# HiLab-git/FPL-plus

Hardware: NVIDIA B200
Metric: train_voxels_per_s (higher is better)
Workload: dtype bf16

## Files before the change

fpl-plus_b200/build.py:

```python
import os
import shutil
import subprocess
import sys

HERE = os.path.dirname(os.path.abspath(__file__))
CSRC = os.path.join(HERE, "csrc")
LIB = os.path.join(HERE, "libfplplus_b200.so")
SOURCES = ["api.cu", "dsbn.cu", "loss.cu", "filter.cu", "conv_direct.cu", "conv_tc.cu", "conv_wgrad_tc.cu", "conv_wgrad_hs.cu", "convt_tc.cu", "conv_tc_dfold.cu", "grad.cu", "adam.cu", "datapath.cu", "head.cu", "head_tc.cu", "stem_tc.cu", "upsample.cu"]
NVCC_FLAGS = ["-gencode", "arch=compute_100a,code=sm_100a", "-lineinfo", "-O3", "-std=c++17",
              "-Xcompiler", "-fPIC", "--use_fast_math=false"]


def _nvcc():
    for cand in (os.environ.get("NVCC"), shutil.which("nvcc"), "/usr/local/cuda/bin/nvcc"):
        if cand and os.path.exists(cand):
            return cand
    raise RuntimeError("nvcc not found; the fplplus_b200 CUDA library cannot be built")


def needs_build():
    if not os.path.exists(LIB):
        return True
    t = os.path.getmtime(LIB)
    deps = [os.path.join(CSRC, f) for f in os.listdir(CSRC)] + [os.path.join(HERE, "..", "include", "fplplus_b200.h")]
    return any(os.path.getmtime(d) > t for d in deps)


def build(force=False, verbose=False):
    ab = os.environ.get("FPL_LIB_AB")
    if ab and os.path.exists(ab):
        return ab
    if not force and not needs_build():
        return LIB
    nvcc = _nvcc()
    flags = [f for f in NVCC_FLAGS if not f.startswith("--use_fast_math")]
    objs = []
    bdir = os.path.join(HERE, "build")
    os.makedirs(bdir, exist_ok=True)
    procs = []
    for src in SOURCES:
        path = os.path.join(CSRC, src)
        if not os.path.exists(path):
            continue
        obj = os.path.join(bdir, src.replace(".cu", ".o"))
        objs.append(obj)
        cmd = [nvcc] + flags + ["-c", path, "-o", obj]
        if verbose:
            print(" ".join(cmd))
        procs.append((src, subprocess.Popen(cmd, stdout=subprocess.PIPE, stderr=subprocess.STDOUT)))
    for src, p in procs:
        out, _ = p.communicate()
        if p.returncode != 0:
            raise RuntimeError("nvcc failed on %s:\n%s" % (src, out.decode()))
    cmd = [nvcc, "-shared", "-gencode", "arch=compute_100a,code=sm_100a", "-o", LIB] + objs
    subprocess.check_call(cmd)
    return LIB


if __name__ == "__main__":
    print(build(force="--force" in sys.argv, verbose=True))
```

fpl-plus_b200/csrc/conv_wgrad_tc.cu:

```cuda
#include "common.cuh"
#include "tc_ptx.cuh"
#include "../../include/fplplus_b200.h"

namespace {

int g_wg_hs_dbg = 0;
int g_wg_hs = 1;
int g_wg_swap = 0, g_wg_allow_m64 = 1, g_wg_m64_quadrant = 1, g_wg_allow_pair = 1, g_wg_force_tw = 0, g_wg_tiles_per_cta = 2, g_wg_skip_epilogue = 0;

constexpr int kThreadsW = 192;
constexpr int kMaxStagesW = 8;
constexpr int kSmemBudgetW = 220 * 1024;

struct WgCfg {
    int th, tw;
    int nkd;
    int c8chunk;
    int mtiles_c, mtiles_kd;
    int m;
    int nb, nchunks;
    int plane_x, plane_dy;
    int dy_off;
    int x_bytes, dy_bytes, stage_bytes, stages, pad_bytes, smem_bytes;
    int tmem_cols;
    int ndy;
    int ncols;
};

bool make_wg_cfg(int h, int w, int cin, int cout, int kd, int allow_m64, int allow_pair, WgCfg& c) {
    if (cin % 8 != 0 || (cout % 16 != 0 && cout != 8) || cin <= 0 || cout <= 0) return false;
    c.tw = w >= 32 ? 32 : (w >= 16 ? 16 : 8);
    c.th = h >= 8 ? 8 : ((h + 1) / 2) * 2;
    const int g_all = cin / 8;
    c.ndy = 1;
    if (allow_pair && kd == 3 && g_all <= 4 && cout % 16 == 0) c.ndy = 2;
    else if (allow_pair && kd == 1 && cout == 8 && g_all <= 2) c.ndy = 4;
    else if (allow_pair && kd == 1 && cout == 8 && g_all <= 4) c.ndy = 2;
    else if (allow_pair && kd == 1 && cout == 16 && g_all <= 8) c.ndy = 2;
    if (c.ndy > 1) { c.nkd = c.ndy + kd - 1; c.c8chunk = g_all; c.mtiles_kd = 1; c.mtiles_c = 1; }
    else if (kd * g_all <= 16) { c.nkd = kd; c.c8chunk = g_all; c.mtiles_kd = 1; c.mtiles_c = 1; }
    else {
        c.nkd = 1; c.mtiles_kd = kd;
        c.c8chunk = g_all < 16 ? g_all : 16;
        if (g_all % c.c8chunk != 0) return false;
        c.mtiles_c = g_all / c.c8chunk;
    }
    const int groups = c.nkd * c.c8chunk;
    c.m = (groups <= 8 && allow_m64) ? 64 : 128;
    if (cout == 8 && c.m != 64) return false;
    c.nb = cout == 8 ? 8 : ((cout % 32 == 0 && c.ndy == 1) ? 32 : 16);
    c.ncols = c.ndy * c.nb;
    c.nchunks = cout / c.nb;
    if (groups > 8 && c.tw == 32 && cin >= 32 && h * w >= 128 * 128) c.tw = 16;
    if (g_wg_force_tw > 0 && g_wg_force_tw <= w) c.tw = g_wg_force_tw;
    c.plane_x = (c.th + 2) * (c.tw + 2) * 16;
    c.plane_dy = c.th * c.tw * 16;
    c.x_bytes = groups * c.plane_x;
    c.dy_bytes = (c.ncols / 8) * c.plane_dy;
    c.dy_off = ((c.x_bytes + 127) / 128) * 128;
    c.stage_bytes = ((c.dy_off + c.dy_bytes + 127) / 128) * 128;
    int over = (c.m / 8 + 1) * c.plane_x - c.stage_bytes;
    c.pad_bytes = over > 0 ? ((over + 127) / 128) * 128 : 0;
    c.stages = (kSmemBudgetW - c.pad_bytes - 2048) / c.stage_bytes;
    if (c.stages > kMaxStagesW) c.stages = kMaxStagesW;
    if (c.stages < 2) return false;
    c.smem_bytes = c.stages * c.stage_bytes + c.pad_bytes + 1024 + 256;
    int cols = 9 * c.ncols;
    c.tmem_cols = 32;
    while (c.tmem_cols < cols) c.tmem_cols *= 2;
    return c.tmem_cols <= 512;
}

struct WgParams {
    float* dw;
    float* dump;
    int N, D, H, W, cin, cout, kd;
    int x_c8off, dy_c8off;
    int th, tw, nkd, c8chunk, mtiles_c, mtiles_kd, m, nb, nchunks;
    int plane_x, plane_dy, x_bytes, dy_off, stage_bytes, stages, tmem_cols;
    int tiles_h, tiles_w, tiles_total, split;
    int swap_lbo_sbo, m64_quadrant_layout;
    int ndy, ncols, dplanes;
    int taps;
    int skip_epilogue;
    int tapmajor;
};

struct WgWork {
    int mt_kd, mt_c, nc, slice;
};

__device__ __forceinline__ WgWork decode_work(const WgParams& P, int b) {
    WgWork w;
    w.slice = b % P.split; b /= P.split;
    w.nc = b % P.nchunks; b /= P.nchunks;
    w.mt_c = b % P.mtiles_c;
    w.mt_kd = b / P.mtiles_c;
    return w;
}

__global__ void __launch_bounds__(kThreadsW) conv3d_wgrad_tc_kernel(const __grid_constant__ CUtensorMap xmap,
                                                                   const __grid_constant__ CUtensorMap dymap, WgParams P) {
    extern __shared__ uint8_t smem_raw[];
    uint8_t* smem = reinterpret_cast<uint8_t*>((reinterpret_cast<uintptr_t>(smem_raw) + 1023) & ~uintptr_t(1023));
    uint64_t* bars = reinterpret_cast<uint64_t*>(smem);
    uint64_t* full_bar = bars;
    uint64_t* empty_bar = bars + kMaxStagesW;
    uint64_t* done_bar = bars + 2 * kMaxStagesW;
    uint32_t* tmem_slot = reinterpret_cast<uint32_t*>(bars + 2 * kMaxStagesW + 1);
    uint8_t* ring = smem + 256;

    const int warp = threadIdx.x >> 5, lane = threadIdx.x & 31;
    const WgWork wk = decode_work(P, blockIdx.x);
    const int tile_begin = (int)(((int64_t)P.tiles_total * wk.slice) / P.split);
    const int tile_end = (int)(((int64_t)P.tiles_total * (wk.slice + 1)) / P.split);
    const int pad_d = P.kd / 2;
    const int kd0 = P.mtiles_kd > 1 ? wk.mt_kd : 0;

    if (warp == 0 && lane == 0) {
        asm volatile("prefetch.tensormap [%0];" ::"l"(&xmap) : "memory");
        asm volatile("prefetch.tensormap [%0];" ::"l"(&dymap) : "memory");
        for (int s = 0; s < P.stages; ++s) { mbar_init(&full_bar[s], 1); mbar_init(&empty_bar[s], 1); }
        mbar_init(done_bar, 1);
        fence_barrier_init();
    }
    if (warp == 1) tmem_alloc(tmem_slot, (uint32_t)P.tmem_cols);
    FPL_PDL_WAIT();
    tc_fence_before();
    __syncthreads();
    tc_fence_after();
    const uint32_t tmem_base = *tmem_slot;

    if (warp == 0) {
        if (lane == 0) {
            int stage = 0; uint32_t phase = 0;
            for (int t = tile_begin; t < tile_end; ++t) {
                int r = t;
                const int dp = r % P.dplanes; r /= P.dplanes;
                const int tw_i = r % P.tiles_w; r /= P.tiles_w;
                const int th_i = r % P.tiles_h;
                const int n = r / P.tiles_h;
                const int d = P.ndy * dp;
                mbar_wait(&empty_bar[stage], phase ^ 1);
                uint8_t* x_dst = ring + (size_t)stage * P.stage_bytes;
                uint8_t* dy_dst = x_dst + P.dy_off;
                mbar_expect_tx(&full_bar[stage], (uint32_t)(P.x_bytes + (P.ncols / 8) * P.plane_dy));
                tma_load_5d(x_dst, &xmap, &full_bar[stage], 2 * (tw_i * P.tw - 1), th_i * P.th - 1,
                            P.x_c8off + wk.mt_c * P.c8chunk, d + kd0 - pad_d, n);
                tma_load_5d(dy_dst, &dymap, &full_bar[stage], 2 * (tw_i * P.tw), th_i * P.th,
                            P.dy_c8off + wk.nc * (P.nb / 8), d, n);
                if (++stage == P.stages) { stage = 0; phase ^= 1; }
            }
        }
    } else if (warp == 1) {
        const uint32_t idesc = (1u << 4) | (1u << 7) | (1u << 10) | (1u << 15) | (1u << 16) |
                               ((uint32_t)(P.ncols >> 3) << 17) | ((uint32_t)(P.m >> 4) << 24);
        const uint32_t pitch_x = (uint32_t)(P.tw + 2) * 16, pitch_dy = (uint32_t)P.tw * 16;
        const uint32_t a_lbo = P.swap_lbo_sbo ? (uint32_t)P.plane_x : pitch_x;
        const uint32_t a_sbo = P.swap_lbo_sbo ? pitch_x : (uint32_t)P.plane_x;
        const uint32_t b_lbo = P.swap_lbo_sbo ? (uint32_t)P.plane_dy : pitch_dy;
        const uint32_t b_sbo = P.swap_lbo_sbo ? pitch_dy : (uint32_t)P.plane_dy;
        const uint64_t a_hi = make_desc(0, a_lbo, a_sbo), b_hi = make_desc(0, b_lbo, b_sbo);
        uint32_t tap_off[9];
#pragma unroll
        for (int t9 = 0; t9 < 9; ++t9) tap_off[t9] = ((uint32_t)(t9 / 3) * pitch_x + (uint32_t)(t9 % 3) * 16) >> 4;
        uint32_t d_tap[9];
#pragma unroll
        for (int t9 = 0; t9 < 9; ++t9) d_tap[t9] = tmem_base + (uint32_t)(t9 * P.ncols);
        const uint32_t ring_u = smem_u32(ring);
        const bool leader = elect_one();
        int stage = 0; uint32_t phase = 0;
        uint32_t accumulate = 0;
        for (int t = tile_begin; t < tile_end; ++t) {
            mbar_wait(&full_bar[stage], phase);
            tc_fence_after();
            const uint32_t x_base = (ring_u + (uint32_t)stage * (uint32_t)P.stage_bytes) >> 4;
            const uint32_t dy_base = x_base + ((uint32_t)P.dy_off >> 4);
            for (int hp = 0; hp < P.th / 2; ++hp) {
                const uint32_t a_row = x_base + (((uint32_t)(2 * hp) * pitch_x) >> 4);
                const uint32_t b_row = dy_base + (((uint32_t)(2 * hp) * pitch_dy) >> 4);
                uint64_t bdesc = b_hi + (uint64_t)b_row, a_col = a_hi + (uint64_t)a_row;
                for (int j = 0; j < P.tw / 8; ++j, bdesc += 8, a_col += 8) {
                    if (P.taps == 1) {
                        if (leader) umma_bf16(tmem_base, a_col + (uint64_t)tap_off[4], bdesc, idesc, accumulate);
                    } else {
#pragma unroll
                        for (int t9 = 0; t9 < 9; ++t9)
                            if (leader) umma_bf16(d_tap[t9], a_col + (uint64_t)tap_off[t9], bdesc, idesc, accumulate);
                    }
                    accumulate = 1;
                }
            }
            if (leader) umma_commit(&empty_bar[stage]);
            __syncwarp();
            if (++stage == P.stages) { stage = 0; phase ^= 1; }
        }
        if (leader) umma_commit(done_bar);
        __syncwarp();
        FPL_PDL_TRIGGER();
    } else if (tile_end > tile_begin) {
        const int quarter = warp & 3;
        mbar_wait(done_bar, 0);
        tc_fence_after();
        const int T = P.kd * P.taps;
        const int tlane = quarter * 32 + lane;
        int row;
        if (P.m == 128 || !P.m64_quadrant_layout) row = tlane;
        else row = (lane < 16) ? quarter * 16 + lane : -1;
        bool valid = row >= 0 && row < P.m;
        int kdi = 0, ci = 0;
        if (valid) {
            const int g = row >> 3;
            valid = g < P.nkd * P.c8chunk;
            kdi = kd0 + g / P.c8chunk;
            ci = (wk.mt_c * P.c8chunk + g % P.c8chunk) * 8 + (row & 7);
        }
        for (int t9 = 0; t9 < P.taps; ++t9) {
            for (int c0 = 0; c0 < P.ncols; c0 += 16) {
                uint32_t r[16];
                tmem_ld16(tmem_base + ((uint32_t)(quarter * 32) << 16) + (uint32_t)(t9 * P.ncols + c0), r);
                tmem_ld_wait();
                if (P.dump != nullptr && blockIdx.x == 0) {
#pragma unroll
                    for (int i = 0; i < 16; ++i) P.dump[((int64_t)t9 * 128 + tlane) * P.ncols + c0 + i] = __uint_as_float(r[i]);
                }
#pragma unroll
                for (int half = 0; half < 2; ++half) {
                    const int col = c0 + 8 * half;
                    const int dd = P.ndy > 1 ? col / P.nb : 0;
                    const int kd_tap = P.ndy > 1 ? kdi - dd : kdi;
                    const int co0 = wk.nc * P.nb + (col - dd * P.nb);
                    if (!(valid && kd_tap >= 0 && kd_tap < P.kd && !P.skip_epilogue)) continue;
                    if (P.tapmajor) {
                        float* base = P.dw + ((int64_t)(kd_tap * P.taps + t9) * P.cout + co0) * P.cin + ci;
#pragma unroll
                        for (int i = 0; i < 8; ++i) atomicAdd(base + (int64_t)i * P.cin, __uint_as_float(r[8 * half + i]));
                    } else {
#pragma unroll
                        for (int i = 0; i < 8; ++i)
                            atomicAdd(P.dw + ((int64_t)(co0 + i) * P.cin + ci) * T + kd_tap * P.taps + t9,
                                      __uint_as_float(r[8 * half + i]));
                    }
                }
            }
        }
    }
    tc_fence_before();
    __syncthreads();
    if (warp == 1) {
        tc_fence_after();
        tmem_dealloc(tmem_base, (uint32_t)P.tmem_cols);
    }
}

float* g_wg_dump = nullptr;

CUresult encode_5d(EncodeTiledFn encode, CUtensorMap* map, const void* base, int n, int d, int c8tot, int h, int w,
                   int box_w, int box_h, int box_c8, int box_d) {
    cuuint64_t gdim[5] = {(cuuint64_t)w * 2, (cuuint64_t)h, (cuuint64_t)c8tot, (cuuint64_t)d, (cuuint64_t)n};
    cuuint64_t gstr[4] = {(cuuint64_t)w * 16, (cuuint64_t)h * w * 16, (cuuint64_t)c8tot * h * w * 16,
                          (cuuint64_t)d * c8tot * h * w * 16};
    cuuint32_t box[5] = {(cuuint32_t)box_w * 2, (cuuint32_t)box_h, (cuuint32_t)box_c8, (cuuint32_t)box_d, 1};
    cuuint32_t estr[5] = {1, 1, 1, 1, 1};
    return encode(map, CU_TENSOR_MAP_DATA_TYPE_UINT64, 5, const_cast<void*>(base), gdim, gstr, box, estr,
                  CU_TENSOR_MAP_INTERLEAVE_NONE, CU_TENSOR_MAP_SWIZZLE_NONE, CU_TENSOR_MAP_L2_PROMOTION_L2_128B,
                  CU_TENSOR_MAP_FLOAT_OOB_FILL_NONE);
}

}

bool fpl_wgrad_hs_eligible(int d, int h, int w, int cin, int cout, int kd, int taps);
int fpl_wgrad_hs_launch(const void* x, int x_c8tot, int x_c8off, const void* dy, int dy_c8tot, int dy_c8off, float* dw, int n,
                        int d, int h, int w, int cin, int cout, void* stream, int tapmajor, int skip_epilogue, int force_tw, int dbg);
bool fpl_wgrad_rs_eligible(int d, int h, int w, int cin, int cout, int kd, int taps);
int fpl_wgrad_rs_launch(const void* x, int x_c8tot, int x_c8off, const void* dy, int dy_c8tot, int dy_c8off, float* dw, int n,
                        int d, int h, int w, void* stream, int tapmajor, int skip_epilogue);

void fpl_wgrad_debug_set(int key, long long value) {
    if (key == 10) g_wg_swap = (int)value;
    if (key == 11) g_wg_allow_m64 = (int)value;
    if (key == 12) g_wg_m64_quadrant = (int)value;
    if (key == 13) g_wg_dump = reinterpret_cast<float*>(value);
    if (key == 14) g_wg_allow_pair = (int)value;
    if (key == 15) g_wg_force_tw = (int)value;
    if (key == 16) g_wg_tiles_per_cta = (int)value;
    if (key == 17) g_wg_skip_epilogue = (int)value;
    if (key == 18) g_wg_hs = (int)value;
    if (key == 19) g_wg_hs_dbg = (int)value;
}

static int wgrad_tc_launch(const void* x, int x_c8tot, int x_c8off, const void* dy, int dy_c8tot, int dy_c8off,
                           float* dw, int n, int d, int h, int w, int cin, int cout, int kd, int taps, void* stream,
                           int tapmajor = 0) {
    FPL_REQUIRE(kd == 1 || kd == 3, "fpl_conv3d_wgrad_tc: kd=%d must be 1 or 3", kd);
    if (g_wg_hs && fpl_wgrad_hs_eligible(d, h, w, cin, cout, kd, taps))
        return fpl_wgrad_hs_launch(x, x_c8tot, x_c8off, dy, dy_c8tot, dy_c8off, dw, n, d, h, w, cin, cout, stream, tapmajor,
                                   g_wg_skip_epilogue, g_wg_force_tw, g_wg_hs_dbg);
    if (g_wg_hs && fpl_wgrad_rs_eligible(d, h, w, cin, cout, kd, taps))
        return fpl_wgrad_rs_launch(x, x_c8tot, x_c8off, dy, dy_c8tot, dy_c8off, dw, n, d, h, w, stream, tapmajor, g_wg_skip_epilogue);
    WgCfg c;
    FPL_REQUIRE(make_wg_cfg(h, w, cin, cout, kd, g_wg_allow_m64, g_wg_allow_pair && d >= 2, c),
                "fpl_conv3d_wgrad_tc: unsupported shape (cin %d, cout %d, %dx%d)", cin, cout, h, w);
    FPL_REQUIRE((reinterpret_cast<uintptr_t>(x) & 15) == 0 && (reinterpret_cast<uintptr_t>(dy) & 15) == 0,
                "fpl_conv3d_wgrad_tc: x/dy must be 16-byte aligned");
    EncodeTiledFn encode = get_encode_fn();
    FPL_REQUIRE(encode != nullptr, "fpl_conv3d_wgrad_tc: cuTensorMapEncodeTiled not available from the driver");
    CUtensorMap xmap, dymap;
    CUresult r = encode_5d(encode, &xmap, x, n, d, x_c8tot, h, w, c.tw + 2, c.th + 2, c.c8chunk, c.nkd);
    FPL_REQUIRE(r == CUDA_SUCCESS, "fpl_conv3d_wgrad_tc: tensor map (x) failed (%d)", (int)r);
    r = encode_5d(encode, &dymap, dy, n, d, dy_c8tot, h, w, c.tw, c.th, c.nb / 8, c.ndy);
    FPL_REQUIRE(r == CUDA_SUCCESS, "fpl_conv3d_wgrad_tc: tensor map (dy) failed (%d)", (int)r);
    WgParams P;
    P.dw = dw; P.dump = g_wg_dump;
    P.N = n; P.D = d; P.H = h; P.W = w; P.cin = cin; P.cout = cout; P.kd = kd;
    P.x_c8off = x_c8off; P.dy_c8off = dy_c8off;
    P.th = c.th; P.tw = c.tw; P.nkd = c.nkd; P.c8chunk = c.c8chunk; P.mtiles_c = c.mtiles_c; P.mtiles_kd = c.mtiles_kd;
    P.m = c.m; P.nb = c.nb; P.nchunks = c.nchunks; P.plane_x = c.plane_x; P.plane_dy = c.plane_dy; P.x_bytes = c.x_bytes; P.dy_off = c.dy_off;
    P.stage_bytes = c.stage_bytes; P.stages = c.stages; P.tmem_cols = c.tmem_cols;
    P.tiles_h = (h + c.th - 1) / c.th; P.tiles_w = (w + c.tw - 1) / c.tw;
    P.ndy = c.ndy; P.ncols = c.ncols; P.dplanes = (d + c.ndy - 1) / c.ndy;
    int64_t tiles = (int64_t)P.tiles_h * P.tiles_w * P.dplanes * n;
    FPL_REQUIRE(tiles < (1ll << 30), "fpl_conv3d_wgrad_tc: too many tiles");
    P.tiles_total = (int)tiles;
    const int pairs = c.mtiles_kd * c.mtiles_c * c.nchunks;
    int split = FPL_NUM_SMS / pairs;
    if (split > P.tiles_total / g_wg_tiles_per_cta) split = P.tiles_total / g_wg_tiles_per_cta;
    if (split < 1) split = 1;
    P.split = split;
    P.swap_lbo_sbo = g_wg_swap; P.m64_quadrant_layout = g_wg_m64_quadrant;
    P.taps = taps; P.skip_epilogue = g_wg_skip_epilogue; P.tapmajor = tapmajor;
    FPL_CHECK_CUDA(cudaFuncSetAttribute(conv3d_wgrad_tc_kernel, cudaFuncAttributeMaxDynamicSharedMemorySize, c.smem_bytes));
    fpl_launch(conv3d_wgrad_tc_kernel, pairs * split, kThreadsW, c.smem_bytes, (cudaStream_t)stream, xmap, dymap, P);
    FPL_LAUNCH_CHECK();
    return 0;
}

extern "C" int fpl_conv3d_wgrad_tc(const void* x, int x_c8tot, int x_c8off, const void* dy, int dy_c8tot, int dy_c8off,
                                   float* dw, int n, int d, int h, int w, int cin, int cout, int kd, void* stream) {
    return wgrad_tc_launch(x, x_c8tot, x_c8off, dy, dy_c8tot, dy_c8off, dw, n, d, h, w, cin, cout, kd, 9, stream);
}

extern "C" int fpl_conv3d_wgrad_tc_k311(const void* x, int x_c8tot, int x_c8off, const void* dy, int dy_c8tot, int dy_c8off,
                                        float* dw, int n, int d, int h, int w, int cin, int cout, void* stream) {
    return wgrad_tc_launch(x, x_c8tot, x_c8off, dy, dy_c8tot, dy_c8off, dw, n, d, h, w, cin, cout, 3, 1, stream);
}

extern "C" int fpl_conv3d_wgrad_tc_tapmajor(const void* x, int x_c8tot, int x_c8off, const void* dy, int dy_c8tot, int dy_c8off,
                                            float* scratch, int n, int d, int h, int w, int cin, int cout, int kd,
                                            void* stream) {
    return wgrad_tc_launch(x, x_c8tot, x_c8off, dy, dy_c8tot, dy_c8off, scratch, n, d, h, w, cin, cout, kd, 9, stream, 1);
}

namespace {
constexpr int kMaxFold = 64;
struct FoldBatch {
    const float* s[kMaxFold];
    float* dw[kMaxFold];
    int cout[kMaxFold], cin[kMaxFold], taps[kMaxFold], scout[kMaxFold];
};
constexpr int kFoldRows = 256;
__global__ void __launch_bounds__(256) fold_tapmajor_kernel(const __grid_constant__ FoldBatch B) {
    FPL_PDL_WAIT();
    __shared__ float tile[kFoldRows * 27];
    const int e = blockIdx.y;
    const float* __restrict__ s = B.s[e];
    float* dw = B.dw[e];
    const int cout = B.cout[e], cin = B.cin[e];
    const bool transposed = B.taps[e] < 0;
    const int T = transposed ? -B.taps[e] : B.taps[e];
    const int Tp = T | 1;
    const uint32_t magic = 0xffffffffu / (uint32_t)T + 1u;
    const int rows = cout * cin;
    const int64_t tap_stride = (int64_t)B.scout[e] * cin;
    for (int r0 = blockIdx.x * kFoldRows; r0 < rows; r0 += gridDim.x * kFoldRows) {
        const int nr = min(kFoldRows, rows - r0);
        const int r = threadIdx.x;
        if (r < nr) {
            int src = r0 + r;
            if (transposed) {
                const int ci = src / cout, co = src - ci * cout;
                src = co * cin + ci;
            }
            const float* sp = s + src;
            if (T == 27) {
                float t27[27];
#pragma unroll
                for (int tap = 0; tap < 27; ++tap) t27[tap] = __ldg(sp + tap * tap_stride);
#pragma unroll
                for (int tap = 0; tap < 27; ++tap) tile[r * Tp + tap] = t27[tap];
            } else {
#pragma unroll 9
                for (int tap = 0; tap < T; ++tap) tile[r * Tp + tap] = __ldg(sp + tap * tap_stride);
            }
        }
        __syncthreads();
        float* out = dw + (int64_t)r0 * T;
        const int total = nr * T;
        for (int i0 = threadIdx.x; i0 < total; i0 += 9 * (int)blockDim.x) {
            float v[9];
#pragma unroll
            for (int k = 0; k < 9; ++k) {
                const int i = i0 + k * (int)blockDim.x;
                v[k] = i < total ? out[i] : 0.0f;
            }
#pragma unroll
            for (int k = 0; k < 9; ++k) {
                const int i = i0 + k * (int)blockDim.x;
                if (i < total) {
                    const int rr = (int)__umulhi((uint32_t)i, magic), tap = i - rr * T;
                    out[i] = v[k] + tile[rr * Tp + tap];
                }
            }
        }
        __syncthreads();
    }
}
}

extern "C" int fpl_wgrad_tapmajor_to_dw_batch(int count, const float* const* h_scratch, float* const* h_dw, const int* h_cout,
                                              const int* h_cin, const int* h_taps, const int* h_scratch_cout, void* stream) {
    FPL_REQUIRE(count >= 0 && count <= kMaxFold, "fpl_wgrad_tapmajor_to_dw_batch: count %d not in [0,%d]", count, kMaxFold);
    if (count == 0) return 0;
    FoldBatch B;
    int max_total = 0;
    for (int e = 0; e < count; ++e) {
        B.s[e] = h_scratch[e]; B.dw[e] = h_dw[e]; B.cout[e] = h_cout[e]; B.cin[e] = h_cin[e]; B.taps[e] = h_taps[e];
        B.scout[e] = h_scratch_cout != nullptr ? h_scratch_cout[e] : h_cout[e];
        FPL_REQUIRE((h_taps[e] < 0 ? -h_taps[e] : h_taps[e]) <= 27 && h_taps[e] != 0, "fpl_wgrad_tapmajor_to_dw_batch: tap count %d out of range", h_taps[e]);
        FPL_REQUIRE(B.scout[e] >= B.cout[e], "fpl_wgrad_tapmajor_to_dw_batch: scratch rows %d < folded rows %d", B.scout[e], B.cout[e]);
        const int total = h_cout[e] * h_cin[e] * (h_taps[e] < 0 ? -h_taps[e] : h_taps[e]);
        if (total > max_total) max_total = total;
    }
    int bx = (max_total / 9 + kFoldRows - 1) / kFoldRows;
    if (bx > 296) bx = 296;
    if (bx < 1) bx = 1;
    fpl_launch(fold_tapmajor_kernel, dim3(bx, count), 256, 0, (cudaStream_t)stream, B);
    FPL_LAUNCH_CHECK();
    return 0;
}
```

fpl-plus_b200/csrc/convt_tc.cu:

```cuda
#include "common.cuh"
#include "tc_ptx.cuh"
#include "../../include/fplplus_b200.h"

namespace {

constexpr int kTH = 16, kTW = 8;
constexpr int kPlane = kTH * kTW * 16;
constexpr int kThreadsT = 192;
constexpr int kMaxStagesT = 8;

__device__ __forceinline__ void tma_load_4d(void* dst, const CUtensorMap* map, uint64_t* bar, int c0, int c1, int c2, int c3) {
    asm volatile(
        "cp.async.bulk.tensor.4d.shared::cluster.global.tile.mbarrier::complete_tx::bytes [%0], [%1, {%3, %4, %5, %6}], [%2];"
        ::"r"(smem_u32(dst)), "l"(map), "r"(smem_u32(bar)), "r"(c0), "r"(c1), "r"(c2), "r"(c3)
        : "memory");
}

struct CtParams {
    const __nv_bfloat16* image;
    const float* bias;
    bf16x8* out;
    int out_c8tot, out_c8off;
    int a_c8tot, a_c8off;
    int N, D, H, W;
    int cin, cout, kd2, ntaps;
    int mode;
    int kdim, ndim;
    int nb, kc, nslices, nchunks, a_bytes, b_bytes, stages, tmem_cols;
    int tiles_h, tiles_w, total_items;
};

struct CtCfg {
    int nb, kc, nslices, nchunks, a_bytes, b_bytes, stages, tmem_cols, smem_bytes;
};

bool make_ct_cfg(int kdim, int ndim, int kc_div, CtCfg& c) {
    if (kdim % 16 || ndim % 16) return false;
    c.nb = ndim;
    if (c.nb > 128) {
        if (ndim % 128 == 0) c.nb = 128;
        else if (ndim % 64 == 0) c.nb = 64;
        else if (ndim % 32 == 0) c.nb = 32;
        else c.nb = 16;
    }
    c.kc = 64;
    while (c.kc > 16 && (kc_div % c.kc != 0)) c.kc /= 2;
    if (kc_div % c.kc != 0) return false;
    c.nslices = ndim / c.nb;
    c.nchunks = kdim / c.kc;
    c.a_bytes = (c.kc / 8) * kPlane;
    c.b_bytes = c.kc * c.nb * 2;
    int stage = c.a_bytes + c.b_bytes;
    c.stages = (96 * 1024) / stage;
    if (c.stages > kMaxStagesT) c.stages = kMaxStagesT;
    if (c.stages < 2) c.stages = 2;
    int cols = 2 * c.nb;
    c.tmem_cols = 32;
    while (c.tmem_cols < cols) c.tmem_cols *= 2;
    c.smem_bytes = c.stages * stage + 1024 + 256 + (ndim > 1024 ? ndim : 1024) * (int)sizeof(float) + 16;
    return true;
}

__global__ void __launch_bounds__(kThreadsT) convt_gemm_tc_kernel(const __grid_constant__ CUtensorMap amap, CtParams P) {
    extern __shared__ uint8_t smem_raw[];
    uint8_t* smem = reinterpret_cast<uint8_t*>((reinterpret_cast<uintptr_t>(smem_raw) + 1023) & ~uintptr_t(1023));
    const int stage_bytes = P.a_bytes + P.b_bytes;
    uint64_t* bars = reinterpret_cast<uint64_t*>(smem + (size_t)P.stages * stage_bytes);
    uint64_t* full_bar = bars;
    uint64_t* empty_bar = bars + kMaxStagesT;
    uint64_t* tmem_full = bars + 2 * kMaxStagesT;
    uint64_t* tmem_empty = bars + 2 * kMaxStagesT + 2;
    uint32_t* tmem_slot = reinterpret_cast<uint32_t*>(bars + 2 * kMaxStagesT + 4);
    float* bias_sm = reinterpret_cast<float*>(bars + 2 * kMaxStagesT + 6);

    const int warp = threadIdx.x >> 5, lane = threadIdx.x & 31;
    if (warp == 0 && lane == 0) {
        asm volatile("prefetch.tensormap [%0];" ::"l"(&amap) : "memory");
        for (int s = 0; s < P.stages; ++s) { mbar_init(&full_bar[s], 1); mbar_init(&empty_bar[s], 1); }
        for (int a = 0; a < 2; ++a) { mbar_init(&tmem_full[a], 1); mbar_init(&tmem_empty[a], 4); }
        fence_barrier_init();
    }
    if (warp == 1) tmem_alloc(tmem_slot, (uint32_t)P.tmem_cols);
    FPL_PDL_WAIT();
    if (P.mode == 0)
        for (int i = threadIdx.x; i < P.ndim; i += kThreadsT) bias_sm[i] = P.bias != nullptr ? P.bias[i % P.cout] : 0.0f;
    tc_fence_before();
    __syncthreads();
    tc_fence_after();
    const uint32_t tmem_base = *tmem_slot;
    const int Do = P.D * P.kd2;
    const int chunks_per_tap = P.cout / P.kc;

    if (warp == 0) {
        if (lane == 0) {
            int stage = 0; uint32_t phase = 0;
            for (int it = blockIdx.x; it < P.total_items; it += gridDim.x) {
                int t = it;
                const int tw = t % P.tiles_w; t /= P.tiles_w;
                const int th = t % P.tiles_h; t /= P.tiles_h;
                const int d = t % P.D; t /= P.D;
                const int n = t % P.N;
                const int slice = t / P.N;
                for (int q = 0; q < P.nchunks; ++q) {
                    mbar_wait(&empty_bar[stage], phase ^ 1);
                    uint8_t* a_dst = smem + (size_t)stage * stage_bytes;
                    mbar_expect_tx(&full_bar[stage], (uint32_t)(P.a_bytes + P.b_bytes));
                    if (P.mode == 0) {
                        tma_load_4d(a_dst, &amap, &full_bar[stage], 0, tw * kTW, th * kTH,
                                    (n * P.D + d) * P.a_c8tot + P.a_c8off + q * (P.kc / 8));
                    } else {
                        const int tap = q / chunks_per_tap, cq = q - tap * chunks_per_tap;
                        const int a = P.kd2 == 2 ? tap >> 2 : 0, b = (tap >> 1) & 1, c = tap & 1;
                        tma_load_4d(a_dst, &amap, &full_bar[stage], 0, 2 * tw * kTW + c, 2 * th * kTH + b,
                                    (n * Do + d * P.kd2 + a) * P.a_c8tot + P.a_c8off + cq * (P.kc / 8));
                    }
                    const uint8_t* b_src = reinterpret_cast<const uint8_t*>(P.image) + (size_t)(slice * P.nchunks + q) * P.b_bytes;
                    bulk_load(a_dst + P.a_bytes, b_src, (uint32_t)P.b_bytes, &full_bar[stage]);
                    if (++stage == P.stages) { stage = 0; phase ^= 1; }
                }
            }
        }
    } else if (warp == 1) {
        const uint32_t idesc = (1u << 4) | (1u << 7) | (1u << 10) | ((uint32_t)(P.nb >> 3) << 17) | (8u << 24);
        const uint64_t a_hi = make_desc(0, kPlane, kTW * 16), b_hi = make_desc(0, (uint32_t)P.nb * 16, 128);
        const uint32_t smem_u = smem_u32(smem) >> 4;
        const int ksteps = P.kc / 16;
        const bool leader = elect_one();
        int stage = 0; uint32_t phase = 0;
        int acc = 0; uint32_t acc_phase = 0;
        for (int it = blockIdx.x; it < P.total_items; it += gridDim.x) {
            mbar_wait(&tmem_empty[acc], acc_phase ^ 1);
            tc_fence_after();
            const uint32_t d_tmem = tmem_base + (uint32_t)(acc * P.nb);
            uint32_t accumulate = 0;
            for (int q = 0; q < P.nchunks; ++q) {
                mbar_wait(&full_bar[stage], phase);
                tc_fence_after();
                const uint32_t a_base = smem_u + (uint32_t)(((size_t)stage * stage_bytes) >> 4);
                const uint32_t b_base = a_base + (uint32_t)(P.a_bytes >> 4);
                uint64_t adesc = a_hi + (uint64_t)a_base, bdesc = b_hi + (uint64_t)b_base;
                const uint64_t b_step = (uint64_t)(2 * P.nb);
                for (int j = 0; j < ksteps; ++j, adesc += 2 * kPlane / 16, bdesc += b_step) {
                    if (leader) umma_bf16(d_tmem, adesc, bdesc, idesc, accumulate);
                    accumulate = 1;
                }
                if (leader) umma_commit(&empty_bar[stage]);
                __syncwarp();
                if (++stage == P.stages) { stage = 0; phase ^= 1; }
            }
            if (leader) umma_commit(&tmem_full[acc]);
            __syncwarp();
            if (++acc == 2) { acc = 0; acc_phase ^= 1; }
        }
        FPL_PDL_TRIGGER();
    } else {
        const int quarter = warp & 3;
        const int row = quarter * 32 + lane;
        const int hl = row / kTW, wl = row % kTW;
        int acc = 0; uint32_t acc_phase = 0;
        const int Ho = P.H * 2, Wo = P.W * 2;
        for (int it = blockIdx.x; it < P.total_items; it += gridDim.x) {
            int t = it;
            const int tw = t % P.tiles_w; t /= P.tiles_w;
            const int th = t % P.tiles_h; t /= P.tiles_h;
            const int d = t % P.D; t /= P.D;
            const int n = t % P.N;
            const int slice = t / P.N;
            mbar_wait(&tmem_full[acc], acc_phase);
            tc_fence_after();
            const int h = th * kTH + hl, w = tw * kTW + wl;
            const bool valid = h < P.H && w < P.W;
            const uint32_t t_row = tmem_base + ((uint32_t)(quarter * 32) << 16) + (uint32_t)(acc * P.nb);
            for (int c0 = 0; c0 < P.nb; c0 += 16) {
                uint32_t r[16];
                tmem_ld16(t_row + (uint32_t)c0, r);
                tmem_ld_wait();
                float v[16];
                const int col = slice * P.nb + c0;
                if (P.mode == 0) {
#pragma unroll
                    for (int i = 0; i < 16; ++i) v[i] = __uint_as_float(r[i]) + bias_sm[col + i];
                    if (valid) {
                        const int tap = col / P.cout, co = col - tap * P.cout;
                        const int a = P.kd2 == 2 ? tap >> 2 : 0, b = (tap >> 1) & 1, c = tap & 1;
                        const int64_t HWo = (int64_t)Ho * Wo;
                        bf16x8* dst = P.out + (((int64_t)n * Do + d * P.kd2 + a) * P.out_c8tot + P.out_c8off + co / 8) * HWo +
                                      (int64_t)(2 * h + b) * Wo + (2 * w + c);
                        st_bf16x8(dst, v);
                        st_bf16x8(dst + HWo, v + 8);
                    }
                } else {
#pragma unroll
                    for (int i = 0; i < 16; ++i) v[i] = __uint_as_float(r[i]);
                    if (valid) {
                        const int64_t HW = (int64_t)P.H * P.W;
                        bf16x8* dst = P.out + (((int64_t)n * P.D + d) * P.out_c8tot + P.out_c8off + col / 8) * HW + (int64_t)h * P.W + w;
                        st_bf16x8(dst, v);
                        st_bf16x8(dst + HW, v + 8);
                    }
                }
            }
            tc_fence_before();
            __syncwarp();
            if (lane == 0) mbar_arrive(&tmem_empty[acc]);
            if (++acc == 2) { acc = 0; acc_phase ^= 1; }
        }
    }
    tc_fence_before();
    __syncthreads();
    if (warp == 1) {
        tc_fence_after();
        tmem_dealloc(tmem_base, (uint32_t)P.tmem_cols);
    }
}

__global__ void convt_prep_kernel(const float* __restrict__ w, __nv_bfloat16* image, int cin, int cout, int ntaps, int mode,
                                  int nb, int kc, int nchunks, int total) {
    FPL_PDL_WAIT();
    for (int i = blockIdx.x * blockDim.x + threadIdx.x; i < total; i += gridDim.x * blockDim.x) {
        int t = i;
        const int el = t % 8; t /= 8;
        const int nrow = t % nb; t /= nb;
        const int k8 = t % (kc / 8); t /= (kc / 8);
        const int q = t % nchunks;
        const int sl = t / nchunks;
        const int k = q * kc + k8 * 8 + el, nn = sl * nb + nrow;
        int ci, co, tap;
        if (mode == 0) { ci = k; tap = nn / cout; co = nn - tap * cout; }
        else { tap = k / cout; co = k - tap * cout; ci = nn; }
        image[i] = __float2bfloat16_rn(w[((int64_t)ci * cout + co) * ntaps + tap]);
    }
}

CUresult encode_4d(EncodeTiledFn encode, CUtensorMap* map, const void* base, int64_t planes, int h, int w, int box_c8,
                   int stride) {
    cuuint64_t gdim[4] = {8, (cuuint64_t)w, (cuuint64_t)h, (cuuint64_t)planes};
    cuuint64_t gstr[3] = {16, (cuuint64_t)w * 16, (cuuint64_t)h * w * 16};
    cuuint32_t box[4] = {8, (cuuint32_t)(kTW * stride), (cuuint32_t)(kTH * stride), (cuuint32_t)box_c8};
    cuuint32_t estr[4] = {1, (cuuint32_t)stride, (cuuint32_t)stride, 1};
    return encode(map, CU_TENSOR_MAP_DATA_TYPE_BFLOAT16, 4, const_cast<void*>(base), gdim, gstr, box, estr,
                  CU_TENSOR_MAP_INTERLEAVE_NONE, CU_TENSOR_MAP_SWIZZLE_NONE, CU_TENSOR_MAP_L2_PROMOTION_L2_128B,
                  CU_TENSOR_MAP_FLOAT_OOB_FILL_NONE);
}

struct CtwParams {
    float* dw;
    int N, D, H, W, cin, cout, kd2, ntaps;
    int x_c8tot, x_c8off, dy_c8tot, dy_c8off;
    int mgroups, m, nb, mtiles, nchunks;
    int x_bytes, dy_tile_bytes, stage_bytes, stages, tmem_cols;
    int tiles_h, tiles_w, tiles_total, split;
    int tapmajor;
};

__global__ void __launch_bounds__(kThreadsT) convt_wgrad_tc_kernel(const __grid_constant__ CUtensorMap xmap,
                                                                  const __grid_constant__ CUtensorMap dymap, CtwParams P) {
    extern __shared__ uint8_t smem_raw[];
    uint8_t* smem = reinterpret_cast<uint8_t*>((reinterpret_cast<uintptr_t>(smem_raw) + 1023) & ~uintptr_t(1023));
    uint64_t* bars = reinterpret_cast<uint64_t*>(smem);
    uint64_t* full_bar = bars;
    uint64_t* empty_bar = bars + kMaxStagesT;
    uint64_t* done_bar = bars + 2 * kMaxStagesT;
    uint32_t* tmem_slot = reinterpret_cast<uint32_t*>(bars + 2 * kMaxStagesT + 1);
    uint8_t* ring = smem + 256;

    const int warp = threadIdx.x >> 5, lane = threadIdx.x & 31;
    int b = blockIdx.x;
    const int slice = b % P.split; b /= P.split;
    const int nc = b % P.nchunks;
    const int mt = b / P.nchunks;
    const int tile_begin = (int)(((int64_t)P.tiles_total * slice) / P.split);
    const int tile_end = (int)(((int64_t)P.tiles_total * (slice + 1)) / P.split);
    const int Do = P.D * P.kd2;

    if (warp == 0 && lane == 0) {
        asm volatile("prefetch.tensormap [%0];" ::"l"(&xmap) : "memory");
        asm volatile("prefetch.tensormap [%0];" ::"l"(&dymap) : "memory");
        for (int s = 0; s < P.stages; ++s) { mbar_init(&full_bar[s], 1); mbar_init(&empty_bar[s], 1); }
        mbar_init(done_bar, 1);
        fence_barrier_init();
    }
    if (warp == 1) tmem_alloc(tmem_slot, (uint32_t)P.tmem_cols);
    FPL_PDL_WAIT();
    tc_fence_before();
    __syncthreads();
    tc_fence_after();
    const uint32_t tmem_base = *tmem_slot;

    if (warp == 0) {
        if (lane == 0) {
            int stage = 0; uint32_t phase = 0;
            for (int t = tile_begin; t < tile_end; ++t) {
                int r = t;
                const int tw = r % P.tiles_w; r /= P.tiles_w;
                const int th = r % P.tiles_h; r /= P.tiles_h;
                const int d = r % P.D;
                const int n = r / P.D;
                mbar_wait(&empty_bar[stage], phase ^ 1);
                uint8_t* x_dst = ring + (size_t)stage * P.stage_bytes;
                mbar_expect_tx(&full_bar[stage], (uint32_t)(P.x_bytes + P.ntaps * P.dy_tile_bytes));
                tma_load_4d(x_dst, &xmap, &full_bar[stage], 0, tw * kTW, th * kTH,
                            (n * P.D + d) * P.x_c8tot + P.x_c8off + mt * P.mgroups);
                for (int tap = 0; tap < P.ntaps; ++tap) {
                    const int a = P.kd2 == 2 ? tap >> 2 : 0, bb = (tap >> 1) & 1, c = tap & 1;
                    tma_load_4d(x_dst + P.x_bytes + (size_t)tap * P.dy_tile_bytes, &dymap, &full_bar[stage], 0,
                                2 * tw * kTW + c, 2 * th * kTH + bb,
                                (n * Do + d * P.kd2 + a) * P.dy_c8tot + P.dy_c8off + nc * (P.nb / 8));
                }
                if (++stage == P.stages) { stage = 0; phase ^= 1; }
            }
        }
    } else if (warp == 1) {
        const uint32_t idesc = (1u << 4) | (1u << 7) | (1u << 10) | (1u << 15) | (1u << 16) |
                               ((uint32_t)(P.nb >> 3) << 17) | ((uint32_t)(P.m >> 4) << 24);
        const uint64_t hi = make_desc(0, kTW * 16, kPlane);
        const uint32_t ring_u = smem_u32(ring);
        const bool leader = elect_one();
        int stage = 0; uint32_t phase = 0;
        uint32_t accumulate = 0;
        for (int t = tile_begin; t < tile_end; ++t) {
            mbar_wait(&full_bar[stage], phase);
            tc_fence_after();
            const uint32_t x_base = (ring_u + (uint32_t)stage * (uint32_t)P.stage_bytes) >> 4;
            const uint32_t dy_base = x_base + ((uint32_t)P.x_bytes >> 4);
            uint64_t adesc = hi + (uint64_t)x_base, b_hp = hi + (uint64_t)dy_base;
            const uint64_t dy_tile16 = (uint64_t)((uint32_t)P.dy_tile_bytes >> 4);
            for (int hp = 0; hp < kTH / 2; ++hp, adesc += 2 * kTW * 16 / 16, b_hp += 2 * kTW * 16 / 16) {
                uint64_t bdesc = b_hp;
                uint32_t d_tap = tmem_base;
                for (int tap = 0; tap < P.ntaps; ++tap, bdesc += dy_tile16, d_tap += (uint32_t)P.nb) {
                    if (leader) umma_bf16(d_tap, adesc, bdesc, idesc, accumulate);
                }
                accumulate = 1;
            }
            if (leader) umma_commit(&empty_bar[stage]);
            __syncwarp();
            if (++stage == P.stages) { stage = 0; phase ^= 1; }
        }
        if (leader) umma_commit(done_bar);
        __syncwarp();
        FPL_PDL_TRIGGER();
    } else if (tile_end > tile_begin) {
        const int quarter = warp & 3;
        mbar_wait(done_bar, 0);
        tc_fence_after();
        const int tlane = quarter * 32 + lane;
        int row = P.m == 128 ? tlane : ((lane < 16) ? quarter * 16 + lane : -1);
        const bool valid = row >= 0 && row < P.mgroups * 8 && (mt * P.mgroups * 8 + row) < P.cin;
        const int ci = mt * P.mgroups * 8 + row;
        for (int tap = 0; tap < P.ntaps; ++tap) {
            for (int c0 = 0; c0 < P.nb; c0 += 16) {
                uint32_t r[16];
                tmem_ld16(tmem_base + ((uint32_t)(quarter * 32) << 16) + (uint32_t)(tap * P.nb + c0), r);
                tmem_ld_wait();
                if (valid) {
#pragma unroll
                    for (int i = 0; i < 16; ++i) {
                        const int co = nc * P.nb + c0 + i;
                        if (P.tapmajor) atomicAdd(P.dw + ((int64_t)tap * P.cout + co) * P.cin + ci, __uint_as_float(r[i]));
                        else atomicAdd(P.dw + ((int64_t)ci * P.cout + co) * P.ntaps + tap, __uint_as_float(r[i]));
                    }
                }
            }
        }
    }
    tc_fence_before();
    __syncthreads();
    if (warp == 1) {
        tc_fence_after();
        tmem_dealloc(tmem_base, (uint32_t)P.tmem_cols);
    }
}

}

extern "C" int64_t fpl_convt_weight_image_bytes(int cin, int cout, int kd2) {
    return (int64_t)cin * cout * 4 * kd2 * 2;
}

extern "C" int fpl_convt_prep_weight(const float* w, int cin, int cout, int kd2, int mode, void* image, void* stream) {
    FPL_REQUIRE(kd2 == 1 || kd2 == 2, "fpl_convt_prep_weight: kd2=%d must be 1 or 2", kd2);
    const int ntaps = 4 * kd2;
    CtCfg c;
    const int kdim = mode == 0 ? cin : ntaps * cout, ndim = mode == 0 ? ntaps * cout : cin;
    FPL_REQUIRE(make_ct_cfg(kdim, ndim, mode == 0 ? cin : cout, c), "fpl_convt_prep_weight: unsupported channels (%d -> %d)", cin, cout);
    const int total = kdim * ndim;
    int blocks = (total + 255) / 256;
    if (blocks > FPL_NUM_SMS * 4) blocks = FPL_NUM_SMS * 4;
    fpl_launch(convt_prep_kernel, blocks, 256, 0, (cudaStream_t)stream, w, (__nv_bfloat16*)image, cin, cout, ntaps, mode, c.nb, c.kc,
                                                               c.nchunks, total);
    FPL_LAUNCH_CHECK();
    return 0;
}

namespace {
constexpr int kMaxCtBatch = 16;
struct CtPrepBatch {
    const float* w[kMaxCtBatch];
    __nv_bfloat16* image[kMaxCtBatch];
    int cin[kMaxCtBatch], cout[kMaxCtBatch], ntaps[kMaxCtBatch], mode[kMaxCtBatch], nb[kMaxCtBatch], kc[kMaxCtBatch],
        nchunks[kMaxCtBatch], total[kMaxCtBatch];
};
__global__ void convt_prep_batch_kernel(const __grid_constant__ CtPrepBatch B) {
    FPL_PDL_WAIT();
    const int e = blockIdx.y;
    const float* __restrict__ w = B.w[e];
    __nv_bfloat16* image = B.image[e];
    const int cout = B.cout[e], ntaps = B.ntaps[e], mode = B.mode[e], nb = B.nb[e], kc = B.kc[e], nchunks = B.nchunks[e];
    for (int i = blockIdx.x * blockDim.x + threadIdx.x; i < B.total[e]; i += gridDim.x * blockDim.x) {
        int t = i;
        const int el = t % 8; t /= 8;
        const int nrow = t % nb; t /= nb;
        const int k8 = t % (kc / 8); t /= (kc / 8);
        const int q = t % nchunks;
        const int sl = t / nchunks;
        const int k = q * kc + k8 * 8 + el, nn = sl * nb + nrow;
        int ci, co, tap;
        if (mode == 0) { ci = k; tap = nn / cout; co = nn - tap * cout; }
        else { tap = k / cout; co = k - tap * cout; ci = nn; }
        image[i] = __float2bfloat16_rn(w[((int64_t)ci * cout + co) * ntaps + tap]);
    }
}
}

extern "C" int fpl_convt_prep_weight_batch(int count, const float* const* h_w, const int* h_cin, const int* h_cout,
                                           const int* h_kd2, const int* h_mode, void* const* h_images, void* stream) {
    FPL_REQUIRE(count >= 0 && count <= kMaxCtBatch, "fpl_convt_prep_weight_batch: count %d not in [0,%d]", count, kMaxCtBatch);
    if (count == 0) return 0;
    CtPrepBatch B;
    int max_total = 0;
    for (int e = 0; e < count; ++e) {
        const int ntaps = 4 * h_kd2[e], mode = h_mode[e], cin = h_cin[e], cout = h_cout[e];
        const int kdim = mode == 0 ? cin : ntaps * cout, ndim = mode == 0 ? ntaps * cout : cin;
        CtCfg c;
        FPL_REQUIRE(make_ct_cfg(kdim, ndim, mode == 0 ? cin : cout, c), "fpl_convt_prep_weight_batch: unsupported channels (%d -> %d)", cin, cout);
        B.w[e] = h_w[e]; B.image[e] = (__nv_bfloat16*)h_images[e]; B.cin[e] = cin; B.cout[e] = cout; B.ntaps[e] = ntaps;
        B.mode[e] = mode; B.nb[e] = c.nb; B.kc[e] = c.kc; B.nchunks[e] = c.nchunks; B.total[e] = kdim * ndim;
        if (B.total[e] > max_total) max_total = B.total[e];
    }
    int bx = (max_total + 255) / 256;
    if (bx > 64) bx = 64;
    fpl_launch(convt_prep_batch_kernel, dim3(bx, count), 256, 0, (cudaStream_t)stream, B);
    FPL_LAUNCH_CHECK();
    return 0;
}

static int convt_gemm_launch(int mode, const void* a, int a_c8tot, int a_c8off, const void* image, const float* bias, void* out,
                             int out_c8tot, int out_c8off, int n, int d, int h, int w, int cin, int cout, int kd2,
                             void* stream) {
    FPL_REQUIRE(kd2 == 1 || kd2 == 2, "fpl_convt_k2s2_tc: kd2=%d must be 1 or 2", kd2);
    const int ntaps = 4 * kd2;
    const int kdim = mode == 0 ? cin : ntaps * cout, ndim = mode == 0 ? ntaps * cout : cin;
    CtCfg c;
    FPL_REQUIRE(make_ct_cfg(kdim, ndim, mode == 0 ? cin : cout, c), "fpl_convt_k2s2_tc: unsupported channels (%d -> %d)", cin, cout);
    FPL_REQUIRE(ndim <= 8192, "fpl_convt_k2s2_tc: GEMM N = %d too large", ndim);
    EncodeTiledFn encode = get_encode_fn();
    FPL_REQUIRE(encode != nullptr, "fpl_convt_k2s2_tc: cuTensorMapEncodeTiled not available from the driver");
    CUtensorMap amap;
    CUresult r;
    if (mode == 0) r = encode_4d(encode, &amap, a, (int64_t)n * d * a_c8tot, h, w, c.kc / 8, 1);
    else r = encode_4d(encode, &amap, a, (int64_t)n * d * kd2 * a_c8tot, 2 * h, 2 * w, c.kc / 8, 2);
    FPL_REQUIRE(r == CUDA_SUCCESS, "fpl_convt_k2s2_tc: tensor map failed (%d)", (int)r);
    CtParams P;
    P.image = (const __nv_bfloat16*)image; P.bias = bias; P.out = (bf16x8*)out; P.out_c8tot = out_c8tot; P.out_c8off = out_c8off;
    P.a_c8tot = a_c8tot; P.a_c8off = a_c8off; P.N = n; P.D = d; P.H = h; P.W = w; P.cin = cin; P.cout = cout; P.kd2 = kd2;
    P.ntaps = ntaps; P.mode = mode; P.kdim = kdim; P.ndim = ndim;
    P.nb = c.nb; P.kc = c.kc; P.nslices = c.nslices; P.nchunks = c.nchunks; P.a_bytes = c.a_bytes; P.b_bytes = c.b_bytes;
    P.stages = c.stages; P.tmem_cols = c.tmem_cols;
    P.tiles_h = (h + kTH - 1) / kTH; P.tiles_w = (w + kTW - 1) / kTW;
    int64_t total = (int64_t)P.tiles_h * P.tiles_w * d * n * c.nslices;
    FPL_REQUIRE(total < (1ll << 30), "fpl_convt_k2s2_tc: too many tiles");
    P.total_items = (int)total;
    FPL_CHECK_CUDA(cudaFuncSetAttribute(convt_gemm_tc_kernel, cudaFuncAttributeMaxDynamicSharedMemorySize, c.smem_bytes));
    int grid = FPL_NUM_SMS * 2;
    if (grid > P.total_items) grid = P.total_items;
    fpl_launch(convt_gemm_tc_kernel, grid, kThreadsT, c.smem_bytes, (cudaStream_t)stream, amap, P);
    FPL_LAUNCH_CHECK();
    return 0;
}

extern "C" int fpl_convt_k2s2_fwd_tc(const void* x, int x_c8tot, int x_c8off, const void* image, const float* bias, void* y,
                                     int y_c8tot, int y_c8off, int n, int d, int h, int w, int cin, int cout, int kd2,
                                     void* stream) {
    return convt_gemm_launch(0, x, x_c8tot, x_c8off, image, bias, y, y_c8tot, y_c8off, n, d, h, w, cin, cout, kd2, stream);
}

extern "C" int fpl_convt_k2s2_dgrad_tc(const void* dy, int dy_c8tot, int dy_c8off, const void* image_t, void* dx, int dx_c8tot,
                                       int dx_c8off, int n, int d, int h, int w, int cin, int cout, int kd2, void* stream) {
    return convt_gemm_launch(1, dy, dy_c8tot, dy_c8off, image_t, nullptr, dx, dx_c8tot, dx_c8off, n, d, h, w, cin, cout, kd2,
                             stream);
}

static int convt_wgrad_launch(const void* x, int x_c8tot, int x_c8off, const void* dy, int dy_c8tot, int dy_c8off,
                              float* dw, int n, int d, int h, int w, int cin, int cout, int kd2, void* stream, int tapmajor) {
    FPL_REQUIRE(kd2 == 1 || kd2 == 2, "fpl_convt_k2s2_wgrad_tc: kd2=%d must be 1 or 2", kd2);
    FPL_REQUIRE(cin % 8 == 0 && cout % 16 == 0, "fpl_convt_k2s2_wgrad_tc: unsupported channels (%d -> %d)", cin, cout);
    EncodeTiledFn encode = get_encode_fn();
    FPL_REQUIRE(encode != nullptr, "fpl_convt_k2s2_wgrad_tc: cuTensorMapEncodeTiled not available from the driver");
    CtwParams P;
    P.dw = dw; P.N = n; P.D = d; P.H = h; P.W = w; P.cin = cin; P.cout = cout; P.kd2 = kd2; P.ntaps = 4 * kd2;
    P.x_c8tot = x_c8tot; P.x_c8off = x_c8off; P.dy_c8tot = dy_c8tot; P.dy_c8off = dy_c8off; P.tapmajor = tapmajor;
    const int g_all = cin / 8;
    P.mgroups = g_all < 16 ? g_all : 16;
    FPL_REQUIRE(g_all % P.mgroups == 0, "fpl_convt_k2s2_wgrad_tc: cin=%d not tileable", cin);
    P.mtiles = g_all / P.mgroups;
    P.m = P.mgroups <= 8 ? 64 : 128;
    P.nb = cout % 32 == 0 ? 32 : 16;
    P.x_bytes = P.mgroups * kPlane;
    if (2 * (P.x_bytes + P.ntaps * (P.nb / 8) * kPlane) > 200 * 1024 - (P.m / 8) * kPlane) P.nb = 16;
    P.nchunks = cout / P.nb;
    P.dy_tile_bytes = (P.nb / 8) * kPlane;
    P.stage_bytes = P.x_bytes + P.ntaps * P.dy_tile_bytes;
    P.stages = (200 * 1024 - (P.m / 8) * kPlane) / P.stage_bytes;
    if (P.stages > kMaxStagesT) P.stages = kMaxStagesT;
    FPL_REQUIRE(P.stages >= 2, "fpl_convt_k2s2_wgrad_tc: stage of %d bytes does not fit twice", P.stage_bytes);
    int cols = P.ntaps * P.nb;
    P.tmem_cols = 32;
    while (P.tmem_cols < cols) P.tmem_cols *= 2;
    CUtensorMap xmap, dymap;
    CUresult r = encode_4d(encode, &xmap, x, (int64_t)n * d * x_c8tot, h, w, P.mgroups, 1);
    FPL_REQUIRE(r == CUDA_SUCCESS, "fpl_convt_k2s2_wgrad_tc: tensor map (x) failed (%d)", (int)r);
    r = encode_4d(encode, &dymap, dy, (int64_t)n * d * kd2 * dy_c8tot, 2 * h, 2 * w, P.nb / 8, 2);
    FPL_REQUIRE(r == CUDA_SUCCESS, "fpl_convt_k2s2_wgrad_tc: tensor map (dy) failed (%d)", (int)r);
    P.tiles_h = (h + kTH - 1) / kTH; P.tiles_w = (w + kTW - 1) / kTW;
    int64_t tiles = (int64_t)P.tiles_h * P.tiles_w * d * n;
    FPL_REQUIRE(tiles < (1ll << 30), "fpl_convt_k2s2_wgrad_tc: too many tiles");
    P.tiles_total = (int)tiles;
    const int pairs = P.mtiles * P.nchunks;
    int split = FPL_NUM_SMS / pairs;
    if (split > P.tiles_total / 4) split = P.tiles_total / 4;
    if (split < 1) split = 1;
    P.split = split;
    const int smem_bytes = P.stages * P.stage_bytes + (P.m / 8) * kPlane + 1024 + 256;
    FPL_CHECK_CUDA(cudaFuncSetAttribute(convt_wgrad_tc_kernel, cudaFuncAttributeMaxDynamicSharedMemorySize, smem_bytes));
    fpl_launch(convt_wgrad_tc_kernel, pairs * split, kThreadsT, smem_bytes, (cudaStream_t)stream, xmap, dymap, P);
    FPL_LAUNCH_CHECK();
    return 0;
}

extern "C" int fpl_convt_k2s2_wgrad_tc(const void* x, int x_c8tot, int x_c8off, const void* dy, int dy_c8tot, int dy_c8off,
                                       float* dw, int n, int d, int h, int w, int cin, int cout, int kd2, void* stream) {
    return convt_wgrad_launch(x, x_c8tot, x_c8off, dy, dy_c8tot, dy_c8off, dw, n, d, h, w, cin, cout, kd2, stream, 0);
}

extern "C" int fpl_convt_k2s2_wgrad_tc_tapmajor(const void* x, int x_c8tot, int x_c8off, const void* dy, int dy_c8tot,
                                                int dy_c8off, float* scratch, int n, int d, int h, int w, int cin, int cout,
                                                int kd2, void* stream) {
    return convt_wgrad_launch(x, x_c8tot, x_c8off, dy, dy_c8tot, dy_c8off, scratch, n, d, h, w, cin, cout, kd2, stream, 1);
}
```

fpl-plus_b200/csrc/tc_ptx.cuh:

```cuda
#pragma once
#include <cuda.h>
#include <stdint.h>

namespace {

__device__ __forceinline__ uint32_t smem_u32(const void* p) { return (uint32_t)__cvta_generic_to_shared(p); }

__device__ __forceinline__ void mbar_init(uint64_t* bar, uint32_t count) {
    asm volatile("mbarrier.init.shared::cta.b64 [%0], %1;" ::"r"(smem_u32(bar)), "r"(count));
}
__device__ __forceinline__ void mbar_expect_tx(uint64_t* bar, uint32_t bytes) {
    asm volatile("mbarrier.arrive.expect_tx.shared::cta.b64 _, [%0], %1;" ::"r"(smem_u32(bar)), "r"(bytes) : "memory");
}
__device__ __forceinline__ void mbar_arrive(uint64_t* bar) {
    asm volatile("mbarrier.arrive.shared::cta.b64 _, [%0];" ::"r"(smem_u32(bar)) : "memory");
}
__device__ __forceinline__ void mbar_wait(uint64_t* bar, uint32_t parity) {
    uint32_t done;
    do {
        asm volatile(
            "{\n"
            ".reg .pred p;\n"
            "mbarrier.try_wait.parity.shared::cta.b64 p, [%1], %2;\n"
            "selp.u32 %0, 1, 0, p;\n"
            "}\n"
            : "=r"(done)
            : "r"(smem_u32(bar)), "r"(parity)
            : "memory");
    } while (!done);
}
__device__ __forceinline__ void fence_barrier_init() { asm volatile("fence.mbarrier_init.release.cluster;" ::: "memory"); }
__device__ __forceinline__ void fence_proxy_async() { asm volatile("fence.proxy.async.shared::cta;" ::: "memory"); }

__device__ __forceinline__ void tma_load_3d(void* dst, const CUtensorMap* map, uint64_t* bar, int c0, int c1, int c2) {
    asm volatile(
        "cp.async.bulk.tensor.3d.shared::cluster.global.tile.mbarrier::complete_tx::bytes [%0], [%1, {%3, %4, %5}], [%2];"
        ::"r"(smem_u32(dst)), "l"(map), "r"(smem_u32(bar)), "r"(c0), "r"(c1), "r"(c2)
        : "memory");
}
__device__ __forceinline__ void tma_load_5d(void* dst, const CUtensorMap* map, uint64_t* bar, int c0, int c1, int c2, int c3,
                                            int c4) {
    asm volatile(
        "cp.async.bulk.tensor.5d.shared::cluster.global.tile.mbarrier::complete_tx::bytes [%0], [%1, {%3, %4, %5, %6, %7}], [%2];"
        ::"r"(smem_u32(dst)), "l"(map), "r"(smem_u32(bar)), "r"(c0), "r"(c1), "r"(c2), "r"(c3), "r"(c4)
        : "memory");
}

__device__ __forceinline__ void bulk_load(void* dst, const void* src, uint32_t bytes, uint64_t* bar) {
    asm volatile("cp.async.bulk.shared::cluster.global.mbarrier::complete_tx::bytes [%0], [%1], %2, [%3];" ::"r"(smem_u32(dst)),
                 "l"(src), "r"(bytes), "r"(smem_u32(bar))
                 : "memory");
}

__device__ __forceinline__ void tmem_alloc(uint32_t* dst_smem, uint32_t ncols) {
    asm volatile("tcgen05.alloc.cta_group::1.sync.aligned.shared::cta.b32 [%0], %1;" ::"r"(smem_u32(dst_smem)), "r"(ncols) : "memory");
    asm volatile("tcgen05.relinquish_alloc_permit.cta_group::1.sync.aligned;" ::: "memory");
}
__device__ __forceinline__ void tmem_dealloc(uint32_t taddr, uint32_t ncols) {
    asm volatile("tcgen05.dealloc.cta_group::1.sync.aligned.b32 %0, %1;" ::"r"(taddr), "r"(ncols) : "memory");
}
__device__ __forceinline__ void tc_fence_before() { asm volatile("tcgen05.fence::before_thread_sync;" ::: "memory"); }
__device__ __forceinline__ void tc_fence_after() { asm volatile("tcgen05.fence::after_thread_sync;" ::: "memory"); }

__device__ __forceinline__ void umma_bf16(uint32_t tmem_d, uint64_t adesc, uint64_t bdesc, uint32_t idesc, uint32_t accumulate) {
    asm volatile(
        "{\n"
        ".reg .pred p;\n"
        "setp.ne.b32 p, %4, 0;\n"
        "tcgen05.mma.cta_group::1.kind::f16 [%0], %1, %2, %3, p;\n"
        "}\n" ::"r"(tmem_d),
        "l"(adesc), "l"(bdesc), "r"(idesc), "r"(accumulate)
        : "memory");
}
__device__ __forceinline__ void umma_commit(uint64_t* bar) {
    asm volatile("tcgen05.commit.cta_group::1.mbarrier::arrive::one.shared::cluster.b64 [%0];" ::"r"(smem_u32(bar)) : "memory");
}
__device__ __forceinline__ void tmem_ld16(uint32_t taddr, uint32_t* r) {
    asm volatile(
        "tcgen05.ld.sync.aligned.32x32b.x16.b32 {%0,%1,%2,%3,%4,%5,%6,%7,%8,%9,%10,%11,%12,%13,%14,%15}, [%16];"
        : "=r"(r[0]), "=r"(r[1]), "=r"(r[2]), "=r"(r[3]), "=r"(r[4]), "=r"(r[5]), "=r"(r[6]), "=r"(r[7]), "=r"(r[8]),
          "=r"(r[9]), "=r"(r[10]), "=r"(r[11]), "=r"(r[12]), "=r"(r[13]), "=r"(r[14]), "=r"(r[15])
        : "r"(taddr));
}
__device__ __forceinline__ void tmem_ld_wait() { asm volatile("tcgen05.wait::ld.sync.aligned;" ::: "memory"); }

__device__ __forceinline__ bool elect_one() {
    uint32_t pred;
    asm volatile(
        "{\n"
        ".reg .pred p;\n"
        "elect.sync _|p, 0xffffffff;\n"
        "selp.u32 %0, 1, 0, p;\n"
        "}\n"
        : "=r"(pred));
    return pred != 0;
}

__device__ __forceinline__ uint64_t make_desc(uint32_t saddr, uint32_t lbo_bytes, uint32_t sbo_bytes) {
    uint64_t d = 0;
    d |= (uint64_t)((saddr >> 4) & 0x3FFFu);
    d |= (uint64_t)((lbo_bytes >> 4) & 0x3FFFu) << 16;
    d |= (uint64_t)((sbo_bytes >> 4) & 0x3FFFu) << 32;
    d |= (uint64_t)1 << 46;
    return d;
}


typedef CUresult (*EncodeTiledFn)(CUtensorMap*, CUtensorMapDataType, cuuint32_t, void*, const cuuint64_t*, const cuuint64_t*,
                                  const cuuint32_t*, const cuuint32_t*, CUtensorMapInterleave, CUtensorMapSwizzle,
                                  CUtensorMapL2promotion, CUtensorMapFloatOOBfill);

inline EncodeTiledFn get_encode_fn() {
    static EncodeTiledFn fn = nullptr;
    if (fn == nullptr) {
        void* p = nullptr;
        cudaDriverEntryPointQueryResult qres;
        if (cudaGetDriverEntryPoint("cuTensorMapEncodeTiled", &p, cudaEnableDefault, &qres) == cudaSuccess &&
            qres == cudaDriverEntryPointSuccess)
            fn = reinterpret_cast<EncodeTiledFn>(p);
    }
    return fn;
}

}
```

fpl-plus_b200/lib.py:

```python
import ctypes
import os
from ctypes import c_char_p, c_double, c_float, c_int, c_int64, c_longlong, c_uint64, c_void_p

from . import build as _build

_P = c_void_p
_I = c_int
_L = c_int64
_F = c_float
_U = c_uint64

_SIGNATURES = {
    "fpl_last_error": (c_char_p, []),
    "fpl_version": (_I, []),
    "fpl_set_sm_budget": (_I, [_I]),
    "fpl_launch_count": (c_longlong, [_I]),
    "fpl_device_is_sm100": (_I, []),
    "fpl_debug_set": (None, [_I, c_longlong]),
    "fpl_conv3d_weight_image_bytes": (_L, [_I, _I, _I]),
    "fpl_conv3d_prep_weight": (_I, [_P, _I, _I, _I, _I, _P, _P]),
    "fpl_conv3d_prep_weight_batch": (_I, [_I, ctypes.POINTER(c_void_p), ctypes.POINTER(_I), ctypes.POINTER(_I),
                                          ctypes.POINTER(_I), ctypes.POINTER(_I), ctypes.POINTER(c_void_p), _P]),
    "fpl_conv3d_tc": (_I, [_P, _I, _I, _P, _P, _P, _I, _I, _P] + [_I] * 7 + [_P]),
    "fpl_conv3d_dfold_image_bytes": (_L, [_I, _I]),
    "fpl_conv3d_dfold_prep_weight": (_I, [_P, _I, _I, _I, _P, _P]),
    "fpl_conv3d_dfold_prep_weight_batch": (_I, [_I, ctypes.POINTER(c_void_p), ctypes.POINTER(_I), ctypes.POINTER(_I),
                                                ctypes.POINTER(_I), ctypes.POINTER(c_void_p), _P]),
    "fpl_conv3d_tc_dfold": (_I, [_P, _I, _I, _P, _P, _P, _I, _I, _P] + [_I] * 6 + [_P]),
    "fpl_patch9_c8": (_I, [_P, _P, _I, _I, _I, _I, _I, _P]),
    "fpl_conv3d_k311_prep_weight": (_I, [_P, _I, _I, _P, _P]),
    "fpl_conv3d_tc_k311": (_I, [_P, _I, _I, _P, _P, _P, _I, _I, _P] + [_I] * 7 + [_P]),
    "fpl_conv3d_wgrad_tc_k311": (_I, [_P, _I, _I, _P, _I, _I, _P] + [_I] * 6 + [_P]),
    "fpl_conv3d_direct": (_I, [_P, _I, _I, _P, _P, _P, _I, _I, _P] + [_I] * 9 + [_P]),
    "fpl_conv3d_wgrad": (_I, [_P, _I, _I, _P, _I, _I, _P] + [_I] * 7 + [_P]),
    "fpl_conv3d_wgrad_tc": (_I, [_P, _I, _I, _P, _I, _I, _P] + [_I] * 7 + [_P]),
    "fpl_conv3d_wgrad_tc_tapmajor": (_I, [_P, _I, _I, _P, _I, _I, _P] + [_I] * 7 + [_P]),
    "fpl_wgrad_tapmajor_to_dw_batch": (_I, [_I, ctypes.POINTER(c_void_p), ctypes.POINTER(c_void_p), ctypes.POINTER(_I),
                                            ctypes.POINTER(_I), ctypes.POINTER(_I), ctypes.POINTER(_I), _P]),
    "fpl_dsbn_eval_affine_batch": (_I, [_I] + [ctypes.POINTER(c_void_p)] * 7 + [ctypes.POINTER(_I), _F, _P]),
    "fpl_conv3d_tc_act": (_I, [_P, _I, _I, _P, _P, _I, _I] + [_I] * 7 + [_P, _P, _P, _F, _U, _U, _P, _P]),
    "fpl_conv3d_tc_dfold_act": (_I, [_P, _I, _I, _P, _P, _I, _I] + [_I] * 6 + [_P, _P, _P, _P]),
    "fpl_conv3d_tc_k311_act": (_I, [_P, _I, _I, _P, _P, _I, _I] + [_I] * 7 + [_P, _P, _P, _P]),
    "fpl_maxpool_c8": (_I, [_P, _I, _I, _P, _I, _I, _I] + [_I] * 5 + [_P]),
    "fpl_head_fwd": (_I, [_P, _I, _I, _P, _P, _P] + [_I] * 6 + [_P]),
    "fpl_head_dgrad": (_I, [_P, _P, _P, _I, _I, _P, _I, _I, _P] + [_I] * 6 + [_P]),
    "fpl_upsample2x_c8": (_I, [_P, _I, _I, _P, _I, _I] + [_I] * 6 + [_P]),
    "fpl_upsample2x_c8_bwd": (_I, [_P, _I, _I, _P, _I, _I] + [_I] * 6 + [_P]),
    "fpl_channel_sum_c8": (_I, [_P, _I, _I, _P] + [_I] * 5 + [_P]),
    "fpl_grad_scatter_add": (_I, [_P, _P, _P, _I, _I, _P]),
    "fpl_stem_conv_fwd": (_I, [_P, _P, _P, _P, _I, _I, _P] + [_I] * 7 + [_P]),
    "fpl_stem_conv_wgrad": (_I, [_P, _P, _I, _I, _P] + [_I] * 7 + [_P]),
    "fpl_head_conv_fwd": (_I, [_P, _I, _I, _P, _P, _P] + [_I] * 6 + [_P]),
    "fpl_head_conv_tc": (_I, [_P, _I, _I, _P, _P, _P] + [_I] * 6 + [_P]),
    "fpl_pack_ncdhw_to_c8": (_I, [_P, _I, _P, _I, _I, _I, _P] + [_I] * 4 + [_P]),
    "fpl_head_conv_bwd": (_I, [_P, _I, _I, _P, _P, _P, _I, _I, _P, _P] + [_I] * 6 + [_P]),
    "fpl_convt_k2s2_fwd": (_I, [_P, _I, _I, _P, _P, _P, _I, _I] + [_I] * 7 + [_P]),
    "fpl_convt_k2s2_bwd": (_I, [_P, _I, _I, _P, _P, _I, _I, _P, _I, _I, _P, _P] + [_I] * 7 + [_P]),
    "fpl_convt_weight_image_bytes": (_L, [_I, _I, _I]),
    "fpl_convt_prep_weight": (_I, [_P, _I, _I, _I, _I, _P, _P]),
    "fpl_convt_prep_weight_batch": (_I, [_I, ctypes.POINTER(c_void_p), ctypes.POINTER(_I), ctypes.POINTER(_I),
                                         ctypes.POINTER(_I), ctypes.POINTER(_I), ctypes.POINTER(c_void_p), _P]),
    "fpl_convt_k2s2_fwd_tc": (_I, [_P, _I, _I, _P, _P, _P, _I, _I] + [_I] * 7 + [_P]),
    "fpl_convt_k2s2_dgrad_tc": (_I, [_P, _I, _I, _P, _P, _I, _I] + [_I] * 7 + [_P]),
    "fpl_convt_k2s2_wgrad_tc": (_I, [_P, _I, _I, _P, _I, _I, _P] + [_I] * 7 + [_P]),
    "fpl_convt_k2s2_wgrad_tc_tapmajor": (_I, [_P, _I, _I, _P, _I, _I, _P] + [_I] * 7 + [_P]),
    "fpl_dsbn_finalize": (_I, [_P, _L, _P, _P, _P, _P, _P, _F, _F, _I, _P, _P, _P, _P, _I, _P]),
    "fpl_dsbn_act_fwd": (_I, [_P, _P, _P, _P, _P, _I, _I, _P, _I, _I, _P, _I, _F, _P, _U, _U, _P] + [_I] * 5 + [_P]),
    "fpl_dsbn_bn_act_fwd": (_I, [_P, _P, _L, _P, _P, _P, _P, _P, _F, _F, _I, _P, _P, _P, _P, _P,
                                 _P, _I, _I, _P, _I, _I, _P, _I, _F, _P, _U, _U, _P] + [_I] * 5 + [_P]),
    "fpl_dsbn_act_bwd_apply_fin": (_I, [_P, _P, _I, _I, _P, _I, _I, _P, _I, _P, _P, _P, _P, _P, _F, _P, _U, _U, _P, _P, _I, _P]
                                   + [_I] * 5 + [_P, _P, _P, _P, _P]),
    "fpl_dsbn_act_bwd_reduce": (_I, [_P, _P, _I, _I, _P, _I, _I, _P, _I, _P, _P, _P, _P, _P, _F, _P, _U, _U, _P, _P]
                                + [_I] * 5 + [_P]),
    "fpl_dsbn_act_bwd_apply": (_I, [_P, _P, _I, _I, _P, _I, _I, _P, _I, _P, _P, _P, _P, _P, _F, _P, _U, _U, _P, _P, _I, _P]
                               + [_I] * 5 + [_P]),
    "fpl_dsbn_bwd_finalize": (_I, [_P, _P, _P, _I, _P, _P, _P, _P, _I, _P]),
    "fpl_conv3d_tc_bwdred": (_I, [_P, _I, _I, _P, _P, _I, _I] + [_I] * 7 + [_P, _P, _P, _P, _P, _P, _F, _U, _U, _P, _P, _P]),
    "fpl_conv3d_tc_dfold_bwdred": (_I, [_P, _I, _I, _P, _P, _I, _I] + [_I] * 6 + [_P, _P, _P, _P, _P, _P, _F, _U, _U, _P, _P, _P]),
    "fpl_gather_patches": (_I, [_P, _I, _I, _I, _I, _I, _P, _P, _P, _P]),
    "fpl_adam_multi_tensor": (_I, [_P, _I, _P, _I, _P, c_double, c_double, c_double, c_double, c_double, _P, _P]),
    "fpl_adam_chunk_elems": (_I, []),
    "fpl_dice_ce_reduce": (_I, [_P, _P, _P, _P, _I, _I, _L, _P]),
    "fpl_dice_ce_grad": (_I, [_P, _P, _P, _P, _F, _F, _F, _P, _P, _P, _I, _I, _L, _P]),
    "fpl_dice_ce_reduce_ex": (_I, [_P, _P, _P, _P, _P, _P, _P, _I, _I, _L, _I, _I, _P]),
    "fpl_dice_ce_grad_ex": (_I, [_P, _P, _P, _P, _P, _P, _P, _F, _F, _F, _F, _P, _P, _P, _I, _I, _L, _I, _I, _P]),
    "fpl_dice_ce_loss_ex": (_I, [_P, _P, _P, _P, _P, _P, _P, _F, _F, _F, _P, _P, _I, _I, _L, _I, _I, _P]),
    "fpl_argmax_label": (_I, [_P, _P, _I, _I, _L, _P]),
    "fpl_mc_uncertainty": (_I, [ctypes.POINTER(c_void_p), _I, _I, _L, _P, _P, _P]),
    "fpl_mc_uncertainty_max_passes": (_I, []),
    "fpl_agree_weight": (_I, [_P, _P, _P, _P, _P, _I, _F, _P, _I, _L, _P]),
    "fpl_window_accumulate": (_I, [_P, _P, _P] + [_I] * 13 + [_F, _P]),
    "fpl_window_normalize": (_I, [_P, _P, _F, _L, _P]),
}

EXPORTED = [k for k in _SIGNATURES if k != "fpl_debug_set"]

_lib = None


class FplError(RuntimeError):
    pass


def load():
    global _lib
    if _lib is None:
        path = _build.build()
        lib = ctypes.CDLL(path)
        for name, (res, args) in _SIGNATURES.items():
            fn = getattr(lib, name)
            fn.restype = res
            fn.argtypes = args
        for item in os.environ.get("FPL_DEBUG_SET", "").split(","):
            if "=" in item:
                k, v = item.split("=", 1)
                lib.fpl_debug_set(int(k), int(v))
        _lib = lib
    return _lib


_call_timer = None


def set_call_timer(fn):
    global _call_timer
    _call_timer = fn


_debug_skip = frozenset(n for n in os.environ.get("FPL_DEBUG_SKIP", "").split(",") if n)
if _debug_skip:
    import sys as _sys
    print("fplplus_b200: FPL_DEBUG_SKIP is set -- %d entry points are NOT launched; results are wrong (profiling only)"
          % len(_debug_skip), file=_sys.stderr)


def call(name, *args):
    if _debug_skip and name in _debug_skip:
        return
    lib = load()
    tok = _call_timer(name, args) if _call_timer is not None else None
    rc = getattr(lib, name)(*args)
    if tok is not None:
        tok.stop()
    if rc != 0:
        raise FplError("%s failed (%d): %s" % (name, rc, lib.fpl_last_error().decode()))


def launch_count(reset=False):
    return int(load().fpl_launch_count(1 if reset else 0))
```

fpl-plus_b200/net.py:

```python
import ctypes
import os

import torch
import torch.nn as nn

from . import ops
from .ops import C8, call, ptr, stream_ptr


class DomainSpecificBatchNorm2d(nn.Module):
    def __init__(self, num_features, num_domains):
        super().__init__()
        self.bns = nn.ModuleList([nn.BatchNorm2d(num_features) for _ in range(num_domains)])


class DomainSpecificBatchNorm3d(nn.Module):
    def __init__(self, num_features, num_domains):
        super().__init__()
        self.bns = nn.ModuleList([nn.BatchNorm3d(num_features) for _ in range(num_domains)])


class ConvBlockND(nn.Module):

    def __init__(self, in_channels, out_channels, num_domains=None, dim=2, dropout_p=0.5):
        super().__init__()
        self.conv2d_1 = nn.Conv2d(in_channels, out_channels, kernel_size=3, padding=1)
        self.conv2d_2 = nn.Conv2d(out_channels, out_channels, kernel_size=3, padding=1)
        self.conv3d_1 = nn.Conv3d(in_channels, out_channels, kernel_size=3, padding=1)
        self.conv3d_2 = nn.Conv3d(out_channels, out_channels, kernel_size=3, padding=1)
        self.bn2d1 = DomainSpecificBatchNorm2d(out_channels, num_domains)
        self.bn2d2 = DomainSpecificBatchNorm2d(out_channels, num_domains)
        self.bn3d1 = DomainSpecificBatchNorm3d(out_channels, num_domains)
        self.bn3d2 = DomainSpecificBatchNorm3d(out_channels, num_domains)
        self.dropout_p = dropout_p
        self.dropout = nn.Dropout(dropout_p)
        self.relu_1 = nn.PReLU()
        self.relu_2 = nn.PReLU()
        self.dim = dim
        self.in_channels, self.out_channels = in_channels, out_channels

    def units(self):
        if self.dim == 2:
            return ((self.conv2d_1, self.bn2d1, self.relu_1, self.dropout),
                    (self.conv2d_2, self.bn2d2, self.relu_2, None))
        return ((self.conv3d_1, self.bn3d1, self.relu_1, self.dropout),
                (self.conv3d_2, self.bn3d2, self.relu_2, None))


class DownBlock(nn.Module):
    def __init__(self, in_channels, out_channels, num_domains=None, dim=2, dropout_p=0.0, downsample=True):
        super().__init__()
        self.downsample, self.dim = downsample, dim
        self.conv = ConvBlockND(in_channels, out_channels, num_domains, dim, dropout_p)


class UpBlock(nn.Module):
    def __init__(self, in_channels1, in_channels2, out_channels, num_domains=None, dim=2, dropout_p=0.0,
                 bilinear=True):
        super().__init__()
        self.bilinear, self.dim = bilinear, dim
        self.conv2d = nn.Conv2d(in_channels1, in_channels2, kernel_size=1)
        self.conv3d = nn.Conv3d(in_channels1, in_channels2, kernel_size=1)
        self.trans2d = nn.ConvTranspose2d(in_channels1, in_channels2, kernel_size=2, stride=2)
        self.trans3d = nn.ConvTranspose3d(in_channels1, in_channels2, kernel_size=2, stride=2)
        self.conv = ConvBlockND(in_channels2 * 2, out_channels, num_domains, dim, dropout_p)


class _Unit(object):

    def __init__(self, name, conv, dsbn, prelu, dropout, kd, is_stem=False):
        self.name, self.conv, self.dsbn, self.prelu, self.dropout = name, conv, dsbn, prelu, dropout
        self.kd, self.is_stem = kd, is_stem
        self.cin, self.cout = conv.in_channels, conv.out_channels


class _Workspace(object):
    def __init__(self, device):
        self.device = device
        self.t = {}

    def get(self, name, shape, dtype):
        t = self.t.get(name)
        if t is None or tuple(t.shape) != tuple(shape) or t.dtype != dtype:
            t = torch.empty(shape, dtype=dtype, device=self.device)
            self.t[name] = t
        return t

    def c8(self, name, n, d, c, h, w):
        return self.get(name, (n, d, c // 8, h, w, 8), torch.bfloat16)


class _Lease(object):

    def __init__(self, pool, ws):
        self.pool, self.ws = pool, ws

    def __del__(self):
        try:
            self.pool.append(self.ws)
        except Exception:
            pass


def _conv_impl():
    return os.environ.get("FPL_CONV_IMPL", "tc")


class UNet2D5_dsbn(nn.Module):

    def __init__(self, params):
        super().__init__()
        self.params = params
        self.in_chns = params['in_chns']
        self.ft_chns = list(params['feature_chns'])
        self.dropout = list(params['dropout'])
        self.dims = list(params['conv_dims'])
        self.n_class = params['class_num']
        self.bilinear = params['bilinear']
        self.num_domains = params['num_domains']
        assert len(self.ft_chns) == 5
        ft, nd, dm, dp = self.ft_chns, self.num_domains, self.dims, self.dropout
        self.block0 = DownBlock(self.in_chns, ft[0], nd, dm[0], dp[0], True)
        self.block1 = DownBlock(ft[0], ft[1], nd, dm[1], dp[1], True)
        self.block2 = DownBlock(ft[1], ft[2], nd, dm[2], dp[2], True)
        self.block3 = DownBlock(ft[2], ft[3], nd, dm[3], dp[3], True)
        self.block4 = DownBlock(ft[3], ft[4], nd, dm[4], dp[4], False)
        self.up1 = UpBlock(ft[4], ft[3], ft[3], nd, dm[3], dropout_p=dp[3], bilinear=self.bilinear)
        self.up2 = UpBlock(ft[3], ft[2], ft[2], nd, dm[2], dropout_p=dp[2], bilinear=self.bilinear)
        self.up3 = UpBlock(ft[2], ft[1], ft[1], nd, dm[1], dropout_p=dp[1], bilinear=self.bilinear)
        self.up4 = UpBlock(ft[1], ft[0], ft[0], nd, dm[0], dropout_p=dp[0], bilinear=self.bilinear)
        self.out_conv = nn.Conv3d(ft[0], self.n_class, kernel_size=(1, 3, 3), padding=(0, 1, 1))
        self._pool = []
        self._infer_ws = None
        self._img_cache = {}
        self._dropout_masks = None
        self._rng_dev = None
        self._rng_lanes = {}
        self._cur_lane = 0
        self._seed_from_device = False
        self._graphs = {}
        self._graph_ws_keep = []
        self._infer_wss = {}
        self.cuda_graphs = os.environ.get("FPL_CUDA_GRAPH", "1") != "0"
        self.wgrad_side_stream = os.environ.get("FPL_WGRAD_STREAM", "0") != "0"
        self._aux_streams = {}
        self._dfold_cache = {}
        self._unit_depth = {}
        self.grad_ready_hook = None
        self.grad_wait_hook = None
        self.grad_bucket_bytes = 4 << 20
        self.grad_tail_bytes = 3 << 19
        self._master = None
        self._head = UNet2D5_dsbn._HeadConv(self.out_conv)
        self._stem = None
        self._head_unit = None
        self._head_dirty = True
        self._stem_dirty = True
        self._geo0 = (0, 0, 0)
        self._grad_pass = False
        self._build_plan()

    def _build_plan(self):
        for c in self.ft_chns:
            if c % 8 != 0:
                raise ValueError("feature_chns must be multiples of 8, got {0:}".format(self.ft_chns))
        blocks = [self.block0, self.block1, self.block2, self.block3, self.block4]
        ups = [self.up1, self.up2, self.up3, self.up4]
        self._down_units, self._up_units = [], []
        for i, b in enumerate(blocks):
            kd = 3 if b.dim == 3 else 1
            (c1, n1, r1, d1), (c2, n2, r2, _d2) = b.conv.units()
            self._down_units.append((_Unit("block%d.conv#1" % i, c1, n1, r1, d1, kd, is_stem=(i == 0)),
                                     _Unit("block%d.conv#2" % i, c2, n2, r2, None, kd)))
        for k, u in enumerate(ups, start=1):
            kd = 3 if u.dim == 3 else 1
            (c1, n1, r1, d1), (c2, n2, r2, _d2) = u.conv.units()
            self._up_units.append((_Unit("up%d.conv#1" % k, c1, n1, r1, d1, kd),
                                   _Unit("up%d.conv#2" % k, c2, n2, r2, None, kd)))
        self._proj_units = []
        if self.bilinear:
            for k, u in enumerate(ups, start=1):
                conv = u.conv3d if u.dim == 3 else u.conv2d
                self._proj_units.append(_Unit("up%d.proj" % k, UNet2D5_dsbn._Conv1x1(conv), None, None, None, 1))

    class _HeadConv(object):

        def __init__(self, out_conv):
            self.src = out_conv
            self.weight = None
            self.bias = None
            self.in_channels, self.out_channels = out_conv.in_channels, 16
            self.seen = None

        def sync(self, force):
            w = self.src.weight
            if self.weight is None or self.weight.device != w.device:
                self.weight = torch.zeros((16,) + tuple(w.shape[1:]), dtype=torch.float32, device=w.device)
                self.bias = torch.zeros(16, dtype=torch.float32, device=w.device)
                force = True
            ver = (w._version, self.src.bias._version)
            if force or ver != self.seen:
                k = w.shape[0]
                self.weight[:k].copy_(w.detach())
                self.bias[:k].copy_(self.src.bias.detach())
                self.seen = ver

    class _Conv1x1(object):

        def __init__(self, conv):
            self.src = conv
            self.weight = None
            self.in_channels, self.out_channels = conv.in_channels, conv.out_channels
            self.seen = None

        @property
        def bias(self):
            return self.src.bias

        def sync(self, force):
            w = self.src.weight
            co, ci = w.shape[0], w.shape[1]
            if self.weight is None or self.weight.device != w.device:
                self.weight = torch.zeros((co, ci, 1, 3, 3), dtype=torch.float32, device=w.device)
                force = True
            if force or w._version != self.seen:
                self.weight[:, :, 0, 1, 1].copy_(w.detach().reshape(co, ci))
                self.seen = w._version

    class _StemConv(object):

        def __init__(self, conv):
            self.src = conv
            self.weight = None
            self.seen = None
            self.image = None

        def sync(self, force):
            w = self.src.weight
            co = w.shape[0]
            if self.weight is None or self.weight.device != w.device:
                self.weight = torch.zeros((co, 48, 3), dtype=torch.float32, device=w.device)
                self.image = torch.empty(48 * 3 * co, dtype=torch.bfloat16, device=w.device)
                force = True
            if force or w._version != self.seen:
                wk = w.detach()[:, 0].reshape(co, 3, 9).permute(0, 2, 1)
                hi = wk.to(torch.bfloat16).float()
                self.weight[:, 0:9, :].copy_(hi)
                self.weight[:, 16:25, :].copy_(hi)
                self.weight[:, 32:41, :].copy_(wk - hi)
                call("fpl_conv3d_k311_prep_weight", ptr(self.weight), 48, co, ptr(self.image), stream_ptr())
                self.seen = w._version

    def _stem_tc(self, depth):
        u = self._down_units[0][0]
        return (u.cin == 1 and u.kd == 3 and depth >= 2 and u.cout in (16, 32, 64) and ops.is_sm100()
                and _conv_impl() == "tc" and os.environ.get("FPL_STEM_IMPL", "tc") == "tc")

    def _stem_direct(self, geo):
        u = self._down_units[0][0]
        d, h, w = geo
        return (u.cin == 1 and u.kd == 3 and u.cout == 16 and w >= 32 and h >= 4 and ops.is_sm100()
                and _conv_impl() == "tc" and os.environ.get("FPL_STEM_TRAIN", "direct") == "direct")

    def _head_cc(self, n, d):
        return (self.ft_chns[0] in (16, 32) and self.n_class <= 8 and d >= 2 and n * d <= 65535 and ops.is_sm100()
                and os.environ.get("FPL_HEAD_IMPL", "cc") == "cc" and os.environ.get("FPL_CONV_IMPL", "tc") == "tc")

    def _head_tc(self):
        return self._use_tc(self.ft_chns[0], 16) and self.n_class <= 8 and os.environ.get("FPL_HEAD_IMPL", "tc") == "tc"

    def _grad_params(self, domain):
        out = [self.out_conv.weight, self.out_conv.bias]
        ups = [self.up1, self.up2, self.up3, self.up4]

        def unit_params(u):
            bn = u.dsbn.bns[domain]
            return [u.conv.weight, u.conv.bias, bn.weight, bn.bias, u.prelu.weight]

        for k in (3, 2, 1, 0):
            u1, u2 = self._up_units[k]
            out += unit_params(u2) + unit_params(u1)
            if self.bilinear:
                t = ups[k].conv3d if ups[k].dim == 3 else ups[k].conv2d
            else:
                t = ups[k].trans3d if ups[k].dim == 3 else ups[k].trans2d
            out += [t.weight, t.bias]
        for i in (4, 3, 2, 1, 0):
            u1, u2 = self._down_units[i]
            out += unit_params(u2) + unit_params(u1)
        return out

    def forward_mc(self, x, domain_label, repeats, graph_lane=0):
        if torch.is_grad_enabled() and any(p.requires_grad for p in self.parameters()):
            raise RuntimeError("forward_mc is an inference call: wrap it in torch.no_grad()")
        if not 1 <= repeats <= self.kMaxMcRepeats:
            raise ValueError("repeats must be in [1, %d]" % self.kMaxMcRepeats)
        if repeats == 1:
            return [self.forward(x, domain_label, graph_lane)]
        return self.forward(x, domain_label, graph_lane, _repeats=repeats)

    def forward(self, x, domain_label=None, graph_lane=0, _repeats=1):
        if domain_label is None:
            raise ValueError("UNet2D5_dsbn.forward needs domain_label")
        if x.dim() != 5:
            raise ValueError('expected 5D input (got {}D input)'.format(x.dim()))
        if not x.is_cuda:
            raise RuntimeError("fplplus_b200.UNet2D5_dsbn runs on CUDA (sm_100a) only; got a %s tensor" % x.device)
        if self.bilinear and not all(self._use_tc(u.cin, u.cout) for u in self._proj_units):
            raise NotImplementedError("bilinear=True needs feature_chns that are multiples of 16 (tensor-core 1x1 projection)")
        domain = int(domain_label[0])
        if not 0 <= domain < self.num_domains:
            raise IndexError("domain_label %d out of range" % domain)
        x = x.float().contiguous()
        params = self._grad_params(domain)
        need_grad = torch.is_grad_enabled() and any(p.requires_grad for p in params)
        if need_grad:
            return _UNetFunction.apply(self, domain, x, *params)
        if self.cuda_graphs and not torch.cuda.is_current_stream_capturing():
            return self._forward_graphed(x, domain, graph_lane, _repeats)
        ws = self._infer_ws
        if ws is None or ws.device != x.device:
            ws = self._infer_ws = _Workspace(x.device)
        logits, _ = self._run_forward(x, domain, ws, _repeats)
        return logits

    def _mode_signature(self, domain):
        sig = [self.training]
        for u1, u2 in self._down_units + self._up_units:
            for u in (u1, u2):
                sig.append(u.dsbn.bns[domain].training)
                if u.dropout is not None:
                    sig.append(u.dropout.training and u.dropout.p > 0.0)
        return tuple(sig)

    kMaxMcRepeats = 16

    def ensure_rng(self, device, lane=0):
        t = self._rng_lanes.get(lane)
        if t is None or t.device != torch.device(device):
            t = self._rng_lanes[lane] = torch.zeros(self.kMaxMcRepeats, dtype=torch.int64, device=device)
        if lane == 0:
            self._rng_dev = t
        return t

    def _draw_seed(self):
        return int(torch.empty((), dtype=torch.int64).random_().item()) & ((1 << 62) - 1)

    def _forward_graphed(self, x, domain, lane=0, repeats=1):
        key = (tuple(x.shape), domain, x.device.index, self._mode_signature(domain), lane, repeats)
        ent = self._graphs.get(key)
        if ent is None:
            self._graphs[key] = ent = {"graph": None, "calls": 0}
        ent["calls"] += 1
        if ent["graph"] is None and ent["calls"] < 2:
            ws = self._infer_wss.get(lane)
            if ws is None or ws.device != x.device:
                ws = self._infer_wss[lane] = _Workspace(x.device)
            logits, _ = self._run_forward(x, domain, ws, repeats)
            return logits
        rng = self.ensure_rng(x.device, lane)
        self._note_depths(self._geometry(x.shape))
        self._refresh_weight_images(with_dgrad=False)
        if ent["graph"] is None:
            if len(self._graphs) > 24:
                for k in [k for k in self._graphs if k != key][:8]:
                    del self._graphs[k]
            ent["x"] = x.clone()
            ent["ws"] = _Workspace(x.device)
            g = torch.cuda.CUDAGraph()
            self._seed_from_device, self._cur_lane = True, lane
            try:
                with torch.cuda.graph(g):
                    ent["out"], _ = self._run_forward(ent["x"], domain, ent["ws"], repeats)
            finally:
                self._seed_from_device, self._cur_lane = False, 0
            ent["graph"] = g
        ent["x"].copy_(x, non_blocking=True)
        if any(key[3][1:]) and self._dropout_masks is None:
            if repeats == 1:
                rng[0:1].fill_(self._draw_seed())
            else:
                for k in range(repeats):
                    rng[k:k + 1].fill_(self._draw_seed())
        ent["graph"].replay()
        if repeats > 1:
            return [o.clone() for o in ent["out"]]
        return ent["out"].clone()

    def _geometry(self, shape):
        n, c, d, h, w = shape
        if c != self.in_chns:
            raise ValueError("expected %d input channels, got %d" % (self.in_chns, c))
        geo = [(d, h, w)]
        for i in range(4):
            d, h, w = geo[-1]
            kd = 2 if self.dims[i] == 3 else 1
            if d % kd or h % 2 or w % 2:
                raise ValueError("input size %s is not divisible by the down-sampling factors" % (tuple(shape[2:]),))
            geo.append((d // kd, h // 2, w // 2))
        return geo

    def _use_tc(self, cin, cout):
        return _conv_impl() == "tc" and cin % 16 == 0 and cout % 16 == 0 and ops.is_sm100()

    def invalidate_weight_images(self):
        for ent in self._img_cache.values():
            ent[0] = -1
        self._head_dirty = True
        self._stem_dirty = True

    def prepare_inference(self, shape):
        self._note_depths(self._geometry(tuple(shape)))
        self._refresh_weight_images(with_dgrad=False)

    def _tc_convs(self):
        out = []
        for u1, u2 in self._down_units + self._up_units:
            for u in (u1, u2):
                if not u.is_stem and self._use_tc(u.cin, u.cout):
                    out.append(u)
        for u in self._proj_units:
            u.conv.sync(self._head_dirty)
            out.append(u)
        if self._head_tc():
            if self._head_unit is None:
                self._head_unit = _Unit("head", self._head, None, None, None, 1)
            self._head.sync(self._head_dirty)
            out.append(self._head_unit)
        self._head_dirty = False
        return out

    def _refresh_weight_images(self, with_dgrad):
        lib = ops._lib.load()
        if self._stem_tc(self._unit_depth.get("block0.conv#1", 0)) and not (with_dgrad and self._stem_direct(self._geo0)):
            if self._stem is None:
                self._stem = UNet2D5_dsbn._StemConv(self._down_units[0][0].conv)
            self._stem.sync(self._stem_dirty)
            self._stem_dirty = False
        todo, todo_df, todo_ct = [], [], []
        for u in self._tc_convs():
            w = u.conv.weight
            depth = self._unit_depth.get(u.name, 0)
            for transpose in ((False, True) if with_dgrad else (False,)):
                if transpose and not self._use_tc(u.cout, u.cin):
                    continue
                if u.name != "head" and self._dfold_ok(u.cout if transpose else u.cin, u.cin if transpose else u.cout,
                                                       u.kd, depth):
                    if not (transpose and u.name == "block0.conv#1"):
                        self._dfold_image(u.conv, transpose, todo_df)
                    continue
                key = (id(w), transpose)
                ent = self._img_cache.get(key)
                if ent is None or ent[1].device != w.device:
                    nbytes = lib.fpl_conv3d_weight_image_bytes(u.cout if transpose else u.cin,
                                                               u.cin if transpose else u.cout, u.kd)
                    ent = self._img_cache[key] = [-1, torch.empty(nbytes // 2, dtype=torch.bfloat16, device=w.device)]
                if ent[0] != w._version:
                    todo.append((w, u.cin, u.cout, u.kd, 1 if transpose else 0, ent))
        if os.environ.get("FPL_CONVT_IMPL", "tc") == "tc":
            for up in (self.up1, self.up2, self.up3, self.up4):
                trans = up.trans3d if up.dim == 3 else up.trans2d
                if self._use_tc(trans.weight.shape[0], trans.weight.shape[1]):
                    kd2 = 2 if up.dim == 3 else 1
                    self._convt_image(trans, kd2, 0, todo_ct)
                    if with_dgrad:
                        self._convt_image(trans, kd2, 1, todo_ct)
        for i in range(0, len(todo_df), 64):
            part = todo_df[i:i + 64]
            n = len(part)
            arr_w = (ctypes.c_void_p * n)(*[t[0].data_ptr() for t in part])
            arr_img = (ctypes.c_void_p * n)(*[t[4][1].data_ptr() for t in part])
            ints = [(ctypes.c_int * n)(*[t[k] for t in part]) for k in (1, 2, 3)]
            call("fpl_conv3d_dfold_prep_weight_batch", n, arr_w, ints[0], ints[1], ints[2], arr_img, stream_ptr())
            for t in part:
                t[4][0] = t[0]._version
        if todo_ct:
            n = len(todo_ct)
            arr_w = (ctypes.c_void_p * n)(*[t[0].data_ptr() for t in todo_ct])
            arr_img = (ctypes.c_void_p * n)(*[t[5][1].data_ptr() for t in todo_ct])
            ints = [(ctypes.c_int * n)(*[t[k] for t in todo_ct]) for k in (1, 2, 3, 4)]
            call("fpl_convt_prep_weight_batch", n, arr_w, ints[0], ints[1], ints[2], ints[3], arr_img, stream_ptr())
            for t in todo_ct:
                t[5][0] = t[0]._version
        for i in range(0, len(todo), 80):
            part = todo[i:i + 80]
            n = len(part)
            arr_w = (ctypes.c_void_p * n)(*[t[0].data_ptr() for t in part])
            arr_img = (ctypes.c_void_p * n)(*[t[5][1].data_ptr() for t in part])
            ints = [(ctypes.c_int * n)(*[t[k] for t in part]) for k in (1, 2, 3, 4)]
            call("fpl_conv3d_prep_weight_batch", n, arr_w, ints[0], ints[1], ints[2], ints[3], arr_img, stream_ptr())
            for t in part:
                t[5][0] = t[0]._version

    def _note_depths(self, geo):
        self._geo0 = tuple(geo[0])
        for i in range(5):
            for u in self._down_units[i]:
                self._unit_depth[u.name] = geo[i][0]
        for k, lvl in zip(range(4), (3, 2, 1, 0)):
            for u in self._up_units[k]:
                self._unit_depth[u.name] = geo[lvl][0]

    def _dfold_ok(self, cin, cout, kd, depth):
        if kd != 3 or depth < 2 or not self._use_tc(cin, cout) or os.environ.get("FPL_DFOLD", "1") == "0":
            return False
        key = (cin, cout)
        ok = self._dfold_cache.get(key)
        if ok is None:
            ok = self._dfold_cache[key] = ops._lib.load().fpl_conv3d_dfold_image_bytes(cin, cout) > 0
        return ok

    def _dfold_image(self, conv, transpose, defer=None):
        w = conv.weight
        key = (id(w), "df%d" % (1 if transpose else 0))
        ent = self._img_cache.get(key)
        cin, cout = conv.in_channels, conv.out_channels
        if ent is None or ent[1].device != w.device:
            nbytes = ops._lib.load().fpl_conv3d_dfold_image_bytes(cout if transpose else cin, cin if transpose else cout)
            ent = self._img_cache[key] = [-1, torch.empty(nbytes // 2, dtype=torch.bfloat16, device=w.device)]
        if ent[0] != w._version:
            if defer is not None:
                defer.append((w, cin, cout, 1 if transpose else 0, ent))
            else:
                call("fpl_conv3d_dfold_prep_weight", ptr(w), cin, cout, 1 if transpose else 0, ptr(ent[1]), stream_ptr())
                ent[0] = w._version
        return ent[1]

    def _convt_tc(self, cin, cout):
        return (self._use_tc(cin, cout) and os.environ.get("FPL_CONVT_IMPL", "tc") == "tc")

    def _convt_image(self, trans, kd2, mode, defer=None):
        w = trans.weight
        key = (id(w), "ct%d" % mode)
        ent = self._img_cache.get(key)
        if ent is None or ent[1].device != w.device:
            nbytes = ops._lib.load().fpl_convt_weight_image_bytes(w.shape[0], w.shape[1], kd2)
            ent = self._img_cache[key] = [-1, torch.empty(nbytes // 2, dtype=torch.bfloat16, device=w.device)]
        if ent[0] != w._version:
            if defer is not None:
                defer.append((w, w.shape[0], w.shape[1], kd2, mode, ent))
            else:
                call("fpl_convt_prep_weight", ptr(w), w.shape[0], w.shape[1], kd2, mode, ptr(ent[1]), stream_ptr())
                ent[0] = w._version
        return ent[1]

    def _weight_image(self, conv, kd, transpose, ws):
        ent = self._img_cache.get((id(conv.weight), transpose))
        if ent is None or ent[0] != conv.weight._version:
            self._refresh_weight_images(with_dgrad=transpose)
            ent = self._img_cache[(id(conv.weight), transpose)]
        return ent[1]

    def _conv_fwd(self, u, xin, x_img, y, stats, n, geo, ws):
        d, h, w = geo
        st = stream_ptr()
        if u.is_stem and self._stem_tc(d) and not (self._grad_pass and self._stem_direct(geo)):
            xs = ws.c8("XS:stem", n, d, 32, h, w)
            call("fpl_patch9_c8", ptr(x_img), ptr(xs), 1, n, d, h, w, st)
            call("fpl_conv3d_tc_k311", ptr(xs), 4, 0, ptr(self._stem.image), ptr(u.conv.bias), ptr(y), y.shape[2], 0,
                 ptr(stats), n, d, h, w, 48, u.cout, 32, st)
        elif u.is_stem:
            call("fpl_stem_conv_fwd", ptr(x_img), ptr(u.conv.weight), ptr(u.conv.bias), ptr(y), y.shape[2], 0,
                 ptr(stats), n, u.cin, d, h, w, u.cout, u.kd, st)
        elif self._dfold_ok(u.cin, u.cout, u.kd, d):
            call("fpl_conv3d_tc_dfold", *xin.args(), ptr(self._dfold_image(u.conv, False)), ptr(u.conv.bias), ptr(y),
                 y.shape[2], 0, ptr(stats), n, d, h, w, u.cin, u.cout, st)
        elif self._use_tc(u.cin, u.cout):
            img = self._weight_image(u.conv, u.kd, False, ws)
            call("fpl_conv3d_tc", *xin.args(), ptr(img), ptr(u.conv.bias), ptr(y), y.shape[2], 0, ptr(stats),
                 n, d, h, w, u.cin, u.cout, u.kd, st)
        else:
            call("fpl_conv3d_direct", *xin.args(), ptr(u.conv.weight), ptr(u.conv.bias), ptr(y), y.shape[2], 0,
                 ptr(stats), n, d, h, w, u.cin, u.cout, u.kd, 0, 0, st)

    def _eval_affine_refresh(self, domain, ws):
        units = [u for pair in self._down_units + self._up_units for u in pair if not u.dsbn.bns[domain].training]
        if not units or os.environ.get("FPL_EVAL_FUSE", "1") == "0" or not ops.is_sm100():
            return {}
        key = "eval_affine:%d" % domain
        total = sum(2 * u.cout for u in units)
        buf = ws.get(key, (total,), torch.float32)
        out, o = {}, 0
        for u in units:
            out[u.name] = (buf[o:o + u.cout], buf[o + u.cout:o + 2 * u.cout])
            o += 2 * u.cout
        m = len(units)
        bns = [u.dsbn.bns[domain] for u in units]
        arr = lambda ts: (ctypes.c_void_p * m)(*[t.data_ptr() for t in ts])
        call("fpl_dsbn_eval_affine_batch", m, arr([b.weight for b in bns]), arr([b.bias for b in bns]),
             arr([b.running_mean for b in bns]), arr([b.running_var for b in bns]), arr([u.conv.bias for u in units]),
             arr([out[u.name][0] for u in units]), arr([out[u.name][1] for u in units]),
             (ctypes.c_int * m)(*[u.cout for u in units]), float(bns[0].eps), stream_ptr())
        return out

    def _unit_fwd_fused(self, u, xin, x_img, out, aff, p, seed, offset, seed_dev, n, geo, ws):
        d, h, w = geo
        st = stream_ptr()
        scale, shift = aff
        if u.is_stem:
            if not self._stem_tc(d) or p > 0.0:
                return False
            xs = ws.c8("XS:stem", n, d, 32, h, w)
            call("fpl_patch9_c8", ptr(x_img), ptr(xs), 1, n, d, h, w, st)
            call("fpl_conv3d_tc_k311_act", ptr(xs), 4, 0, ptr(self._stem.image), *out.args(), n, d, h, w, 48, u.cout, 32,
                 ptr(scale), ptr(shift), ptr(u.prelu.weight), st)
            return True
        if self._dfold_ok(u.cin, u.cout, u.kd, d):
            if p > 0.0:
                return False
            call("fpl_conv3d_tc_dfold_act", *xin.args(), ptr(self._dfold_image(u.conv, False)), *out.args(), n, d, h, w,
                 u.cin, u.cout, ptr(scale), ptr(shift), ptr(u.prelu.weight), st)
            return True
        if self._use_tc(u.cin, u.cout):
            img = self._weight_image(u.conv, u.kd, False, ws)
            call("fpl_conv3d_tc_act", *xin.args(), ptr(img), *out.args(), n, d, h, w, u.cin, u.cout, u.kd, ptr(scale),
                 ptr(shift), ptr(u.prelu.weight), p, seed, offset, ptr(seed_dev) if p > 0.0 else None, st)
            return True
        return False

    def _unit_fwd(self, u, domain, xin, x_img, out, pooled, pool_idx, pool_kd, n, geo, ws, small, rec):
        d, h, w = geo
        c = u.cout
        aff = rec["eval_affine"].get(u.name)
        if aff is not None:
            p, seed, offset = 0.0, 0, 0
            drop = u.dropout is not None and u.dropout.training and u.dropout.p > 0.0
            explicit = drop and self._dropout_masks is not None and u.name in self._dropout_masks
            if not explicit:
                if drop:
                    p, seed, offset = float(u.dropout.p), rec["seed"], rec["next_offset"]
                if self._unit_fwd_fused(u, xin, x_img, out, aff, p, seed, offset, rec["seed_dev"], n, geo, ws):
                    if drop:
                        rec["next_offset"] += 2 * n * d * (c // 8) * h * w
                    if pooled is not None:
                        call("fpl_maxpool_c8", *out.args(), *pooled.args(), pool_kd, n, d, h, w, c, stream_ptr())
                    return
        y = ws.c8("Y:" + u.name, n, d, c, h, w)
        stats = small.f64(2 * c)
        self._conv_fwd(u, xin, x_img, y, stats, n, geo, ws)
        bn = u.dsbn.bns[domain]
        if bn.weight.dtype != torch.float32:
            raise RuntimeError("fplplus_b200 supports tensor_type=float only")
        scale, shift, mean, invstd = small.f32(c), small.f32(c), small.f32(c), small.f32(c)
        training = 1 if bn.training else 0
        p, mask, seed, offset = 0.0, None, 0, 0
        if u.dropout is not None and u.dropout.training and u.dropout.p > 0.0:
            p = float(u.dropout.p)
            if self._dropout_masks is not None and u.name in self._dropout_masks:
                mask = self._dropout_masks[u.name]
            else:
                seed, offset = rec["seed"], rec["next_offset"]
                rec["next_offset"] += 2 * n * d * (c // 8) * h * w
        pv = pooled.args() if pooled is not None else (None, 0, 0)
        call("fpl_dsbn_bn_act_fwd", ptr(y), ptr(stats), n * d * h * w, ptr(bn.weight), ptr(bn.bias),
             ptr(bn.running_mean), ptr(bn.running_var), ptr(bn.num_batches_tracked), float(bn.momentum), float(bn.eps),
             training, ptr(scale), ptr(shift), ptr(mean), ptr(invstd), ptr(u.prelu.weight), *out.args(), *pv,
             ptr(pool_idx), pool_kd, p, ptr(mask), seed, offset, ptr(rec["seed_dev"]) if p > 0.0 and mask is None else None,
             n, d, h, w, c, stream_ptr())
        rec[u.name] = dict(y=y, xin=xin, scale=scale, shift=shift, mean=mean, invstd=invstd, training=training,
                           p=p, mask=mask, seed=seed, offset=offset, geo=geo, bn=bn,
                           seed_dev=rec["seed_dev"] if p > 0.0 and mask is None else None,
                           stem_direct=u.is_stem and self._grad_pass and self._stem_direct(geo))

    def _first_dropout_level(self):
        for i in range(5):
            dr = self._down_units[i][0].dropout
            if dr is not None and dr.training and dr.p > 0.0:
                return i
        return 5

    def _run_forward(self, x, domain, ws, repeats=1):
        n = x.shape[0]
        geo = self._geometry(x.shape)
        ft = self.ft_chns
        small = _SmallPool(ws, "fwd", x.device)
        self._note_depths(geo)
        self._refresh_weight_images(with_dgrad=self._grad_pass)
        if self._seed_from_device:
            seed, seed_dev = 0, self.ensure_rng(x.device, self._cur_lane)
        else:
            seed, seed_dev = self._draw_seed(), None
        rec = {"seed": seed, "seed_dev": seed_dev, "next_offset": 0, "geo": geo, "n": n, "x": x}
        rec["eval_affine"] = {} if self._grad_pass else self._eval_affine_refresh(domain, ws)
        if repeats > 1:
            assert not torch.is_grad_enabled()
            seeds = [(seed, seed_dev if seed_dev is None else seed_dev[0:1])]
            for k in range(1, repeats):
                seeds.append((0, seed_dev[k:k + 1]) if self._seed_from_device else (self._draw_seed(), None))
            split = self._first_dropout_level()
            cur = None
            for i in range(split):
                cur = self._down_level(i, domain, cur, x, n, geo, ws, small, rec)
            outs = []
            for k in range(repeats):
                rec["seed"], rec["seed_dev"] = seeds[k]
                rec["next_offset"] = 0
                c2 = cur
                for i in range(split, 5):
                    c2 = self._down_level(i, domain, c2, x, n, geo, ws, small, rec)
                outs.append(self._up_path_and_head(c2, domain, x, n, geo, ws, small, rec)[0])
            return outs, rec
        cur = None
        for i in range(5):
            cur = self._down_level(i, domain, cur, x, n, geo, ws, small, rec)
        return self._up_path_and_head(cur, domain, x, n, geo, ws, small, rec)

    def _down_level(self, i, domain, cur, x, n, geo, ws, small, rec):
        ft = self.ft_chns
        u1, u2 = self._down_units[i]
        d, h, w = geo[i]
        c = ft[i]
        a1 = C8(ws.c8("A1:block%d" % i, n, d, c, h, w))
        self._unit_fwd(u1, domain, cur, x, a1, None, None, 0, n, geo[i], ws, small, rec)
        if i < 4:
            cat = ws.c8("cat%d" % i, n, d, 2 * c, h, w)
            d2, h2, w2 = geo[i + 1]
            pooled = C8(ws.c8("P%d" % i, n, d2, c, h2, w2))
            idx = ws.get("idx%d" % i, (n, d2, c // 8, h2, w2, 8), torch.uint8)
            pool_kd = 2 if self.dims[i] == 3 else 1
            self._unit_fwd(u2, domain, a1, None, C8(cat, 0, c), pooled, idx, pool_kd, n, geo[i], ws, small, rec)
            rec["idx%d" % i] = (idx, pool_kd)
            cur = pooled
        else:
            a2 = C8(ws.c8("A2:block4", n, d, c, h, w))
            self._unit_fwd(u2, domain, a1, None, a2, None, None, 0, n, geo[i], ws, small, rec)
            cur = a2
        return cur

    def _up_path_and_head(self, low, domain, x, n, geo, ws, small, rec):
        ft = self.ft_chns
        ups = [self.up1, self.up2, self.up3, self.up4]
        for k, lvl in zip(range(4), (3, 2, 1, 0)):
            up = ups[k]
            u1, u2 = self._up_units[k]
            d, h, w = geo[lvl]
            dl, hl, wl = geo[lvl + 1]
            c, c_low = ft[lvl], ft[lvl + 1]
            cat = ws.t["cat%d" % lvl]
            trans = up.trans3d if up.dim == 3 else up.trans2d
            kd2 = 2 if up.dim == 3 else 1
            if self.bilinear:
                pu = self._proj_units[k]
                t_low = ws.c8("T:up%d" % (k + 1), n, dl, c, hl, wl)
                call("fpl_conv3d_tc", *low.args(), ptr(self._weight_image(pu.conv, 1, False, ws)), ptr(pu.conv.bias), ptr(t_low),
                     c // 8, 0, None, n, dl, hl, wl, c_low, c, 1, stream_ptr())
                call("fpl_upsample2x_c8", ptr(t_low), c // 8, 0, ptr(cat), 2 * c // 8, c // 8, n, dl, hl, wl, c, kd2,
                     stream_ptr())
            elif self._convt_tc(c_low, c):
                call("fpl_convt_k2s2_fwd_tc", *low.args(), ptr(self._convt_image(trans, kd2, 0)), ptr(trans.bias), ptr(cat),
                     2 * c // 8, c // 8, n, dl, hl, wl, c_low, c, kd2, stream_ptr())
            else:
                call("fpl_convt_k2s2_fwd", *low.args(), ptr(trans.weight), ptr(trans.bias), ptr(cat), 2 * c // 8, c // 8,
                     n, dl, hl, wl, c_low, c, kd2, stream_ptr())
            rec["up%d.low" % (k + 1)] = low
            a1 = C8(ws.c8("A1:up%d" % (k + 1), n, d, c, h, w))
            self._unit_fwd(u1, domain, C8(cat, 0, 2 * c), None, a1, None, None, 0, n, geo[lvl], ws, small, rec)
            a2 = C8(ws.c8("A2:up%d" % (k + 1), n, d, c, h, w))
            self._unit_fwd(u2, domain, a1, None, a2, None, None, 0, n, geo[lvl], ws, small, rec)
            low = a2
        d, h, w = geo[0]
        logits = torch.empty((n, self.n_class, d, h, w), dtype=torch.float32, device=x.device)
        if self._head_cc(n, d):
            call("fpl_head_fwd", *low.args(), ptr(self.out_conv.weight), ptr(self.out_conv.bias), ptr(logits), n, d, h, w,
                 ft[0], self.n_class, stream_ptr())
        elif self._head_tc():
            img = self._weight_image(self._head, 1, False, ws)
            call("fpl_head_conv_tc", *low.args(), ptr(img), ptr(self._head.bias), ptr(logits), n, d, h, w, ft[0],
                 self.n_class, stream_ptr())
        else:
            call("fpl_head_conv_fwd", *low.args(), ptr(self.out_conv.weight), ptr(self.out_conv.bias), ptr(logits),
                 n, d, h, w, ft[0], self.n_class, stream_ptr())
        rec["head_in"] = low
        return logits, rec

    def _bwdred_ok(self, u_prev, r_prev):
        return (u_prev is not None and r_prev.get("mask") is None and os.environ.get("FPL_BWD_FUSE", "0") != "0"
                and ops.is_sm100())

    def _unit_bwd(self, u, r, g1, g_pool, pool_idx, pool_kd, n, ws, small, grads, need_dx, fold=None, prev=None):
        d, h, w = r["geo"]
        c = u.cout
        st = stream_ptr()
        g1a = g1.args() if g1 is not None else (None, 0, 0)
        gpa = g_pool.args() if g_pool is not None else (None, 0, 0)
        common = (ptr(r["y"]), *g1a, *gpa, ptr(pool_idx), pool_kd, ptr(r["scale"]), ptr(r["shift"]), ptr(r["mean"]),
                  ptr(r["invstd"]), ptr(u.prelu.weight), r["p"], ptr(r["mask"]), r["seed"], r["offset"], ptr(r["seed_dev"]))
        red = r.pop("red_fused", None)
        if red is None:
            red = small.f64(2 * c + 1)
            call("fpl_dsbn_act_bwd_reduce", *common, ptr(red), n, d, h, w, c, st)
        dy = ws.c8("dY:" + u.name, n, d, c, h, w)
        bn = r["bn"]
        call("fpl_dsbn_act_bwd_apply_fin", *common, ptr(red), r["training"], ptr(dy), n, d, h, w, c, st,
             ptr(grads[bn.weight]), ptr(grads[bn.bias]), ptr(grads[u.prelu.weight]), ptr(grads[u.conv.bias]))
        dw = grads[u.conv.weight]
        if u.is_stem and r.get("stem_direct"):
            call("fpl_stem_conv_wgrad", ptr(r["x_img"]), ptr(dy), c // 8, 0, ptr(dw), n, u.cin, d, h, w, c, u.kd, st)
            return None
        if u.is_stem and self._stem_tc(d):
            xs = ws.c8("XS:stem", n, d, 32, h, w)
            dw16 = ws.get("dW16s", (c, 16, 3), torch.float32)
            dw16.zero_()
            call("fpl_conv3d_wgrad_tc_k311", ptr(xs), 4, 0, ptr(dy), c // 8, 0, ptr(dw16), n, d, h, w, 16, c, st)
            dw.view(c, 1, 3, 3, 3).add_(dw16[:, :9, :].permute(0, 2, 1).reshape(c, 1, 3, 3, 3))
            return None
        if u.is_stem:
            if self._use_tc(16, c) and u.cin <= 8 and os.environ.get("FPL_WGRAD_IMPL", "tc") == "tc":
                x8 = ws.c8("X8", n, d, 8, h, w)
                call("fpl_pack_ncdhw_to_c8", ptr(r["x_img"]), u.cin, ptr(x8), 1, 0, 1, None, n, d, h, w, st)
                dw8 = ws.get("dW8", (c, 8, u.kd, 3, 3), torch.float32)
                dw8.zero_()
                call("fpl_conv3d_wgrad_tc", ptr(x8), 1, 0, ptr(dy), c // 8, 0, ptr(dw8), n, d, h, w, 8, c, u.kd, st)
                dw.view(c, u.cin, u.kd, 3, 3).add_(dw8[:, :u.cin])
            else:
                call("fpl_stem_conv_wgrad", ptr(r["x_img"]), ptr(dy), c // 8, 0, ptr(dw), n, u.cin, d, h, w, c, u.kd, st)
            return None
        xin = r["xin"]
        aux = self._aux_stream()
        if aux is not None:
            cur = torch.cuda.current_stream()
            ready = torch.cuda.Event()
            ready.record(cur)
            aux.wait_event(ready)
            with torch.cuda.stream(aux):
                self._wgrad(u, xin, dy, dw, n, d, h, w, fold)
        else:
            self._wgrad(u, xin, dy, dw, n, d, h, w, fold)
        if not need_dx:
            return None
        dx = ws.c8("dX:" + u.name, n, d, u.cin, h, w)
        br = None
        if prev is not None and self._bwdred_ok(*prev) and (self._dfold_ok(u.cout, u.cin, u.kd, d) or self._use_tc(u.cout, u.cin)):
            up, rp = prev
            rp["red_fused"] = small.f64(2 * up.cout + 1)
            br = (ptr(rp["y"]), ptr(rp["scale"]), ptr(rp["shift"]), ptr(rp["mean"]), ptr(rp["invstd"]), ptr(up.prelu.weight),
                  rp["p"], rp["seed"], rp["offset"], ptr(rp["seed_dev"]), ptr(rp["red_fused"]))
        if self._dfold_ok(u.cout, u.cin, u.kd, d):
            if br is not None:
                call("fpl_conv3d_tc_dfold_bwdred", ptr(dy), c // 8, 0, ptr(self._dfold_image(u.conv, True)), ptr(dx),
                     u.cin // 8, 0, n, d, h, w, c, u.cin, *br, st)
            else:
                call("fpl_conv3d_tc_dfold", ptr(dy), c // 8, 0, ptr(self._dfold_image(u.conv, True)), None, ptr(dx),
                     u.cin // 8, 0, None, n, d, h, w, c, u.cin, st)
        elif self._use_tc(u.cout, u.cin):
            img = self._weight_image(u.conv, u.kd, True, ws)
            if br is not None:
                call("fpl_conv3d_tc_bwdred", ptr(dy), c // 8, 0, ptr(img), ptr(dx), u.cin // 8, 0, n, d, h, w, c, u.cin,
                     u.kd, *br, st)
            else:
                call("fpl_conv3d_tc", ptr(dy), c // 8, 0, ptr(img), None, ptr(dx), u.cin // 8, 0, None,
                     n, d, h, w, c, u.cin, u.kd, st)
        else:
            call("fpl_conv3d_direct", ptr(dy), c // 8, 0, ptr(u.conv.weight), None, ptr(dx), u.cin // 8, 0, None,
                 n, d, h, w, c, u.cin, u.kd, 1, 0, st)
        return C8(dx)

    def _aux_stream(self):
        if not self.wgrad_side_stream:
            return None
        cur = torch.cuda.current_stream()
        key = cur.cuda_stream
        st = self._aux_streams.get(key)
        if st is None:
            st = self._aux_streams[key] = torch.cuda.Stream(device=cur.device)
        return st

    def _join_aux(self):
        aux = self._aux_stream()
        if aux is not None:
            torch.cuda.current_stream().wait_stream(aux)

    def _wgrad(self, u, xin, dy, dw, n, d, h, w, fold=None):
        impl = os.environ.get("FPL_WGRAD_IMPL", "tc")
        if impl == "tc" and u.cin % 8 == 0 and u.cout % 16 == 0 and ops.is_sm100():
            if fold is not None:
                scr = fold["alloc"](u.cout * u.cin * u.kd * 9)
                call("fpl_conv3d_wgrad_tc_tapmajor", *xin.args(), ptr(dy), u.cout // 8, 0, ptr(scr), n, d, h, w, u.cin,
                     u.cout, u.kd, stream_ptr())
                fold["pending"].append((scr, dw, u.cout, u.cin, u.kd * 9))
                return
            call("fpl_conv3d_wgrad_tc", *xin.args(), ptr(dy), u.cout // 8, 0, ptr(dw), n, d, h, w, u.cin, u.cout,
                 u.kd, stream_ptr())
        else:
            call("fpl_conv3d_wgrad", *xin.args(), ptr(dy), u.cout // 8, 0, ptr(dw), n, d, h, w, u.cin, u.cout, u.kd,
                 stream_ptr())

    def _run_backward(self, rec, dlogits, domain, ws):
        n, geo, ft = rec["n"], rec["geo"], self.ft_chns
        params = self._grad_params(domain)
        sizes = [(p.numel() + 3) // 4 * 4 for p in params]
        flat = torch.zeros(sum(sizes), dtype=torch.float32, device=dlogits.device)
        grads, offs, o = {}, [], 0
        for p, s in zip(params, sizes):
            grads[p] = flat[o:o + p.numel()]
            offs.append(o)
            o += s
        fired = [0]
        fold = None
        if os.environ.get("FPL_WGRAD_TAPMAJOR", "1") != "0" and ops.is_sm100():
            total = sum((u.conv.weight.numel() + 3) // 4 * 4 for pair in self._down_units + self._up_units for u in pair
                        if not u.is_stem) + 16 * self.ft_chns[0] * 9 + sum(
                            (t.weight.numel() + 3) // 4 * 4 for up in (self.up1, self.up2, self.up3, self.up4)
                            for t in (up.trans3d, up.trans2d) if t is not None) + sum(
                            9 * u.cin * u.cout for u in self._proj_units)
            scratch = ws.get("wgrad_scratch", (total,), torch.float32)
            aux0 = self._aux_stream()
            if aux0 is not None:
                cur0 = torch.cuda.current_stream()
                aux0.wait_stream(cur0)
                with torch.cuda.stream(aux0):
                    scratch.zero_()
                scratch_zeroed = torch.cuda.Event()
                scratch_zeroed.record(aux0)
            else:
                scratch.zero_()
                scratch_zeroed = None
            cursor = [0]

            def alloc(numel):
                t = scratch[cursor[0]:cursor[0] + numel]
                cursor[0] += (numel + 3) // 4 * 4
                return t
            fold = {"alloc": alloc, "pending": []}

        def flush_fold():
            if fold is None or not fold["pending"]:
                return
            self._join_aux()
            part = fold["pending"]
            m = len(part)
            arr_s = (ctypes.c_void_p * m)(*[t[0].data_ptr() for t in part])
            arr_d = (ctypes.c_void_p * m)(*[t[1].data_ptr() for t in part])
            ints = [(ctypes.c_int * m)(*[t[k] for t in part]) for k in (2, 3, 4)]
            scout = (ctypes.c_int * m)(*[t[5] if len(t) > 5 else t[2] for t in part])
            call("fpl_wgrad_tapmajor_to_dw_batch", m, arr_s, arr_d, ints[0], ints[1], ints[2], scout, stream_ptr())
            fold["pending"] = []

        def fire(n_params_done):
            if self.grad_ready_hook is not None:
                end = offs[n_params_done - 1] + sizes[n_params_done - 1]
                last = n_params_done == len(params)
                pending_b, remaining_b = (end - fired[0]) * 4, (len(flat) - end) * 4
                if end > fired[0] and (last or pending_b >= self.grad_bucket_bytes
                                       or (remaining_b <= self.grad_tail_bytes and pending_b >= (1 << 20))):
                    flush_fold()
                    self._join_aux()
                    self.grad_ready_hook(flat, fired[0], end, n_params_done == len(params))
                    fired[0] = end

        small = _SmallPool(ws, "bwd", dlogits.device)
        st = stream_ptr()
        d, h, w = geo[0]
        head_in = rec["head_in"]

        def scratch_ready():
            if fold is not None and scratch_zeroed is not None:
                torch.cuda.current_stream().wait_event(scratch_zeroed)
        g = C8(ws.c8("dX:head", n, d, ft[0], h, w))
        dlogits = dlogits.contiguous()
        if self._head_cc(n, d):
            k = self.n_class
            dl8 = ws.c8("dL8", n, d, 8, h, w)
            call("fpl_head_dgrad", ptr(dlogits), ptr(self.out_conv.weight), *g.args(), ptr(dl8), 1, 0,
                 ptr(grads[self.out_conv.bias]), n, d, h, w, ft[0], k, st)
            scratch_ready()
            if fold is not None:
                scr = fold["alloc"](8 * ft[0] * 9)
                call("fpl_conv3d_wgrad_tc_tapmajor", *head_in.args(), ptr(dl8), 1, 0, ptr(scr), n, d, h, w, ft[0], 8, 1, st)
                fold["pending"].append((scr, grads[self.out_conv.weight], k, ft[0], 9, 8))
            else:
                dw8 = ws.get("dW16", (8, ft[0], 1, 3, 3), torch.float32)
                dw8.zero_()
                call("fpl_conv3d_wgrad_tc", *head_in.args(), ptr(dl8), 1, 0, ptr(dw8), n, d, h, w, ft[0], 8, 1, st)
                grads[self.out_conv.weight].view(k, ft[0], 1, 3, 3).add_(dw8[:k])
        elif self._head_tc():
            k = self.n_class
            dl16 = ws.c8("dL16", n, d, 16, h, w)
            call("fpl_pack_ncdhw_to_c8", ptr(dlogits), k, ptr(dl16), 2, 0, 2, ptr(grads[self.out_conv.bias]), n, d, h, w, st)
            img_t = self._weight_image(self._head, 1, True, ws)
            call("fpl_conv3d_tc", ptr(dl16), 2, 0, ptr(img_t), None, *g.args(), None, n, d, h, w, 16, ft[0], 1, st)
            co = 8 if (ft[0] <= 32 and d >= 2) else 16
            scratch_ready()
            if fold is not None:
                scr = fold["alloc"](co * ft[0] * 9)
                call("fpl_conv3d_wgrad_tc_tapmajor", *head_in.args(), ptr(dl16), 2, 0, ptr(scr), n, d, h, w, ft[0], co, 1, st)
                fold["pending"].append((scr, grads[self.out_conv.weight], k, ft[0], 9, co))
            else:
                dw16 = ws.get("dW16", (co, ft[0], 1, 3, 3), torch.float32)
                dw16.zero_()
                call("fpl_conv3d_wgrad_tc", *head_in.args(), ptr(dl16), 2, 0, ptr(dw16), n, d, h, w, ft[0], co, 1, st)
                grads[self.out_conv.weight].view(k, ft[0], 1, 3, 3).add_(dw16[:k])
        else:
            call("fpl_head_conv_bwd", *head_in.args(), ptr(self.out_conv.weight), ptr(dlogits), *g.args(),
                 ptr(grads[self.out_conv.weight]), ptr(grads[self.out_conv.bias]), n, d, h, w, ft[0], self.n_class, st)
        scratch_ready()
        ups = [self.up1, self.up2, self.up3, self.up4]
        skip_grads = {}
        done = 2
        fire(done)
        for k, lvl in zip((3, 2, 1, 0), (0, 1, 2, 3)):
            u1, u2 = self._up_units[k]
            up = ups[k]
            c, c_low = ft[lvl], ft[lvl + 1]
            r1 = rec[u1.name]
            g = self._unit_bwd(u2, rec[u2.name], g, None, None, 0, n, ws, small, grads, True, fold, prev=(u1, r1))
            dcat = self._unit_bwd(u1, r1, g, None, None, 0, n, ws, small, grads, True, fold)
            skip_grads[lvl] = C8(dcat.buf, 0, c)
            trans = up.trans3d if up.dim == 3 else up.trans2d
            kd2 = 2 if up.dim == 3 else 1
            dl, hl, wl = geo[lvl + 1]
            low = rec["up%d.low" % (k + 1)]
            glow = C8(ws.c8("dlow%d" % lvl, n, dl, c_low, hl, wl))
            if self.bilinear:
                pu = self._proj_units[k]
                proj = up.conv3d if up.dim == 3 else up.conv2d
                g_t = ws.c8("dT:up%d" % (k + 1), n, dl, c, hl, wl)
                call("fpl_upsample2x_c8_bwd", ptr(dcat.buf), 2 * c // 8, c // 8, ptr(g_t), c // 8, 0, n, dl, hl, wl, c, kd2, st)
                call("fpl_channel_sum_c8", ptr(g_t), c // 8, 0, ptr(grads[proj.bias]), n, dl, hl, wl, c, st)
                if fold is not None:
                    scr = fold["alloc"](9 * c * c_low)
                    call("fpl_conv3d_wgrad_tc_tapmajor", *low.args(), ptr(g_t), c // 8, 0, ptr(scr), n, dl, hl, wl, c_low, c, 1, st)
                    fold["pending"].append((scr[4 * c * c_low:5 * c * c_low], grads[proj.weight], c, c_low, 1))
                else:
                    dw9 = ws.get("dW9:up%d" % (k + 1), (c, c_low, 1, 3, 3), torch.float32)
                    dw9.zero_()
                    call("fpl_conv3d_wgrad_tc", *low.args(), ptr(g_t), c // 8, 0, ptr(dw9), n, dl, hl, wl, c_low, c, 1, st)
                    grads[proj.weight].view(c, c_low).add_(dw9[:, :, 0, 1, 1])
                call("fpl_conv3d_tc", ptr(g_t), c // 8, 0, ptr(self._weight_image(pu.conv, 1, True, ws)), None, *glow.args(),
                     None, n, dl, hl, wl, c, c_low, 1, st)
            elif self._convt_tc(c_low, c):
                call("fpl_convt_k2s2_dgrad_tc", ptr(dcat.buf), 2 * c // 8, c // 8, ptr(self._convt_image(trans, kd2, 1)),
                     *glow.args(), n, dl, hl, wl, c_low, c, kd2, st)
                if fold is not None:
                    scr = fold["alloc"](c_low * c * 4 * kd2)
                    call("fpl_convt_k2s2_wgrad_tc_tapmajor", *low.args(), ptr(dcat.buf), 2 * c // 8, c // 8, ptr(scr),
                         n, dl, hl, wl, c_low, c, kd2, st)
                    fold["pending"].append((scr, grads[trans.weight], c, c_low, -4 * kd2))
                else:
                    call("fpl_convt_k2s2_wgrad_tc", *low.args(), ptr(dcat.buf), 2 * c // 8, c // 8, ptr(grads[trans.weight]),
                         n, dl, hl, wl, c_low, c, kd2, st)
                call("fpl_convt_k2s2_bwd", *low.args(), ptr(trans.weight), ptr(dcat.buf), 2 * c // 8, c // 8, None, 0, 0,
                     None, ptr(grads[trans.bias]), n, dl, hl, wl, c_low, c, kd2, st)
            else:
                call("fpl_convt_k2s2_bwd", *low.args(), ptr(trans.weight), ptr(dcat.buf), 2 * c // 8, c // 8, *glow.args(),
                     ptr(grads[trans.weight]), ptr(grads[trans.bias]), n, dl, hl, wl, c_low, c, kd2, st)
            g = glow
            done += 12
            fire(done)
        g_pool = None
        for i in (4, 3, 2, 1, 0):
            u1, u2 = self._down_units[i]
            r1 = rec[u1.name]
            if i == 4:
                g = self._unit_bwd(u2, rec[u2.name], g, None, None, 0, n, ws, small, grads, True, fold, prev=(u1, r1))
            else:
                idx, pool_kd = rec["idx%d" % i]
                g = self._unit_bwd(u2, rec[u2.name], skip_grads[i], g_pool, idx, pool_kd, n, ws, small, grads, True, fold,
                                   prev=(u1, r1))
            r1["x_img"] = rec["x"]
            if i > 0:
                g_pool = self._unit_bwd(u1, r1, g, None, None, 0, n, ws, small, grads, True, fold)
            else:
                self._unit_bwd(u1, r1, g, None, None, 0, n, ws, small, grads, False, fold)
            done += 10
            fire(done)
        assert done == len(params)
        flush_fold()
        self._join_aux()
        return self._deliver_grads(params, offs, flat, grads)

    def _master_grads(self, device):
        m = self._master
        if m is None or m["buf"].device != device:
            order, off, o = [], {}, 0
            for d in range(self.num_domains):
                for p in self._grad_params(d):
                    if p not in off:
                        off[p] = o
                        order.append(p)
                        o += (p.numel() + 3) // 4 * 4
            m = self._master = {"buf": torch.zeros(o, dtype=torch.float32, device=device), "off": off, "tables": {},
                                "event": None}
        return m

    def _deliver_grads(self, params, offs, flat, grads):
        views = [grads[p].view(p.shape) for p in params]
        if os.environ.get("FPL_GRAD_DIRECT", "1") == "0":
            return views
        m = self._master_grads(flat.device)
        base, off = m["buf"].data_ptr(), m["off"]
        if any(p.grad is not None and p.grad.data_ptr() != base + 4 * off[p] for p in params):
            return views
        if self.grad_wait_hook is not None:
            self.grad_wait_hook()
        cur = torch.cuda.current_stream()
        capturing = torch.cuda.is_current_stream_capturing()
        if self.out_conv.weight.grad is None:
            m["buf"].zero_()
            m["event"] = torch.cuda.Event()
            m["event"].record(cur)
            m["event_captured"] = capturing
        elif m["event"] is not None and m.get("event_captured", False) == capturing:
            cur.wait_event(m["event"])
        key = tuple(id(p) for p in params)
        tab = m["tables"].get(key)
        if tab is None:
            rows = [[so, off[p], p.numel()] for p, so in zip(params, offs)]
            tab = m["tables"][key] = (torch.tensor(rows, dtype=torch.int32, device=flat.device),
                                      max(p.numel() for p in params))
        call("fpl_grad_scatter_add", ptr(m["buf"]), ptr(flat), ptr(tab[0]), len(params), tab[1], stream_ptr())
        for p in params:
            if p.grad is None:
                p.grad = m["buf"][off[p]:off[p] + p.numel()].view(p.shape)
        return [None] * len(params)


class _SmallPool(object):

    def __init__(self, ws, tag, device, n32=1 << 16, n64=1 << 15):
        self.b32 = ws.get("small32:" + tag, (n32,), torch.float32)
        self.b64 = ws.get("small64:" + tag, (n64,), torch.float64)
        self.b32.zero_()
        self.b64.zero_()
        self.o32 = self.o64 = 0

    def f32(self, n):
        n4 = (n + 3) // 4 * 4
        t = self.b32[self.o32:self.o32 + n]
        self.o32 += n4
        assert self.o32 <= self.b32.numel()
        return t

    def f64(self, n):
        n2 = (n + 1) // 2 * 2
        t = self.b64[self.o64:self.o64 + n]
        self.o64 += n2
        assert self.o64 <= self.b64.numel()
        return t


class _UNetFunction(torch.autograd.Function):
    @staticmethod
    def forward(ctx, net, domain, x, *params):
        if torch.cuda.is_current_stream_capturing():
            ws, home = _Workspace(x.device), net._graph_ws_keep
        else:
            ws, home = (net._pool.pop() if net._pool else _Workspace(x.device)), net._pool
            if ws.device != x.device:
                ws = _Workspace(x.device)
        net._grad_pass = True
        try:
            logits, rec = net._run_forward(x, domain, ws)
        finally:
            net._grad_pass = False
        ctx.net, ctx.domain, ctx.rec = net, domain, rec
        ctx.lease = _Lease(home, ws)
        return logits

    @staticmethod
    def backward(ctx, dlogits):
        net = ctx.net
        grads = net._run_backward(ctx.rec, dlogits, ctx.domain, ctx.lease.ws)
        ctx.rec = None
        return (None, None, None) + tuple(grads)
```

include/fplplus_b200.h:

```cpp
#ifndef FPLPLUS_B200_H
#define FPLPLUS_B200_H

#include <stdint.h>

#ifdef __cplusplus
extern "C" {
#endif

const char* fpl_last_error(void);
int fpl_version(void);
int fpl_set_sm_budget(int sms);
long long fpl_launch_count(int reset);
int fpl_device_is_sm100(void);
void fpl_debug_set(int key, long long value);


int64_t fpl_conv3d_weight_image_bytes(int cin, int cout, int kd);
int fpl_conv3d_prep_weight(const float* w, int cin, int cout, int kd, int transpose_flip,
                           void* image, void* stream);
int fpl_conv3d_prep_weight_batch(int count, const float* const* h_w, const int* h_cin, const int* h_cout,
                                 const int* h_kd, const int* h_transpose_flip, void* const* h_images, void* stream);
int fpl_conv3d_tc(const void* x, int x_c8tot, int x_c8off, const void* image, const float* bias,
                  void* y, int y_c8tot, int y_c8off, double* stats,
                  int n, int d, int h, int w, int cin, int cout, int kd, void* stream);
int64_t fpl_conv3d_dfold_image_bytes(int cin, int cout);
int fpl_conv3d_dfold_prep_weight(const float* w, int cin, int cout, int transpose_flip, void* image, void* stream);
int fpl_conv3d_dfold_prep_weight_batch(int count, const float* const* h_w, const int* h_cin, const int* h_cout,
                                       const int* h_transpose_flip, void* const* h_images, void* stream);
int fpl_conv3d_tc_dfold(const void* x, int x_c8tot, int x_c8off, const void* image, const float* bias,
                        void* y, int y_c8tot, int y_c8off, double* stats,
                        int n, int d, int h, int w, int cin, int cout, void* stream);
int fpl_patch9_c8(const float* x, void* out, int split_hi_lo, int n, int d, int h, int w, void* stream);
int fpl_conv3d_k311_prep_weight(const float* w, int cin, int cout, void* image, void* stream);
int fpl_conv3d_tc_k311(const void* x, int x_c8tot, int x_c8off, const void* image, const float* bias,
                       void* y, int y_c8tot, int y_c8off, double* stats,
                       int n, int d, int h, int w, int cin, int cout, int a_channels, void* stream);
int fpl_conv3d_wgrad_tc_k311(const void* x, int x_c8tot, int x_c8off, const void* dy, int dy_c8tot, int dy_c8off,
                             float* dw, int n, int d, int h, int w, int cin, int cout, void* stream);
int fpl_conv3d_direct(const void* x, int x_c8tot, int x_c8off, const float* w, const float* bias,
                      void* y, int y_c8tot, int y_c8off, double* stats,
                      int n, int d, int h, int w_, int cin, int cout, int kd,
                      int transpose_flip, int round_w_bf16, void* stream);
int fpl_conv3d_wgrad(const void* x, int x_c8tot, int x_c8off, const void* dy, int dy_c8tot, int dy_c8off,
                     float* dw, int n, int d, int h, int w, int cin, int cout, int kd, void* stream);

int fpl_conv3d_wgrad_tc(const void* x, int x_c8tot, int x_c8off, const void* dy, int dy_c8tot, int dy_c8off,
                        float* dw, int n, int d, int h, int w, int cin, int cout, int kd, void* stream);

int fpl_conv3d_wgrad_tc_tapmajor(const void* x, int x_c8tot, int x_c8off, const void* dy, int dy_c8tot, int dy_c8off,
                                 float* scratch, int n, int d, int h, int w, int cin, int cout, int kd, void* stream);
int fpl_wgrad_tapmajor_to_dw_batch(int count, const float* const* h_scratch, float* const* h_dw, const int* h_cout,
                                   const int* h_cin, const int* h_taps, const int* h_scratch_cout, void* stream);

int fpl_grad_scatter_add(float* dst, const float* src, const int* d_table, int segments, int max_numel, void* stream);

int fpl_conv3d_tc_bwdred(const void* x, int x_c8tot, int x_c8off, const void* image, void* y, int y_c8tot, int y_c8off,
                         int n, int d, int h, int w, int cin, int cout, int kd, const void* y_prev,
                         const float* scale, const float* shift, const float* mean, const float* invstd,
                         const float* slope, float drop_p, uint64_t seed, uint64_t offset, const uint64_t* seed_dev,
                         double* red, void* stream);
int fpl_conv3d_tc_dfold_bwdred(const void* x, int x_c8tot, int x_c8off, const void* image, void* y, int y_c8tot,
                               int y_c8off, int n, int d, int h, int w, int cin, int cout, const void* y_prev,
                               const float* scale, const float* shift, const float* mean, const float* invstd,
                               const float* slope, float drop_p, uint64_t seed, uint64_t offset,
                               const uint64_t* seed_dev, double* red, void* stream);

int fpl_gather_patches(const void* d_rows, int n, int c, int pd, int ph, int pw, float* out_image,
                       uint8_t* out_label, uint8_t* out_code, void* stream);

int fpl_adam_multi_tensor(const void* d_segs, int nseg, const int* d_chunks, int nchunks, const float* lr_dev,
                          double lr_host, double beta1, double beta2, double eps, double weight_decay,
                          unsigned int* d_done_counter, void* stream);
int fpl_adam_chunk_elems(void);

int fpl_dsbn_eval_affine_batch(int count, const float* const* h_gamma, const float* const* h_beta,
                               const float* const* h_running_mean, const float* const* h_running_var,
                               const float* const* h_conv_bias, float* const* h_scale, float* const* h_shift,
                               const int* h_c, float eps, void* stream);
int fpl_conv3d_tc_act(const void* x, int x_c8tot, int x_c8off, const void* image, void* a, int a_c8tot, int a_c8off,
                      int n, int d, int h, int w, int cin, int cout, int kd, const float* scale, const float* shift,
                      const float* slope, float drop_p, uint64_t seed, uint64_t offset, const uint64_t* seed_dev,
                      void* stream);
int fpl_conv3d_tc_dfold_act(const void* x, int x_c8tot, int x_c8off, const void* image, void* a, int a_c8tot, int a_c8off,
                            int n, int d, int h, int w, int cin, int cout, const float* scale, const float* shift,
                            const float* slope, void* stream);
int fpl_conv3d_tc_k311_act(const void* x, int x_c8tot, int x_c8off, const void* image, void* a, int a_c8tot, int a_c8off,
                           int n, int d, int h, int w, int cin, int cout, int a_channels, const float* scale,
                           const float* shift, const float* slope, void* stream);

int fpl_maxpool_c8(const void* a, int a_c8tot, int a_c8off, void* pooled, int p_c8tot, int p_c8off, int pool_kd,
                   int n, int d, int h, int w, int c, void* stream);

int fpl_head_fwd(const void* x, int x_c8tot, int x_c8off, const float* w, const float* bias, float* logits, int n, int d,
                 int h, int w_, int cin, int classes, void* stream);
int fpl_head_dgrad(const float* dlogits, const float* w, void* g, int g_c8tot, int g_c8off, void* dl8, int dl_c8tot,
                   int dl_c8off, float* dbias, int n, int d, int h, int w_, int cin, int classes, void* stream);

int fpl_upsample2x_c8(const void* x, int x_c8tot, int x_c8off, void* y, int y_c8tot, int y_c8off, int n, int d, int h, int w,
                      int c, int kd2, void* stream);
int fpl_upsample2x_c8_bwd(const void* gy, int gy_c8tot, int gy_c8off, void* gx, int gx_c8tot, int gx_c8off, int n, int d,
                          int h, int w, int c, int kd2, void* stream);
int fpl_channel_sum_c8(const void* g, int g_c8tot, int g_c8off, float* out, int n, int d, int h, int w, int c, void* stream);

int fpl_stem_conv_fwd(const float* x, const float* w, const float* bias, void* y, int y_c8tot, int y_c8off,
                      double* stats, int n, int cin, int d, int h, int w_, int cout, int kd, void* stream);
int fpl_stem_conv_wgrad(const float* x, const void* dy, int dy_c8tot, int dy_c8off, float* dw,
                        int n, int cin, int d, int h, int w_, int cout, int kd, void* stream);
int fpl_head_conv_fwd(const void* x, int x_c8tot, int x_c8off, const float* w, const float* bias,
                      float* logits, int n, int d, int h, int w_, int cin, int classes, void* stream);
int fpl_head_conv_tc(const void* x, int x_c8tot, int x_c8off, const void* image16, const float* bias16,
                     float* logits, int n, int d, int h, int w, int cin, int classes, void* stream);
int fpl_pack_ncdhw_to_c8(const float* x, int c, void* out, int out_c8tot, int out_c8off, int groups,
                         float* chan_sum, int n, int d, int h, int w, void* stream);
int fpl_head_conv_bwd(const void* x, int x_c8tot, int x_c8off, const float* w, const float* dlogits,
                      void* dx, int dx_c8tot, int dx_c8off, float* dw, float* db,
                      int n, int d, int h, int w_, int cin, int classes, void* stream);

int fpl_convt_k2s2_fwd(const void* x, int x_c8tot, int x_c8off, const float* w, const float* bias,
                       void* y, int y_c8tot, int y_c8off, int n, int d, int h, int w_, int cin, int cout,
                       int kd2, void* stream);
int fpl_convt_k2s2_bwd(const void* x, int x_c8tot, int x_c8off, const float* w,
                       const void* dy, int dy_c8tot, int dy_c8off,
                       void* dx, int dx_c8tot, int dx_c8off, float* dw, float* db,
                       int n, int d, int h, int w_, int cin, int cout, int kd2, void* stream);

int64_t fpl_convt_weight_image_bytes(int cin, int cout, int kd2);
int fpl_convt_prep_weight(const float* w, int cin, int cout, int kd2, int mode, void* image, void* stream);
int fpl_convt_prep_weight_batch(int count, const float* const* h_w, const int* h_cin, const int* h_cout,
                                const int* h_kd2, const int* h_mode, void* const* h_images, void* stream);
int fpl_convt_k2s2_fwd_tc(const void* x, int x_c8tot, int x_c8off, const void* image, const float* bias, void* y,
                          int y_c8tot, int y_c8off, int n, int d, int h, int w, int cin, int cout, int kd2, void* stream);
int fpl_convt_k2s2_dgrad_tc(const void* dy, int dy_c8tot, int dy_c8off, const void* image_t, void* dx, int dx_c8tot,
                            int dx_c8off, int n, int d, int h, int w, int cin, int cout, int kd2, void* stream);
int fpl_convt_k2s2_wgrad_tc(const void* x, int x_c8tot, int x_c8off, const void* dy, int dy_c8tot, int dy_c8off,
                            float* dw, int n, int d, int h, int w, int cin, int cout, int kd2, void* stream);
int fpl_convt_k2s2_wgrad_tc_tapmajor(const void* x, int x_c8tot, int x_c8off, const void* dy, int dy_c8tot, int dy_c8off,
                                     float* scratch, int n, int d, int h, int w, int cin, int cout, int kd2, void* stream);


int fpl_dsbn_finalize(const double* stats, int64_t count, const float* gamma, const float* beta,
                      float* running_mean, float* running_var, int64_t* num_batches_tracked,
                      float momentum, float eps, int training,
                      float* scale, float* shift, float* save_mean, float* save_invstd, int c, void* stream);
int fpl_dsbn_act_fwd(const void* y, const float* scale, const float* shift, const float* slope,
                     void* a, int a_c8tot, int a_c8off,
                     void* pooled, int p_c8tot, int p_c8off, uint8_t* pool_idx, int pool_kd,
                     float drop_p, const uint8_t* drop_mask, uint64_t seed, uint64_t offset, const uint64_t* seed_dev,
                     int n, int d, int h, int w, int c, void* stream);
int fpl_dsbn_bn_act_fwd(const void* y, const double* stats, int64_t count, const float* gamma, const float* beta,
                        float* running_mean, float* running_var, int64_t* num_batches_tracked, float momentum,
                        float eps, int training, float* scale, float* shift, float* save_mean, float* save_invstd,
                        const float* slope, void* a, int a_c8tot, int a_c8off, void* pooled, int p_c8tot, int p_c8off,
                        uint8_t* pool_idx, int pool_kd, float drop_p, const uint8_t* drop_mask, uint64_t seed,
                        uint64_t offset, const uint64_t* seed_dev, int n, int d, int h, int w, int c, void* stream);
int fpl_dsbn_act_bwd_reduce(const void* y, const void* g1, int g1_c8tot, int g1_c8off,
                            const void* g_pool, int gp_c8tot, int gp_c8off, const uint8_t* pool_idx, int pool_kd,
                            const float* scale, const float* shift, const float* save_mean,
                            const float* save_invstd, const float* slope,
                            float drop_p, const uint8_t* drop_mask, uint64_t seed, uint64_t offset,
                            const uint64_t* seed_dev, double* red, int n, int d, int h, int w, int c, void* stream);
int fpl_dsbn_act_bwd_apply(const void* y, const void* g1, int g1_c8tot, int g1_c8off,
                           const void* g_pool, int gp_c8tot, int gp_c8off, const uint8_t* pool_idx, int pool_kd,
                           const float* scale, const float* shift, const float* save_mean,
                           const float* save_invstd, const float* slope,
                           float drop_p, const uint8_t* drop_mask, uint64_t seed, uint64_t offset,
                           const uint64_t* seed_dev, const double* red, int training, void* dy,
                           int n, int d, int h, int w, int c, void* stream);
int fpl_dsbn_act_bwd_apply_fin(const void* y, const void* g1, int g1_c8tot, int g1_c8off,
                               const void* g_pool, int gp_c8tot, int gp_c8off, const uint8_t* pool_idx, int pool_kd,
                               const float* scale, const float* shift, const float* save_mean,
                               const float* save_invstd, const float* slope,
                               float drop_p, const uint8_t* drop_mask, uint64_t seed, uint64_t offset,
                               const uint64_t* seed_dev, const double* red, int training, void* dy,
                               int n, int d, int h, int w, int c, void* stream,
                               float* dgamma, float* dbeta, float* dslope, float* dbias_conv);
int fpl_dsbn_bwd_finalize(const double* red, const float* scale, const float* save_invstd, int training,
                          float* dgamma, float* dbeta, float* dslope, float* dbias_conv, int c, void* stream);


int fpl_dice_ce_reduce(const float* logits, const float* soft_y, const float* weight,
                       double* sums, int n, int c, int64_t spatial, void* stream);
int fpl_dice_ce_grad(const float* logits, const float* soft_y, const float* weight,
                     const double* sums, float w_dice, float w_ce, float grad_scale,
                     const float* grad_scale_dev, float* loss, float* dlogits,
                     int n, int c, int64_t spatial, void* stream);
int fpl_dice_ce_reduce_ex(const float* logits, const float* soft_y, const uint8_t* label, const float* weight,
                          const uint8_t* weight_code, const float* image_weight, double* sums, int n, int c,
                          int64_t spatial, int want_entropy, int prob_input, void* stream);
int fpl_dice_ce_grad_ex(const float* logits, const float* soft_y, const uint8_t* label, const float* weight,
                        const uint8_t* weight_code, const float* image_weight, const double* sums,
                        float w_dice, float w_ce, float w_entropy, float grad_scale, const float* grad_scale_dev,
                        float* loss, float* dlogits, int n, int c, int64_t spatial, int prob_input, int n_global,
                        void* stream);
int fpl_dice_ce_loss_ex(const float* logits, const float* soft_y, const uint8_t* label, const float* weight,
                        const uint8_t* weight_code, const float* image_weight, const double* sums,
                        float w_dice, float w_ce, float w_entropy, float* loss, double* hard_dice, int n, int c,
                        int64_t spatial, int prob_input, int n_global, void* stream);


int fpl_argmax_label(const float* logits, uint8_t* label, int b, int c, int64_t spatial, void* stream);
int fpl_mc_uncertainty(const float* const* h_logits_k, int k, int c, int64_t spatial,
                       double* out, float* uncertainty_map, void* stream);
int fpl_mc_uncertainty_max_passes(void);
int fpl_agree_weight(const float* logits_tgt, const float* logits_src, uint8_t* label_tgt, uint8_t* label_src,
                     float* weight, int fold_image_weight, float image_weight, long long* out_count,
                     int c, int64_t spatial, void* stream);


int fpl_window_accumulate(const float* patch, float* out, float* count, int b, int c,
                          int vd, int vh, int vw, int d0, int h0, int w0, int pd, int ph, int pw,
                          int flip_h, int flip_w, float scale, void* stream);
int fpl_window_normalize(float* out, const float* count, float scale, int64_t numel, void* stream);

#ifdef __cplusplus
}
#endif
#endif
```

Measured before the change: 1.008 billion.

## Batch small-layer weight-gradient convs into one grouped persistent kernel

Adds a grouped wgrad kernel that handles several small-resolution conv and ConvT weight-gradient layers in a single launch. Work items from all layers are spread over a fixed set of CTAs using a cost-balanced item list. The aim is to cut launch overhead and fill the GPU at deep decoder levels, where each layer alone launches too few CTAs. It also moves the shared tile configuration code into a common header. The cost is extra host-side planning, a large kernel parameter block, and layers queued until a flush point.

```diff
diff --git a/fpl-plus_b200/build.py b/fpl-plus_b200/build.py
--- a/fpl-plus_b200/build.py
+++ b/fpl-plus_b200/build.py
@@ -6,7 +6,7 @@
 HERE = os.path.dirname(os.path.abspath(__file__))
 CSRC = os.path.join(HERE, "csrc")
 LIB = os.path.join(HERE, "libfplplus_b200.so")
-SOURCES = ["api.cu", "dsbn.cu", "loss.cu", "filter.cu", "conv_direct.cu", "conv_tc.cu", "conv_wgrad_tc.cu", "conv_wgrad_hs.cu", "convt_tc.cu", "conv_tc_dfold.cu", "grad.cu", "adam.cu", "datapath.cu", "head.cu", "head_tc.cu", "stem_tc.cu", "upsample.cu"]
+SOURCES = ["api.cu", "dsbn.cu", "loss.cu", "filter.cu", "conv_direct.cu", "conv_tc.cu", "conv_wgrad_tc.cu", "conv_wgrad_group.cu", "conv_wgrad_hs.cu", "convt_tc.cu", "conv_tc_dfold.cu", "grad.cu", "adam.cu", "datapath.cu", "head.cu", "head_tc.cu", "stem_tc.cu", "upsample.cu"]
 NVCC_FLAGS = ["-gencode", "arch=compute_100a,code=sm_100a", "-lineinfo", "-O3", "-std=c++17",
               "-Xcompiler", "-fPIC", "--use_fast_math=false"]
 
diff --git a/fpl-plus_b200/csrc/conv_wgrad_group.cu b/fpl-plus_b200/csrc/conv_wgrad_group.cu
--- /dev/null
+++ b/fpl-plus_b200/csrc/conv_wgrad_group.cu
@@ -0,0 +1,418 @@
+#include "common.cuh"
+#include "tc_ptx.cuh"
+#include "wgrad_cfg.cuh"
+#include "../../include/fplplus_b200.h"
+
+#include <algorithm>
+#include <cmath>
+#include <cstring>
+#include <vector>
+
+namespace {
+
+constexpr int kGroupMax = FPL_WGRAD_GROUP_MAX;
+constexpr int kGroupItems = 1024;
+constexpr int kGroupCtas = 160;
+constexpr int kThreadsG = 192;
+constexpr int kMaxStagesG = 8;
+constexpr int kSmemBudgetG = 220 * 1024;
+
+struct GwLayer {
+    float* dw;
+    int kind;
+    int N, D, H, W, cin, cout;
+    int x_c8tot, x_c8off, dy_c8tot, dy_c8off;
+    int kd;
+    int ntaps;
+    int th, tw, nkd, c8chunk;
+    int mtiles_c, mtiles_kd, m, nb, nchunks, ndy, ncols, dplanes;
+    int plane_x, plane_dy;
+    int dy_off, tx_bytes;
+    int tiles_h, tiles_w, tiles_total, split;
+};
+
+struct GwParams {
+    CUtensorMap xmap[kGroupMax];
+    CUtensorMap dymap[kGroupMax];
+    GwLayer L[kGroupMax];
+    int stage_bytes, stages, tmem_cols;
+    uint16_t cta_begin[kGroupCtas + 1];
+    uint16_t item[kGroupItems];
+};
+
+static_assert(sizeof(GwParams) <= 32764, "kernel parameter limit");
+
+struct GwWork {
+    int layer, mt_kd, mt_c, nc, tile_begin, tile_end;
+};
+
+__device__ __forceinline__ GwWork decode_item(const GwParams& P, int it) {
+    GwWork w;
+    const int code = P.item[it];
+    w.layer = code >> 12;
+    int b = code & 4095;
+    const GwLayer& L = P.L[w.layer];
+    const int slice = b % L.split; b /= L.split;
+    w.nc = b % L.nchunks; b /= L.nchunks;
+    w.mt_c = b % L.mtiles_c;
+    w.mt_kd = b / L.mtiles_c;
+    w.tile_begin = (int)(((int64_t)L.tiles_total * slice) / L.split);
+    w.tile_end = (int)(((int64_t)L.tiles_total * (slice + 1)) / L.split);
+    return w;
+}
+
+__device__ __forceinline__ int warp_uniform(int v) { return __reduce_max_sync(0xffffffffu, v); }
+
+__global__ void __launch_bounds__(kThreadsG) wgrad_group_kernel(const __grid_constant__ GwParams P) {
+    extern __shared__ uint8_t smem_raw[];
+    uint8_t* smem = reinterpret_cast<uint8_t*>((reinterpret_cast<uintptr_t>(smem_raw) + 1023) & ~uintptr_t(1023));
+    uint64_t* bars = reinterpret_cast<uint64_t*>(smem);
+    uint64_t* full_bar = bars;
+    uint64_t* empty_bar = bars + kMaxStagesG;
+    uint64_t* acc_full = bars + 2 * kMaxStagesG;
+    uint64_t* acc_empty = bars + 2 * kMaxStagesG + 1;
+    uint32_t* tmem_slot = reinterpret_cast<uint32_t*>(bars + 2 * kMaxStagesG + 2);
+    uint8_t* ring = smem + 256;
+
+    const int warp = threadIdx.x >> 5, lane = threadIdx.x & 31;
+    const int it_begin = P.cta_begin[blockIdx.x], it_end = P.cta_begin[blockIdx.x + 1];
+
+    if (warp == 0 && lane == 0) {
+        for (int s = 0; s < P.stages; ++s) { mbar_init(&full_bar[s], 1); mbar_init(&empty_bar[s], 1); }
+        mbar_init(acc_full, 1);
+        mbar_init(acc_empty, 4);
+        fence_barrier_init();
+    }
+    if (warp == 1) tmem_alloc(tmem_slot, (uint32_t)P.tmem_cols);
+    FPL_PDL_WAIT();
+    tc_fence_before();
+    __syncthreads();
+    tc_fence_after();
+    const uint32_t tmem_base = *tmem_slot;
+
+    if (warp == 0) {
+        if (lane == 0) {
+            int stage = 0; uint32_t phase = 0;
+            for (int it = it_begin; it < it_end; ++it) {
+                const GwWork wk = decode_item(P, it);
+                const GwLayer& L = P.L[wk.layer];
+                const CUtensorMap* xmap = &P.xmap[wk.layer];
+                const CUtensorMap* dymap = &P.dymap[wk.layer];
+                asm volatile("prefetch.tensormap [%0];" ::"l"(xmap) : "memory");
+                asm volatile("prefetch.tensormap [%0];" ::"l"(dymap) : "memory");
+                for (int t = wk.tile_begin; t < wk.tile_end; ++t) {
+                    mbar_wait(&empty_bar[stage], phase ^ 1);
+                    uint8_t* x_dst = ring + (size_t)stage * P.stage_bytes;
+                    mbar_expect_tx(&full_bar[stage], (uint32_t)L.tx_bytes);
+                    int r = t;
+                    if (L.kind == 0) {
+                        const int dp = r % L.dplanes; r /= L.dplanes;
+                        const int tw_i = r % L.tiles_w; r /= L.tiles_w;
+                        const int th_i = r % L.tiles_h;
+                        const int n = r / L.tiles_h;
+                        const int d = L.ndy * dp;
+                        const int kd0 = L.mtiles_kd > 1 ? wk.mt_kd : 0;
+                        tma_load_5d(x_dst, xmap, &full_bar[stage], 2 * (tw_i * L.tw - 1), th_i * L.th - 1,
+                                    L.x_c8off + wk.mt_c * L.c8chunk, d + kd0 - L.kd / 2, n);
+                        tma_load_5d(x_dst + L.dy_off, dymap, &full_bar[stage], 2 * (tw_i * L.tw), th_i * L.th,
+                                    L.dy_c8off + wk.nc * (L.nb / 8), d, n);
+                    } else {
+                        const int tw_i = r % L.tiles_w; r /= L.tiles_w;
+                        const int th_i = r % L.tiles_h; r /= L.tiles_h;
+                        const int d = r % L.D;
+                        const int n = r / L.D;
+                        tma_load_4d(x_dst, xmap, &full_bar[stage], 0, tw_i * kCtTW, th_i * kCtTH,
+                                    (n * L.D + d) * L.x_c8tot + L.x_c8off + wk.mt_c * L.c8chunk);
+                        for (int tap = 0; tap < L.ntaps; ++tap) {
+                            const int a = L.kd == 2 ? tap >> 2 : 0, bb = (tap >> 1) & 1, c = tap & 1;
+                            tma_load_4d(x_dst + L.dy_off + (size_t)tap * L.plane_dy, dymap, &full_bar[stage], 0,
+                                        2 * tw_i * kCtTW + c, 2 * th_i * kCtTH + bb,
+                                        (n * L.D * L.kd + d * L.kd + a) * L.dy_c8tot + L.dy_c8off + wk.nc * (L.nb / 8));
+                        }
+                    }
+                    if (++stage == P.stages) { stage = 0; phase ^= 1; }
+                }
+            }
+        }
+    } else if (warp == 1) {
+        const uint32_t ring_u = smem_u32(ring);
+        const uint32_t tmem_u = (uint32_t)warp_uniform((int)tmem_base);
+        const bool leader = elect_one();
+        int stage = 0; uint32_t phase = 0, acc_phase = 0;
+        for (int it = it_begin; it < it_end; ++it) {
+            const GwWork wk = decode_item(P, it);
+            const GwLayer& L = P.L[wk.layer];
+            const int kind = warp_uniform(L.kind), ncols = warp_uniform(L.ncols), m = warp_uniform(L.m);
+            const int ntiles = warp_uniform(wk.tile_end - wk.tile_begin);
+            const uint32_t dy_off16 = (uint32_t)warp_uniform(L.dy_off) >> 4;
+            const uint32_t idesc = (1u << 4) | (1u << 7) | (1u << 10) | (1u << 15) | (1u << 16) |
+                                   ((uint32_t)(ncols >> 3) << 17) | ((uint32_t)(m >> 4) << 24);
+            mbar_wait(acc_empty, acc_phase ^ 1);
+            tc_fence_after();
+            uint32_t accumulate = 0;
+            if (kind == 0) {
+                const int th = warp_uniform(L.th), tw = warp_uniform(L.tw);
+                const uint32_t pitch_x = (uint32_t)(tw + 2) * 16, pitch_dy = (uint32_t)tw * 16;
+                const uint64_t a_hi = make_desc(0, pitch_x, (uint32_t)warp_uniform(L.plane_x));
+                const uint64_t b_hi = make_desc(0, pitch_dy, (uint32_t)warp_uniform(L.plane_dy));
+                uint32_t tap_off[9], d_tap[9];
+#pragma unroll
+                for (int t9 = 0; t9 < 9; ++t9) {
+                    tap_off[t9] = ((uint32_t)(t9 / 3) * pitch_x + (uint32_t)(t9 % 3) * 16) >> 4;
+                    d_tap[t9] = tmem_u + (uint32_t)(t9 * ncols);
+                }
+                for (int t = 0; t < ntiles; ++t) {
+                    mbar_wait(&full_bar[stage], phase);
+                    tc_fence_after();
+                    const uint32_t x_base = (ring_u + (uint32_t)stage * (uint32_t)P.stage_bytes) >> 4;
+                    const uint32_t dy_base = x_base + dy_off16;
+                    for (int hp = 0; hp < th / 2; ++hp) {
+                        const uint32_t a_row = x_base + (((uint32_t)(2 * hp) * pitch_x) >> 4);
+                        const uint32_t b_row = dy_base + (((uint32_t)(2 * hp) * pitch_dy) >> 4);
+                        uint64_t bdesc = b_hi + (uint64_t)b_row, a_col = a_hi + (uint64_t)a_row;
+                        for (int j = 0; j < tw / 8; ++j, bdesc += 8, a_col += 8) {
+#pragma unroll
+                            for (int t9 = 0; t9 < 9; ++t9)
+                                if (leader) umma_bf16(d_tap[t9], a_col + (uint64_t)tap_off[t9], bdesc, idesc, accumulate);
+                            accumulate = 1;
+                        }
+                    }
+                    if (leader) umma_commit(&empty_bar[stage]);
+                    __syncwarp();
+                    if (++stage == P.stages) { stage = 0; phase ^= 1; }
+                }
+            } else {
+                const uint64_t hi = make_desc(0, kCtTW * 16, kCtPlane);
+                const int ntaps = warp_uniform(L.ntaps);
+                const uint32_t dy_tile16 = (uint32_t)warp_uniform(L.plane_dy) >> 4;
+                for (int t = 0; t < ntiles; ++t) {
+                    mbar_wait(&full_bar[stage], phase);
+                    tc_fence_after();
+                    const uint32_t x_base = (ring_u + (uint32_t)stage * (uint32_t)P.stage_bytes) >> 4;
+                    const uint32_t dy_base = x_base + dy_off16;
+                    uint64_t adesc = hi + (uint64_t)x_base, b_hp = hi + (uint64_t)dy_base;
+                    for (int hp = 0; hp < kCtTH / 2; ++hp, adesc += 2 * kCtTW * 16 / 16, b_hp += 2 * kCtTW * 16 / 16) {
+                        uint64_t bdesc = b_hp;
+                        uint32_t d_tap = tmem_u;
+                        for (int tap = 0; tap < ntaps; ++tap, bdesc += dy_tile16, d_tap += (uint32_t)ncols) {
+                            if (leader) umma_bf16(d_tap, adesc, bdesc, idesc, accumulate);
+                        }
+                        accumulate = 1;
+                    }
+                    if (leader) umma_commit(&empty_bar[stage]);
+                    __syncwarp();
+                    if (++stage == P.stages) { stage = 0; phase ^= 1; }
+                }
+            }
+            if (leader) umma_commit(acc_full);
+            __syncwarp();
+            acc_phase ^= 1;
+        }
+        FPL_PDL_TRIGGER();
+    } else {
+        const int quarter = warp & 3;
+        const int tlane = quarter * 32 + lane;
+        const uint32_t t_row = tmem_base + ((uint32_t)(quarter * 32) << 16);
+        uint32_t acc_phase = 0;
+        for (int it = it_begin; it < it_end; ++it) {
+            const GwWork wk = decode_item(P, it);
+            const GwLayer& L = P.L[wk.layer];
+            mbar_wait(acc_full, acc_phase);
+            tc_fence_after();
+            const int row = L.m == 128 ? tlane : ((lane < 16) ? quarter * 16 + lane : -1);
+            if (L.kind == 0) {
+                bool valid = row >= 0 && row < L.m;
+                int kdi = 0, ci = 0;
+                if (valid) {
+                    const int g = row >> 3;
+                    valid = g < L.nkd * L.c8chunk;
+                    kdi = (L.mtiles_kd > 1 ? wk.mt_kd : 0) + g / L.c8chunk;
+                    ci = (wk.mt_c * L.c8chunk + g % L.c8chunk) * 8 + (row & 7);
+                }
+                for (int t9 = 0; t9 < 9; ++t9) {
+                    for (int c0 = 0; c0 < L.ncols; c0 += 16) {
+                        uint32_t r[16];
+                        tmem_ld16(t_row + (uint32_t)(t9 * L.ncols + c0), r);
+                        tmem_ld_wait();
+#pragma unroll
+                        for (int half = 0; half < 2; ++half) {
+                            const int col = c0 + 8 * half;
+                            const int dd = L.ndy > 1 ? col / L.nb : 0;
+                            const int kd_tap = kdi - dd;
+                            const int co0 = wk.nc * L.nb + (col - dd * L.nb);
+                            if (!(valid && kd_tap >= 0 && kd_tap < L.kd)) continue;
+                            float* base = L.dw + ((int64_t)(kd_tap * 9 + t9) * L.cout + co0) * L.cin + ci;
+#pragma unroll
+                            for (int i = 0; i < 8; ++i) atomicAdd(base + (int64_t)i * L.cin, __uint_as_float(r[8 * half + i]));
+                        }
+                    }
+                }
+            } else {
+                const int ci = wk.mt_c * L.c8chunk * 8 + row;
+                const bool valid = row >= 0 && row < L.c8chunk * 8 && ci < L.cin;
+                for (int tap = 0; tap < L.ntaps; ++tap) {
+                    for (int c0 = 0; c0 < L.nb; c0 += 16) {
+                        uint32_t r[16];
+                        tmem_ld16(t_row + (uint32_t)(tap * L.nb + c0), r);
+                        tmem_ld_wait();
+                        if (valid) {
+                            float* base = L.dw + ((int64_t)tap * L.cout + wk.nc * L.nb + c0) * L.cin + ci;
+#pragma unroll
+                            for (int i = 0; i < 16; ++i) atomicAdd(base + (int64_t)i * L.cin, __uint_as_float(r[i]));
+                        }
+                    }
+                }
+            }
+            tc_fence_before();
+            __syncwarp();
+            if (lane == 0) mbar_arrive(acc_empty);
+            acc_phase ^= 1;
+        }
+    }
+    tc_fence_before();
+    __syncthreads();
+    if (warp == 1) {
+        tc_fence_after();
+        tmem_dealloc(tmem_base, (uint32_t)P.tmem_cols);
+    }
+}
+
+int mma_cycles(int m, int n) { return std::max(std::max((m + n) / 4, n / 2), 30); }
+
+}
+
+extern "C" int fpl_conv3d_wgrad_group(int count, const int* h_desc, const void* const* h_x, const void* const* h_dy,
+                                      float* const* h_scratch, void* stream) {
+    FPL_REQUIRE(count >= 0 && count <= kGroupMax, "fpl_conv3d_wgrad_group: count %d not in [0,%d]", count, kGroupMax);
+    if (count == 0) return 0;
+    FPL_REQUIRE(h_desc != nullptr && h_x != nullptr && h_dy != nullptr && h_scratch != nullptr,
+                "fpl_conv3d_wgrad_group: NULL host array");
+    EncodeTiledFn encode = nullptr;
+    GwParams P;
+    memset(&P, 0, sizeof(P));
+    std::vector<double> tile_cost(count), epi_cost(count);
+    int max_stage = 0, max_cols = 0;
+    double total = 0.0;
+    for (int l = 0; l < count; ++l) {
+        const int* q = h_desc + FPL_WGRAD_GROUP_DESC * l;
+        const int kind = q[0], n = q[1], d = q[2], h = q[3], w = q[4], cin = q[5], cout = q[6], kd = q[7];
+        const int x_c8tot = q[8], x_c8off = q[9], dy_c8tot = q[10], dy_c8off = q[11];
+        FPL_REQUIRE(kind == 0 || kind == 1, "fpl_conv3d_wgrad_group: layer %d: kind %d must be 0 (conv) or 1 (ConvT)", l, kind);
+        FPL_REQUIRE(n > 0 && d > 0 && h > 0 && w > 0, "fpl_conv3d_wgrad_group: layer %d: empty grid", l);
+        FPL_REQUIRE(cin % 8 == 0 && cout % 16 == 0 && cin > 0 && cout > 0,
+                    "fpl_conv3d_wgrad_group: layer %d: channels %d -> %d (need cin %% 8, cout %% 16)", l, cin, cout);
+        FPL_REQUIRE(x_c8off >= 0 && x_c8off + cin / 8 <= x_c8tot && dy_c8off >= 0 && dy_c8off + cout / 8 <= dy_c8tot,
+                    "fpl_conv3d_wgrad_group: layer %d: channel slice outside its buffer", l);
+        FPL_REQUIRE((reinterpret_cast<uintptr_t>(h_x[l]) & 15) == 0 && (reinterpret_cast<uintptr_t>(h_dy[l]) & 15) == 0 &&
+                        h_x[l] != nullptr && h_dy[l] != nullptr,
+                    "fpl_conv3d_wgrad_group: layer %d: x / dy must be non-NULL and 16-byte aligned", l);
+        FPL_REQUIRE(h_scratch[l] != nullptr && (reinterpret_cast<uintptr_t>(h_scratch[l]) & 3) == 0,
+                    "fpl_conv3d_wgrad_group: layer %d: scratch must be non-NULL and 4-byte aligned", l);
+        if (encode == nullptr) encode = get_encode_fn();
+        FPL_REQUIRE(encode != nullptr, "fpl_conv3d_wgrad_group: cuTensorMapEncodeTiled not available from the driver");
+        GwLayer& L = P.L[l];
+        L.dw = h_scratch[l]; L.kind = kind; L.N = n; L.D = d; L.H = h; L.W = w; L.cin = cin; L.cout = cout; L.kd = kd;
+        L.x_c8tot = x_c8tot; L.x_c8off = x_c8off; L.dy_c8tot = dy_c8tot; L.dy_c8off = dy_c8off;
+        int stage_bytes;
+        CUresult r1, r2;
+        if (kind == 0) {
+            FPL_REQUIRE(kd == 1 || kd == 3, "fpl_conv3d_wgrad_group: layer %d: kd=%d must be 1 or 3", l, kd);
+            WgCfg c;
+            FPL_REQUIRE(make_wg_cfg(h, w, cin, cout, kd, 1, d >= 2, c),
+                        "fpl_conv3d_wgrad_group: layer %d: unsupported shape (cin %d, cout %d, %dx%d)", l, cin, cout, h, w);
+            L.ntaps = 9; L.th = c.th; L.tw = c.tw; L.nkd = c.nkd; L.c8chunk = c.c8chunk;
+            L.mtiles_c = c.mtiles_c; L.mtiles_kd = c.mtiles_kd; L.m = c.m; L.nb = c.nb; L.nchunks = c.nchunks;
+            L.ndy = c.ndy; L.ncols = c.ncols; L.dplanes = (d + c.ndy - 1) / c.ndy;
+            L.plane_x = c.plane_x; L.plane_dy = c.plane_dy; L.dy_off = c.dy_off;
+            L.tx_bytes = c.x_bytes + (c.ncols / 8) * c.plane_dy;
+            L.tiles_h = (h + c.th - 1) / c.th; L.tiles_w = (w + c.tw - 1) / c.tw;
+            stage_bytes = c.stage_bytes;
+            const int64_t tiles = (int64_t)L.tiles_h * L.tiles_w * L.dplanes * n;
+            FPL_REQUIRE(tiles < (1ll << 30), "fpl_conv3d_wgrad_group: layer %d: too many tiles", l);
+            L.tiles_total = (int)tiles;
+            tile_cost[l] = (double)(c.th / 2) * (c.tw / 8) * 9 * mma_cycles(c.m, c.ncols);
+            r1 = encode_5d(encode, &P.xmap[l], h_x[l], n, d, x_c8tot, h, w, c.tw + 2, c.th + 2, c.c8chunk, c.nkd);
+            r2 = encode_5d(encode, &P.dymap[l], h_dy[l], n, d, dy_c8tot, h, w, c.tw, c.th, c.nb / 8, c.ndy);
+        } else {
+            FPL_REQUIRE(kd == 1 || kd == 2, "fpl_conv3d_wgrad_group: layer %d: ConvT kd2=%d must be 1 or 2", l, kd);
+            CtwCfg c;
+            FPL_REQUIRE(make_ctw_cfg(cin, cout, kd, c), "fpl_conv3d_wgrad_group: layer %d: ConvT %d -> %d not tileable", l, cin, cout);
+            L.ntaps = 4 * kd; L.th = kCtTH; L.tw = kCtTW; L.nkd = 1; L.c8chunk = c.mgroups;
+            L.mtiles_c = c.mtiles; L.mtiles_kd = 1; L.m = c.m; L.nb = c.nb; L.nchunks = c.nchunks;
+            L.ndy = 1; L.ncols = c.nb; L.dplanes = d;
+            L.plane_x = kCtPlane; L.plane_dy = c.dy_tile_bytes; L.dy_off = c.x_bytes;
+            L.tx_bytes = c.stage_bytes;
+            L.tiles_h = (h + kCtTH - 1) / kCtTH; L.tiles_w = (w + kCtTW - 1) / kCtTW;
+            stage_bytes = c.stage_bytes;
+            const int64_t tiles = (int64_t)L.tiles_h * L.tiles_w * d * n;
+            FPL_REQUIRE(tiles < (1ll << 30), "fpl_conv3d_wgrad_group: layer %d: too many tiles", l);
+            L.tiles_total = (int)tiles;
+            tile_cost[l] = (double)(kCtTH / 2) * L.ntaps * mma_cycles(c.m, c.nb);
+            r1 = encode_4d(encode, &P.xmap[l], h_x[l], (int64_t)n * d * x_c8tot, h, w, c.mgroups, 1);
+            r2 = encode_4d(encode, &P.dymap[l], h_dy[l], (int64_t)n * d * kd * dy_c8tot, 2 * h, 2 * w, c.nb / 8, 2);
+        }
+        FPL_REQUIRE(r1 == CUDA_SUCCESS && r2 == CUDA_SUCCESS, "fpl_conv3d_wgrad_group: layer %d: tensor map failed (%d, %d)",
+                    l, (int)r1, (int)r2);
+        epi_cost[l] = (double)L.ntaps * L.ncols * 128 / 8;
+        max_stage = std::max(max_stage, (stage_bytes + 127) / 128 * 128);
+        max_cols = std::max(max_cols, L.ntaps * L.ncols);
+        total += tile_cost[l] * L.tiles_total * L.mtiles_c * L.mtiles_kd * L.nchunks;
+    }
+    int pad = 0;
+    for (int l = 0; l < count; ++l) {
+        const GwLayer& L = P.L[l];
+        const int window = L.kind == 0 ? (L.m / 8 + 1) * L.plane_x : (L.m / 8) * kCtPlane;
+        const int over = window - max_stage;
+        pad = std::max(pad, over);
+    }
+    pad = (pad + 127) / 128 * 128;
+    P.stage_bytes = max_stage;
+    P.stages = std::min(kMaxStagesG, (kSmemBudgetG - pad - 2048) / max_stage);
+    FPL_REQUIRE(P.stages >= 2, "fpl_conv3d_wgrad_group: stage of %d bytes does not fit twice", max_stage);
+    P.tmem_cols = 32;
+    while (P.tmem_cols < max_cols) P.tmem_cols *= 2;
+    FPL_REQUIRE(P.tmem_cols <= 512, "fpl_conv3d_wgrad_group: %d TMEM columns", max_cols);
+    const int smem_bytes = P.stages * P.stage_bytes + pad + 1024 + 256;
+
+    const int ctas_max = std::min(FPL_NUM_SMS, kGroupCtas);
+    struct Item { double cost; int code; };
+    std::vector<Item> items;
+    for (double share = total / ctas_max / 2;; share *= 2) {
+        items.clear();
+        for (int l = 0; l < count; ++l) {
+            GwLayer& L = P.L[l];
+            const double layer_tiles = tile_cost[l] * L.tiles_total;
+            int split = (int)std::min<double>(L.tiles_total, std::max(1.0, std::ceil(layer_tiles / share)));
+            const int pairs = L.mtiles_c * L.mtiles_kd * L.nchunks;
+            while (split > 1 && pairs * split > 4096) --split;
+            FPL_REQUIRE(pairs * split <= 4096, "fpl_conv3d_wgrad_group: layer %d: %d M/N tiles", l, pairs);
+            L.split = split;
+            for (int b = 0; b < pairs * split; ++b) {
+                const int s = b % split;
+                const int nt = (int)(((int64_t)L.tiles_total * (s + 1)) / split - ((int64_t)L.tiles_total * s) / split);
+                items.push_back({nt * tile_cost[l] + epi_cost[l], (l << 12) | b});
+            }
+        }
+        if ((int)items.size() <= kGroupItems) break;
+    }
+    std::stable_sort(items.begin(), items.end(), [](const Item& a, const Item& b) { return a.cost > b.cost; });
+    const int ctas = std::min<int>(ctas_max, (int)items.size());
+    std::vector<double> load(ctas, 0.0);
+    std::vector<std::vector<uint16_t>> per(ctas);
+    for (const Item& it : items) {
+        const int c = (int)(std::min_element(load.begin(), load.end()) - load.begin());
+        load[c] += it.cost;
+        per[c].push_back((uint16_t)it.code);
+    }
+    int k = 0;
+    for (int c = 0; c < ctas; ++c) {
+        P.cta_begin[c] = (uint16_t)k;
+        for (uint16_t code : per[c]) P.item[k++] = code;
+    }
+    P.cta_begin[ctas] = (uint16_t)k;
+
+    FPL_CHECK_CUDA(cudaFuncSetAttribute(wgrad_group_kernel, cudaFuncAttributeMaxDynamicSharedMemorySize, smem_bytes));
+    fpl_launch(wgrad_group_kernel, ctas, kThreadsG, smem_bytes, (cudaStream_t)stream, P);
+    FPL_LAUNCH_CHECK();
+    return 0;
+}
diff --git a/fpl-plus_b200/csrc/conv_wgrad_tc.cu b/fpl-plus_b200/csrc/conv_wgrad_tc.cu
--- a/fpl-plus_b200/csrc/conv_wgrad_tc.cu
+++ b/fpl-plus_b200/csrc/conv_wgrad_tc.cu
@@ -1,5 +1,6 @@
 #include "common.cuh"
 #include "tc_ptx.cuh"
+#include "wgrad_cfg.cuh"
 #include "../../include/fplplus_b200.h"
 
 namespace {
@@ -12,20 +13,7 @@
 constexpr int kMaxStagesW = 8;
 constexpr int kSmemBudgetW = 220 * 1024;
 
-struct WgCfg {
-    int th, tw;
-    int nkd;
-    int c8chunk;
-    int mtiles_c, mtiles_kd;
-    int m;
-    int nb, nchunks;
-    int plane_x, plane_dy;
-    int dy_off;
-    int x_bytes, dy_bytes, stage_bytes, stages, pad_bytes, smem_bytes;
-    int tmem_cols;
-    int ndy;
-    int ncols;
-};
+}
 
 bool make_wg_cfg(int h, int w, int cin, int cout, int kd, int allow_m64, int allow_pair, WgCfg& c) {
     if (cin % 8 != 0 || (cout % 16 != 0 && cout != 8) || cin <= 0 || cout <= 0) return false;
@@ -71,6 +59,8 @@
     return c.tmem_cols <= 512;
 }
 
+namespace {
+
 struct WgParams {
     float* dw;
     float* dump;
@@ -255,6 +245,8 @@
 
 float* g_wg_dump = nullptr;
 
+}
+
 CUresult encode_5d(EncodeTiledFn encode, CUtensorMap* map, const void* base, int n, int d, int c8tot, int h, int w,
                    int box_w, int box_h, int box_c8, int box_d) {
     cuuint64_t gdim[5] = {(cuuint64_t)w * 2, (cuuint64_t)h, (cuuint64_t)c8tot, (cuuint64_t)d, (cuuint64_t)n};
@@ -265,8 +257,6 @@
     return encode(map, CU_TENSOR_MAP_DATA_TYPE_UINT64, 5, const_cast<void*>(base), gdim, gstr, box, estr,
                   CU_TENSOR_MAP_INTERLEAVE_NONE, CU_TENSOR_MAP_SWIZZLE_NONE, CU_TENSOR_MAP_L2_PROMOTION_L2_128B,
                   CU_TENSOR_MAP_FLOAT_OOB_FILL_NONE);
-}
-
 }
 
 bool fpl_wgrad_hs_eligible(int d, int h, int w, int cin, int cout, int kd, int taps);
diff --git a/fpl-plus_b200/csrc/convt_tc.cu b/fpl-plus_b200/csrc/convt_tc.cu
--- a/fpl-plus_b200/csrc/convt_tc.cu
+++ b/fpl-plus_b200/csrc/convt_tc.cu
@@ -1,20 +1,14 @@
 #include "common.cuh"
 #include "tc_ptx.cuh"
+#include "wgrad_cfg.cuh"
 #include "../../include/fplplus_b200.h"
 
 namespace {
 
-constexpr int kTH = 16, kTW = 8;
-constexpr int kPlane = kTH * kTW * 16;
+constexpr int kTH = kCtTH, kTW = kCtTW;
+constexpr int kPlane = kCtPlane;
 constexpr int kThreadsT = 192;
 constexpr int kMaxStagesT = 8;
-
-__device__ __forceinline__ void tma_load_4d(void* dst, const CUtensorMap* map, uint64_t* bar, int c0, int c1, int c2, int c3) {
-    asm volatile(
-        "cp.async.bulk.tensor.4d.shared::cluster.global.tile.mbarrier::complete_tx::bytes [%0], [%1, {%3, %4, %5, %6}], [%2];"
-        ::"r"(smem_u32(dst)), "l"(map), "r"(smem_u32(bar)), "r"(c0), "r"(c1), "r"(c2), "r"(c3)
-        : "memory");
-}
 
 struct CtParams {
     const __nv_bfloat16* image;
@@ -232,17 +226,6 @@
     }
 }
 
-CUresult encode_4d(EncodeTiledFn encode, CUtensorMap* map, const void* base, int64_t planes, int h, int w, int box_c8,
-                   int stride) {
-    cuuint64_t gdim[4] = {8, (cuuint64_t)w, (cuuint64_t)h, (cuuint64_t)planes};
-    cuuint64_t gstr[3] = {16, (cuuint64_t)w * 16, (cuuint64_t)h * w * 16};
-    cuuint32_t box[4] = {8, (cuuint32_t)(kTW * stride), (cuuint32_t)(kTH * stride), (cuuint32_t)box_c8};
-    cuuint32_t estr[4] = {1, (cuuint32_t)stride, (cuuint32_t)stride, 1};
-    return encode(map, CU_TENSOR_MAP_DATA_TYPE_BFLOAT16, 4, const_cast<void*>(base), gdim, gstr, box, estr,
-                  CU_TENSOR_MAP_INTERLEAVE_NONE, CU_TENSOR_MAP_SWIZZLE_NONE, CU_TENSOR_MAP_L2_PROMOTION_L2_128B,
-                  CU_TENSOR_MAP_FLOAT_OOB_FILL_NONE);
-}
-
 struct CtwParams {
     float* dw;
     int N, D, H, W, cin, cout, kd2, ntaps;
@@ -374,6 +357,17 @@
 
 }
 
+CUresult encode_4d(EncodeTiledFn encode, CUtensorMap* map, const void* base, int64_t planes, int h, int w, int box_c8,
+                   int stride) {
+    cuuint64_t gdim[4] = {8, (cuuint64_t)w, (cuuint64_t)h, (cuuint64_t)planes};
+    cuuint64_t gstr[3] = {16, (cuuint64_t)w * 16, (cuuint64_t)h * w * 16};
+    cuuint32_t box[4] = {8, (cuuint32_t)(kTW * stride), (cuuint32_t)(kTH * stride), (cuuint32_t)box_c8};
+    cuuint32_t estr[4] = {1, (cuuint32_t)stride, (cuuint32_t)stride, 1};
+    return encode(map, CU_TENSOR_MAP_DATA_TYPE_BFLOAT16, 4, const_cast<void*>(base), gdim, gstr, box, estr,
+                  CU_TENSOR_MAP_INTERLEAVE_NONE, CU_TENSOR_MAP_SWIZZLE_NONE, CU_TENSOR_MAP_L2_PROMOTION_L2_128B,
+                  CU_TENSOR_MAP_FLOAT_OOB_FILL_NONE);
+}
+
 extern "C" int64_t fpl_convt_weight_image_bytes(int cin, int cout, int kd2) {
     return (int64_t)cin * cout * 4 * kd2 * 2;
 }
@@ -491,6 +485,25 @@
                              stream);
 }
 
+bool make_ctw_cfg(int cin, int cout, int kd2, CtwCfg& c) {
+    if (cin % 8 != 0 || cout % 16 != 0 || cin <= 0 || cout <= 0 || (kd2 != 1 && kd2 != 2)) return false;
+    const int ntaps = 4 * kd2;
+    const int g_all = cin / 8;
+    c.mgroups = g_all < 16 ? g_all : 16;
+    if (g_all % c.mgroups != 0) return false;
+    c.mtiles = g_all / c.mgroups;
+    c.m = c.mgroups <= 8 ? 64 : 128;
+    c.nb = cout % 32 == 0 ? 32 : 16;
+    c.x_bytes = c.mgroups * kCtPlane;
+    if (2 * (c.x_bytes + ntaps * (c.nb / 8) * kCtPlane) > 200 * 1024 - (c.m / 8) * kCtPlane) c.nb = 16;
+    c.nchunks = cout / c.nb;
+    c.dy_tile_bytes = (c.nb / 8) * kCtPlane;
+    c.stage_bytes = c.x_bytes + ntaps * c.dy_tile_bytes;
+    c.stages = (200 * 1024 - (c.m / 8) * kCtPlane) / c.stage_bytes;
+    if (c.stages > kMaxStagesT) c.stages = kMaxStagesT;
+    return c.stages >= 2;
+}
+
 static int convt_wgrad_launch(const void* x, int x_c8tot, int x_c8off, const void* dy, int dy_c8tot, int dy_c8off,
                               float* dw, int n, int d, int h, int w, int cin, int cout, int kd2, void* stream, int tapmajor) {
     FPL_REQUIRE(kd2 == 1 || kd2 == 2, "fpl_convt_k2s2_wgrad_tc: kd2=%d must be 1 or 2", kd2);
@@ -500,20 +513,10 @@
     CtwParams P;
     P.dw = dw; P.N = n; P.D = d; P.H = h; P.W = w; P.cin = cin; P.cout = cout; P.kd2 = kd2; P.ntaps = 4 * kd2;
     P.x_c8tot = x_c8tot; P.x_c8off = x_c8off; P.dy_c8tot = dy_c8tot; P.dy_c8off = dy_c8off; P.tapmajor = tapmajor;
-    const int g_all = cin / 8;
-    P.mgroups = g_all < 16 ? g_all : 16;
-    FPL_REQUIRE(g_all % P.mgroups == 0, "fpl_convt_k2s2_wgrad_tc: cin=%d not tileable", cin);
-    P.mtiles = g_all / P.mgroups;
-    P.m = P.mgroups <= 8 ? 64 : 128;
-    P.nb = cout % 32 == 0 ? 32 : 16;
-    P.x_bytes = P.mgroups * kPlane;
-    if (2 * (P.x_bytes + P.ntaps * (P.nb / 8) * kPlane) > 200 * 1024 - (P.m / 8) * kPlane) P.nb = 16;
-    P.nchunks = cout / P.nb;
-    P.dy_tile_bytes = (P.nb / 8) * kPlane;
-    P.stage_bytes = P.x_bytes + P.ntaps * P.dy_tile_bytes;
-    P.stages = (200 * 1024 - (P.m / 8) * kPlane) / P.stage_bytes;
-    if (P.stages > kMaxStagesT) P.stages = kMaxStagesT;
-    FPL_REQUIRE(P.stages >= 2, "fpl_convt_k2s2_wgrad_tc: stage of %d bytes does not fit twice", P.stage_bytes);
+    CtwCfg c;
+    FPL_REQUIRE(make_ctw_cfg(cin, cout, kd2, c), "fpl_convt_k2s2_wgrad_tc: cin=%d / cout=%d not tileable", cin, cout);
+    P.mgroups = c.mgroups; P.mtiles = c.mtiles; P.m = c.m; P.nb = c.nb; P.nchunks = c.nchunks;
+    P.x_bytes = c.x_bytes; P.dy_tile_bytes = c.dy_tile_bytes; P.stage_bytes = c.stage_bytes; P.stages = c.stages;
     int cols = P.ntaps * P.nb;
     P.tmem_cols = 32;
     while (P.tmem_cols < cols) P.tmem_cols *= 2;
diff --git a/fpl-plus_b200/csrc/tc_ptx.cuh b/fpl-plus_b200/csrc/tc_ptx.cuh
--- a/fpl-plus_b200/csrc/tc_ptx.cuh
+++ b/fpl-plus_b200/csrc/tc_ptx.cuh
@@ -36,6 +36,12 @@
     asm volatile(
         "cp.async.bulk.tensor.3d.shared::cluster.global.tile.mbarrier::complete_tx::bytes [%0], [%1, {%3, %4, %5}], [%2];"
         ::"r"(smem_u32(dst)), "l"(map), "r"(smem_u32(bar)), "r"(c0), "r"(c1), "r"(c2)
+        : "memory");
+}
+__device__ __forceinline__ void tma_load_4d(void* dst, const CUtensorMap* map, uint64_t* bar, int c0, int c1, int c2, int c3) {
+    asm volatile(
+        "cp.async.bulk.tensor.4d.shared::cluster.global.tile.mbarrier::complete_tx::bytes [%0], [%1, {%3, %4, %5, %6}], [%2];"
+        ::"r"(smem_u32(dst)), "l"(map), "r"(smem_u32(bar)), "r"(c0), "r"(c1), "r"(c2), "r"(c3)
         : "memory");
 }
 __device__ __forceinline__ void tma_load_5d(void* dst, const CUtensorMap* map, uint64_t* bar, int c0, int c1, int c2, int c3,
diff --git a/fpl-plus_b200/csrc/wgrad_cfg.cuh b/fpl-plus_b200/csrc/wgrad_cfg.cuh
--- /dev/null
+++ b/fpl-plus_b200/csrc/wgrad_cfg.cuh
@@ -0,0 +1,31 @@
+#pragma once
+#include "tc_ptx.cuh"
+
+struct WgCfg {
+    int th, tw;
+    int nkd;
+    int c8chunk;
+    int mtiles_c, mtiles_kd;
+    int m;
+    int nb, nchunks;
+    int plane_x, plane_dy;
+    int dy_off;
+    int x_bytes, dy_bytes, stage_bytes, stages, pad_bytes, smem_bytes;
+    int tmem_cols;
+    int ndy;
+    int ncols;
+};
+bool make_wg_cfg(int h, int w, int cin, int cout, int kd, int allow_m64, int allow_pair, WgCfg& c);
+CUresult encode_5d(EncodeTiledFn encode, CUtensorMap* map, const void* base, int n, int d, int c8tot, int h, int w,
+                   int box_w, int box_h, int box_c8, int box_d);
+
+constexpr int kCtTH = 16, kCtTW = 8;
+constexpr int kCtPlane = kCtTH * kCtTW * 16;
+struct CtwCfg {
+    int mgroups, mtiles, m;
+    int nb, nchunks;
+    int x_bytes, dy_tile_bytes, stage_bytes, stages;
+};
+bool make_ctw_cfg(int cin, int cout, int kd2, CtwCfg& c);
+CUresult encode_4d(EncodeTiledFn encode, CUtensorMap* map, const void* base, int64_t planes, int h, int w, int box_c8,
+                   int stride);
diff --git a/fpl-plus_b200/lib.py b/fpl-plus_b200/lib.py
--- a/fpl-plus_b200/lib.py
+++ b/fpl-plus_b200/lib.py
@@ -37,6 +37,8 @@
     "fpl_conv3d_wgrad_tc_tapmajor": (_I, [_P, _I, _I, _P, _I, _I, _P] + [_I] * 7 + [_P]),
     "fpl_wgrad_tapmajor_to_dw_batch": (_I, [_I, ctypes.POINTER(c_void_p), ctypes.POINTER(c_void_p), ctypes.POINTER(_I),
                                             ctypes.POINTER(_I), ctypes.POINTER(_I), ctypes.POINTER(_I), _P]),
+    "fpl_conv3d_wgrad_group": (_I, [_I, ctypes.POINTER(_I), ctypes.POINTER(c_void_p), ctypes.POINTER(c_void_p),
+                                    ctypes.POINTER(c_void_p), _P]),
     "fpl_dsbn_eval_affine_batch": (_I, [_I] + [ctypes.POINTER(c_void_p)] * 7 + [ctypes.POINTER(_I), _F, _P]),
     "fpl_conv3d_tc_act": (_I, [_P, _I, _I, _P, _P, _I, _I] + [_I] * 7 + [_P, _P, _P, _F, _U, _U, _P, _P]),
     "fpl_conv3d_tc_dfold_act": (_I, [_P, _I, _I, _P, _P, _I, _I] + [_I] * 6 + [_P, _P, _P, _P]),
diff --git a/fpl-plus_b200/net.py b/fpl-plus_b200/net.py
--- a/fpl-plus_b200/net.py
+++ b/fpl-plus_b200/net.py
@@ -875,8 +875,12 @@
         if impl == "tc" and u.cin % 8 == 0 and u.cout % 16 == 0 and ops.is_sm100():
             if fold is not None:
                 scr = fold["alloc"](u.cout * u.cin * u.kd * 9)
-                call("fpl_conv3d_wgrad_tc_tapmajor", *xin.args(), ptr(dy), u.cout // 8, 0, ptr(scr), n, d, h, w, u.cin,
-                     u.cout, u.kd, stream_ptr())
+                if d * h * w <= fold["group_vox"]:
+                    fold["group"].append(((0, n, d, h, w, u.cin, u.cout, u.kd, *xin.args()[1:], u.cout // 8, 0),
+                                          xin.args()[0], ptr(dy), ptr(scr)))
+                else:
+                    call("fpl_conv3d_wgrad_tc_tapmajor", *xin.args(), ptr(dy), u.cout // 8, 0, ptr(scr), n, d, h, w, u.cin,
+                         u.cout, u.kd, stream_ptr())
                 fold["pending"].append((scr, dw, u.cout, u.cin, u.kd * 9))
                 return
             call("fpl_conv3d_wgrad_tc", *xin.args(), ptr(dy), u.cout // 8, 0, ptr(dw), n, d, h, w, u.cin, u.cout,
@@ -921,9 +925,21 @@
                 t = scratch[cursor[0]:cursor[0] + numel]
                 cursor[0] += (numel + 3) // 4 * 4
                 return t
-            fold = {"alloc": alloc, "pending": []}
+            group_vox = geo[2][0] * geo[2][1] * geo[2][2] if len(geo) > 2 else 0
+            fold = {"alloc": alloc, "pending": [], "group": [], "group_vox": group_vox}
+
+        def flush_group():
+            if fold is None or not fold["group"]:
+                return
+            part = fold["group"]
+            m = len(part)
+            desc = (ctypes.c_int * (12 * m))(*[v for t in part for v in t[0]])
+            arrs = [(ctypes.c_void_p * m)(*[t[k] for t in part]) for k in (1, 2, 3)]
+            call("fpl_conv3d_wgrad_group", m, desc, *arrs, stream_ptr())
+            fold["group"] = []
 
         def flush_fold():
+            flush_group()
             if fold is None or not fold["pending"]:
                 return
             self._join_aux()
@@ -1033,8 +1049,12 @@
                      *glow.args(), n, dl, hl, wl, c_low, c, kd2, st)
                 if fold is not None:
                     scr = fold["alloc"](c_low * c * 4 * kd2)
-                    call("fpl_convt_k2s2_wgrad_tc_tapmajor", *low.args(), ptr(dcat.buf), 2 * c // 8, c // 8, ptr(scr),
-                         n, dl, hl, wl, c_low, c, kd2, st)
+                    if dl * hl * wl <= fold["group_vox"]:
+                        fold["group"].append(((1, n, dl, hl, wl, c_low, c, kd2, *low.args()[1:], 2 * c // 8, c // 8),
+                                              low.args()[0], ptr(dcat.buf), ptr(scr)))
+                    else:
+                        call("fpl_convt_k2s2_wgrad_tc_tapmajor", *low.args(), ptr(dcat.buf), 2 * c // 8, c // 8, ptr(scr),
+                             n, dl, hl, wl, c_low, c, kd2, st)
                     fold["pending"].append((scr, grads[trans.weight], c, c_low, -4 * kd2))
                 else:
                     call("fpl_convt_k2s2_wgrad_tc", *low.args(), ptr(dcat.buf), 2 * c // 8, c // 8, ptr(grads[trans.weight]),
@@ -1062,6 +1082,8 @@
                 g_pool = self._unit_bwd(u1, r1, g, None, None, 0, n, ws, small, grads, True, fold)
             else:
                 self._unit_bwd(u1, r1, g, None, None, 0, n, ws, small, grads, False, fold)
+            if i == 0 or fold is None or geo[i - 1][0] * geo[i - 1][1] * geo[i - 1][2] > fold["group_vox"]:
+                flush_group()
             done += 10
             fire(done)
         assert done == len(params)
diff --git a/include/fplplus_b200.h b/include/fplplus_b200.h
--- a/include/fplplus_b200.h
+++ b/include/fplplus_b200.h
@@ -136,6 +136,11 @@
                             float* dw, int n, int d, int h, int w, int cin, int cout, int kd2, void* stream);
 int fpl_convt_k2s2_wgrad_tc_tapmajor(const void* x, int x_c8tot, int x_c8off, const void* dy, int dy_c8tot, int dy_c8off,
                                      float* scratch, int n, int d, int h, int w, int cin, int cout, int kd2, void* stream);
+
+#define FPL_WGRAD_GROUP_MAX 16
+#define FPL_WGRAD_GROUP_DESC 12
+int fpl_conv3d_wgrad_group(int count, const int* h_desc, const void* const* h_x, const void* const* h_dy,
+                           float* const* h_scratch, void* stream);
 
 
 int fpl_dsbn_finalize(const double* stats, int64_t count, const float* gamma, const float* beta,
```

Result: faster. 1.048 billion, median of 6 (+4.0%).
